# caki35/UNet-Torch

Measured on AMD Instinct MI355X. Metric: images/sec training step, 4-level U-Net 1ch→2cls 512×512, at 1/2/4/8 MI355X, higher is better.
Workload: dtype f16

## Files before the change

### include/unetmi.h

```cpp
#ifndef UNETMI_H
#define UNETMI_H
#include <stddef.h>
#include <stdint.h>

#ifdef __cplusplus
extern "C" {
#endif

typedef void* umi_stream_t;

enum { UMI_F32 = 0, UMI_F16 = 1 };
enum { UMI_OK = 0, UMI_ERR_BADARG = -1, UMI_ERR_UNSUPPORTED = -2, UMI_ERR_WORKSPACE = -3 };
enum { UMI_CONV_UPSAMPLE2 = 1,
       UMI_CONV_FORCE_GENERIC = 2,
       UMI_CONV_DGRAD_STRIDED = 4,
       UMI_CONV_ACCUMULATE = 8,
       UMI_CONV_F32_MFMA = 16       };

int umi_version(void);
const char* umi_arch(void);

int umi_tune_conv3x3_impl(int impl);

int umi_pack_kn(const float* src, void* dst, int T, int K, int N, long st, long sk, long sn,
                int flip_t, int Kpad, int Npad, int dtype, umi_stream_t stream);

int umi_pack_kn8(const float* src, void* dst, int T, int K, int N, long st, long sk, long sn,
                 int flip_t, int Kpad, int Npad, int dtype, umi_stream_t stream);

int umi_conv_fwd(const void* x, int ldx, const void* tx, const void* wp, const float* bias,
                 void* y, int ldy, float* stat_part,
                 int N, int H, int W, int Ci, int Co, int R, int S, int stride, int pad,
                 int Ho, int Wo, int off_h, int off_w, int out_H, int out_W,
                 int in_dtype, int out_dtype, int flags, umi_stream_t stream);
int umi_linear_fused(const void* x, int ldx, const void* wp8, const float* bias, void* y, int ldy, long M, int Ci, int Co,
                     int epi, float p, unsigned seed, const unsigned* seed_dev, void* mask, const void* aux, int ldaux,
                     void* y2, int ldy2, int dtype, umi_stream_t stream);

int umi_conv_fwd_plan(int N, int H, int W, int Ci, int Co, int R, int S, int stride, int pad,
                      int ldx, int ldy, int in_dtype, int out_dtype, int flags, int has_bias,
                      int* layout, int* stat_rows);

int umi_bn_finalize(const float* stat_part, int rows, int C, double count,
                    const float* gamma, const float* beta, float eps, float momentum,
                    float* running_mean, float* running_var,
                    void* tx_out, float* rstd_out, umi_stream_t stream);

int umi_pool2_fwd(const void* x, int ldx, const void* tx, void* y, int ldy,
                  int N, int H, int W, int C, int dtype, umi_stream_t stream);
int umi_pool2_bwd(const void* dpool, int lddp, const void* x, int ldx, const void* tx,
                  void* da, int ldda, int accumulate,
                  int N, int H, int W, int C, int dtype, umi_stream_t stream);

size_t umi_bn_bwd_ws_bytes(long M, int C);
int umi_bn_bwd_reduce(const void* da, int ldda, const void* y, int ldy, const void* tx,
                      const float* rstd, float* sum_dz, float* sum_dzx,
                      long M, int C, int dtype, void* ws, size_t ws_bytes, umi_stream_t stream);
int umi_bn_bwd_apply(void* da, int ldda, const void* y, int ldy, const void* tx,
                     const float* rstd, const float* sum_dz, const float* sum_dzx,
                     long M, int C, int dtype, umi_stream_t stream);

int umi_conv_dgrad_bnred(const void* dy, int lddy, const void* wp8, void* da, int ldda, const void* ybn, int ldybn,
                         const void* txbn, const float* rstd, float* part, int N, int H, int W, int Ci, int Co,
                         int dtype, umi_stream_t stream);

int umi_conv_gather_bnred_rows(int N, int H, int W, int Ci, int Co, int R, int S, int stride, int pad, int Ho, int Wo,
                               int ldx, int ldy, int dtype, int flags);
int umi_conv_gather_bnred(const void* x, int ldx, const void* wp8, void* y, int ldy, const void* ybn, int ldybn,
                          const void* txbn, const float* rstd, float* part, int N, int H, int W, int Ci, int Co, int R, int S,
                          int stride, int pad, int Ho, int Wo, int dtype, int flags, umi_stream_t stream);

int umi_head_dgrad_bnred_rows(long P, int Ci, int Co, int ldda, int dtype);
int umi_head_dgrad_bnred(const void* dl, int lddl, const void* wp, void* da, int ldda, const void* ybn, int ldybn,
                         const void* txbn, const float* rstd, float* part, long P, int Ci, int Co, int dtype,
                         umi_stream_t stream);
size_t umi_head_bwd_fused_ws_bytes(long P, int Ci, int Co);
int umi_head_bwd_fused(const void* dl, int lddl, const void* wp, void* da, int ldda, const void* ybn, int ldybn,
                       const void* txbn, const float* rstd, float* part, float* dW, long s_co, long s_ci, float out_scale,
                       void* ws, size_t ws_bytes, long P, int Ci, int Co, int dtype, umi_stream_t stream);

int umi_conv3x3_fwd_act(const void* x, int ldx, const void* tx, const void* wp8, const void* out_tx, void* y, int ldy,
                        int N, int H, int W, int Ci, int Co, int dtype, umi_stream_t stream);
int umi_bn_stats_rows(long M, int C);
int umi_bn_stats(const void* x, int ldx, float* part, long M, int C, int dtype, umi_stream_t stream);
int umi_pool2_bwd_bnred_stat_rows(int N, int H, int W, int C);
int umi_pool2_bwd_bnred(const void* dpool, int lddp, const void* x, int ldx, const void* tx, const float* rstd, void* da,
                        int ldda, int accumulate, float* part, int N, int H, int W, int C, int dtype, umi_stream_t stream);
int umi_bn_bwd_from_partials(const float* part, int rows, int C, float* sum_dz, float* sum_dzx, umi_stream_t stream);

size_t umi_conv_wgrad_ws_bytes(int N, int Ho, int Wo, int Ci, int Co, int R, int S, int dtype, int flags);
int umi_conv_wgrad(const void* x, int ldx, const void* txa, const void* dy, int lddy, const void* txb,
                   float* dW, long s_co, long s_ci, long s_t, float out_scale,
                   int N, int H, int W, int Ci, int Co, int R, int S, int stride, int pad,
                   int Ho, int Wo, int dtype, int flags, void* ws, size_t ws_bytes, umi_stream_t stream);
typedef struct umi_wgrad_pending {
    const float* part;
    float* dW;
    long s_co, s_ci, s_t;
    float scale;
    int splits, RS, Ci, Co;
} umi_wgrad_pending;
int umi_conv_wgrad_deferred(const void* x, int ldx, const void* txa, const void* dy, int lddy, const void* txb,
                            float* dW, long s_co, long s_ci, long s_t, float out_scale, int N, int H, int W, int Ci, int Co,
                            int R, int S, int stride, int pad, int Ho, int Wo, int dtype, int flags, void* ws, size_t ws_bytes,
                            umi_wgrad_pending* out, umi_stream_t stream);
int umi_wgrad_reduce_group(int n, const void* items , umi_stream_t stream);
int umi_conv_wgrad_bias(const void* x, int ldx, const void* dy, int lddy, const void* txb, float* dW, long s_co, long s_ci,
                        long s_t, float* dbias, float out_scale, int N, int H, int W, int Ci, int Co, int Ho, int Wo, int dtype,
                        int flags, void* ws, size_t ws_bytes, umi_wgrad_pending* out, umi_stream_t stream);
int umi_conv_wgrad_group(int n, const void* const* x, int ldx, const void* const* dy, int lddy, float* const* dW, long s_co,
                         long s_ci, float out_scale, long M, int Ci, int Co, int dtype, umi_stream_t stream);
int umi_conv_wgrad_bnapply(const void* x, int ldx, const void* txa, const void* da, int ldda, const void* y, int ldy,
                           const void* tx_bn, const float* rstd, const float* sum_dz, const float* sum_dzx, void* dz,
                           int lddz, float* dW, long s_co, long s_ci, long s_t, float out_scale, int N, int H, int W,
                           int Ci, int Co, int R, int S, int stride, int pad, int dtype, int flags, void* ws,
                           size_t ws_bytes, umi_stream_t stream);

size_t umi_colsum_ws_bytes(long M, int C);
int umi_colsum(const void* x, int ldx, float* out, float out_scale, long M, int C, int dtype,
               void* ws, size_t ws_bytes, umi_stream_t stream);
int umi_colsum_group(int n, const void* const* xs, int ldx, float* const* outs, float out_scale, long M, int C, int dtype,
                     void* ws, size_t ws_bytes, umi_stream_t stream);

int umi_materialize_nchw(const void* x, int ldx, const void* tx, float* y_nchw,
                         int N, int H, int W, int C, int dtype, umi_stream_t stream);


int umi_wstd_fwd(const float* w, float* wstd, float* rstd, int Co, int K, float eps, umi_stream_t stream);
int umi_wstd_bwd(const float* wstd, const float* rstd, const float* g, float* dw, int Co, int K, umi_stream_t stream);
typedef struct umi_wstd_desc {
    const float* w;
    float* ws;
    float* rstd;
    long off;
    int Co, K;
    float eps;
    int blk0;
    float* dw;
} umi_wstd_desc;
int umi_wstd_fwd_multi(const void* descs, int n_desc, int total_rows, umi_stream_t stream);
int umi_wstd_bwd_multi(const void* descs, int n_desc, int total_rows, const float* g_base, float* dw_base, umi_stream_t stream);

size_t umi_gn_fwd_ws_bytes(int N, long HW, int C);
int umi_gn_fwd(const void* x, int ldx, const float* gamma, const float* beta, const void* res, int ldr, void* y, int ldy,
               float* mean, float* rstd, int relu, int N, long HW, int C, int G, float eps, int dtype,
               void* ws, size_t ws_bytes, umi_stream_t stream);
size_t umi_gn_bwd_ws_bytes(int N, long HW, int C, int G);
int umi_gn_bwd(const void* dy, int lddy, const void* y, int ldy, const void* x, int ldx, const float* mean,
               const float* rstd, const float* gamma, int relu, void* dx, int lddx, void* dres, int lddr,
               float* dgamma, float* dbeta, float out_scale, int N, long HW, int C, int G, int dtype,
               void* ws, size_t ws_bytes, float* part_out, umi_stream_t stream);
int umi_gn_param_grads_group(int n, const float* const* parts, const int* Cs, int N, float* const* dgammas,
                             float* const* dbetas, float out_scale, umi_stream_t stream);

int umi_pool3s2_fwd(const void* x, int ldx, void* y, int ldy, void* idx, int N, int H, int W, int C, int dtype,
                    umi_stream_t stream);
int umi_pool3s2_bwd(const void* dy, int lddy, const void* x, int ldx, const void* idx, void* dx, int lddx, int N, int H, int W,
                    int C, int dtype, umi_stream_t stream);

int umi_ln_fwd(const void* x, int ldx, const float* gamma, const float* beta, void* y, int ldy, float* mean, float* rstd,
               long M, int C, float eps, int dtype, umi_stream_t stream);
size_t umi_ln_bwd_ws_bytes(long M, int C);
int umi_ln_bwd(const void* dy, int lddy, const void* x, int ldx, const float* gamma, const float* mean,
               const float* rstd, void* dx, int lddx, float* dgamma, float* dbeta, float out_scale, long M, int C,
               int dtype, void* ws, size_t ws_bytes, int* rows_out, umi_stream_t stream);

int umi_elementwise(int mode, const void* x, int ldx, const void* g, int ldg, void* y, int ldy, long M, int C,
                    long bcast_rows, int dtype, umi_stream_t stream);

int umi_dropout(const void* x, int ldx, void* y, int ldy, void* mask, int backward, float p, unsigned seed, long M, int C,
                int dtype, const void* tx, const unsigned* seed_dev, umi_stream_t stream);
int umi_dropout_fused(const void* x, int ldx, void* y, int ldy, void* mask, int backward, float p, unsigned seed, long M, int C,
                      int dtype, const unsigned* seed_dev, const void* aux, int ldaux, int gelu, umi_stream_t stream);

int umi_attn_fwd(const void* q, const void* k, const void* v, int ld, void* o, int ldo, float* lse, int B, int N, int heads,
                 int D, int dtype, umi_stream_t stream);
int umi_attn_bwd(const void* q, const void* k, const void* v, int ld, const void* o, const void* dO, int ldo,
                 const float* lse, void* dq, void* dk, void* dv, int ldd, float* delta, int B, int N, int heads, int D,
                 int dtype, umi_stream_t stream);

int umi_bilinear2x(const void* x, int ldx, const void* tx, void* y, int ldy, int backward, int N, int H, int W, int C,
                   int dtype, umi_stream_t stream);

size_t umi_dice_ce_ws_bytes(int N, int C, long HW);
int umi_dice_ce_fwd(const float* logits, const void* target, int target_dtype, int N, int C, long HW, float* stats, void* ws,
                    size_t ws_bytes, umi_stream_t stream);
int umi_dice_ce_bwd(const float* logits, const void* target, int target_dtype, const float* stats, const float* gout, int N,
                    int C, long HW, float* dlogits, umi_stream_t stream);

size_t umi_hdt_ws_bytes(int B, int H, int W);
int umi_hdt_fwd(const float* pred, const float* target, int B, int C, int H, int W, float alpha, float* D, float* fields,
                float* loss, void* ws, size_t ws_bytes, umi_stream_t stream);
int umi_hdt_bwd(const float* pred, const float* target, const float* D, const float* gout, int B, int C, int H, int W,
                float* dpred, umi_stream_t stream);

size_t umi_binloss_ws_bytes(int B, int C, long HW);
int umi_dice_bce_fwd(const float* pred, const float* target, int B, long HW, double* stats, float* loss, void* ws,
                     size_t ws_bytes, umi_stream_t stream);
int umi_dice_bce_bwd(const float* pred, const float* target, const double* stats, const float* gout, int B, long HW,
                     float* dpred, umi_stream_t stream);
int umi_tversky_fwd(const float* pred, const void* target, int target_dtype, int B, int C, long HW, float alpha, float beta,
                    double* stats, float* loss, void* ws, size_t ws_bytes, umi_stream_t stream);
int umi_tversky_bwd(const float* pred, const void* target, int target_dtype, const double* stats, const float* gout, int B,
                    int C, long HW, float alpha, float beta, float* dpred, umi_stream_t stream);

size_t umi_topk_loss_ws_bytes(long N);
int umi_topk_loss_fwd(const float* pred, const float* target, long N, long k, int mode, unsigned char* mask, float* loss,
                      void* ws, size_t ws_bytes, umi_stream_t stream);
int umi_topk_loss_bwd(const float* pred, const float* target, const unsigned char* mask, const float* gout, long N, long k,
                      float* dpred, umi_stream_t stream);

size_t umi_mt_ratio_ws_bytes(int B, long HW);
size_t umi_mt_ratio_stats_len(int B);
int umi_mt_ratio_fwd(const float* o1, const float* o2, const float* l1, const float* l2, int B, long HW, int gate,
                     const float* gate_dev, double* stats, float* loss, float* loss1, float* loss2, float* ratio, void* ws, size_t ws_bytes,
                     umi_stream_t stream);
int umi_mt_ratio_bwd(const float* o1, const float* o2, const float* l1, const float* l2, const double* stats,
                     const float* gout, int B, long HW, float* d1, float* d2, umi_stream_t stream);

typedef struct umi_optim_desc {
    float* p;
    const float* g;
    float* s0;
    float* s1;
    long n;
    int blk0;
    int pad_;
} umi_optim_desc;
int umi_optim_block_elems(void);
int umi_table_upload(const void* host_pinned, void* dev, size_t nbytes, umi_stream_t stream);
int umi_optim_sgd_multi(const void* descs, int n_desc, int total_blocks, double lr, double momentum, double dampening,
                        double weight_decay, int nesterov, int first_step, umi_stream_t stream);
int umi_optim_adam_multi(const void* descs, int n_desc, int total_blocks, double step_size, double beta1, double beta2,
                         double bc2_sqrt, double eps, double weight_decay, umi_stream_t stream);

typedef struct umi_optim_hyper {
    double lr, base_lr, iter, max_iter, power, adam_t, beta1, beta2;
    float lr_f, step_size_f, bc2_sqrt_f, pad_;
    double pad2_[2];
} umi_optim_hyper;
size_t umi_optim_hyper_bytes(void);
int umi_optim_hyper_pre(void* hyper, int adam, umi_stream_t stream);
int umi_optim_hyper_poly(void* hyper, umi_stream_t stream);
int umi_optim_sgd_multi_dev(const void* descs, int n_desc, int total_blocks, const void* hyper, double momentum,
                            double dampening, double weight_decay, int nesterov, int first_step, umi_stream_t stream);
int umi_optim_adam_multi_dev(const void* descs, int n_desc, int total_blocks, const void* hyper, double beta1, double beta2,
                             double eps, double weight_decay, umi_stream_t stream);

typedef struct umi_pack_desc {
    const float* src;
    void* dst;
    long st, sk, sn;
    int T, K, N, flip_t, Kpad, Npad, k8, blk0;
    int ldn, pad_;
} umi_pack_desc;
int umi_pack_block_elems(void);
int umi_pack_kn_multi(const void* descs, int n_desc, int total_blocks, int dtype, umi_stream_t stream);

int umi_add2_relu_fwd(const void* a, int lda, const void* txa, const void* b, int ldb, const void* txb, void* y, int ldy,
                      long M, int C, int dtype, umi_stream_t stream);
int umi_add2_relu_bwd(const void* dy, int lddy, const void* y, int ldy, void* da, int ldda, void* db, int lddb, long M, int C,
                      int dtype, umi_stream_t stream);
int umi_gate_fwd(const void* x, int ldx, const void* txx, const void* p, const void* txp, void* y, int ldy, long M, int C,
                 int dtype, umi_stream_t stream);
int umi_gate_bwd(const void* dy, int lddy, const void* x, int ldx, const void* txx, const void* p, const void* txp, void* dx,
                 int lddx, void* dp, long M, int C, int dtype, umi_stream_t stream);

size_t umi_znorm_ws_bytes(void);
int umi_znorm_hwc(const void* img, int src_dtype, float* out_chw, long HW, int C, int reverse_channels, void* ws,
// ... 57 lines not shown
```

### unet-torch_amd/csrc/api.hip

```cpp
#include "kernels.h"
#include <stdio.h>
#include <stdlib.h>

static ConvFwdProblem fwd_problem(int N, int H, int W, int Ci, int Co, int R, int S, int stride, int pad, int Ho, int Wo, int ldx,
                                  int ldy, int in_dtype, int out_dtype, int flags, bool has_tx, bool has_bias, bool has_stats) {
    return ConvFwdProblem{N, H, W, Ci, Co, R, S, stride, pad, Ho, Wo, ldx, ldy, in_dtype, out_dtype, flags, has_tx, has_bias, has_stats};
}
static ConvFwdProblem fwd_problem_3x3(int N, int H, int W, int Ci, int Co, int ldx, int ldy, int dtype, bool has_tx) {
    return fwd_problem(N, H, W, Ci, Co, 3, 3, 1, 1, H, W, ldx, ldy, dtype, dtype, 0, has_tx, false, false);
}

extern "C" int umi_version(void) { return 1; }
extern "C" const char* umi_arch(void) { return "gfx950"; }

extern "C" int umi_linear_fused(const void* x, int ldx, const void* wp8, const float* bias, void* y, int ldy, long M, int Ci,
                                int Co, int epi, float p, unsigned seed, const unsigned* seed_dev, void* mask, const void* aux,
                                int ldaux, void* y2, int ldy2, int dtype, umi_stream_t stream) {
    if (!x || !wp8 || !y || !mask || M <= 0 || M >= (1L << 31) || Ci <= 0 || Co <= 0 || !(p >= 0.f && p <= 1.f)) return UMI_ERR_BADARG;
    if (epi != 1 && epi != 2) return UMI_ERR_BADARG;
    if ((epi == 1 && (!y2 || ldy2 % 8)) || (epi == 2 && (!aux || ldaux % 8))) return UMI_ERR_BADARG;
    const ConvFwdProblem pr = fwd_problem(1, 1, (int)M, Ci, Co, 1, 1, 1, 0, 1, (int)M, ldx, ldy, dtype, dtype, 0, false, bias != nullptr, false);
    if (umi_conv_fwd_path(pr) != FWD_MFMA1X1) return UMI_ERR_UNSUPPORTED;
    if (((uintptr_t)x | (uintptr_t)y | (uintptr_t)wp8 | (uintptr_t)y2 | (uintptr_t)aux) & 15 || ((uintptr_t)mask & 7)) return UMI_ERR_UNSUPPORTED;
    const UmiLinearEpi e{epi, p, seed, seed_dev, mask, aux, ldaux, y2, ldy2, nullptr, nullptr, nullptr};
    return umi_conv1x1_mfma(pr, x, nullptr, wp8, bias, y, 0, 0, 1, (int)M, (hipStream_t)stream, &e);
}

extern "C" int umi_conv_gather_bnred_rows(int N, int H, int W, int Ci, int Co, int R, int S, int stride, int pad, int Ho, int Wo,
                                          int ldx, int ldy, int dtype, int flags) {
    if (flags & (UMI_CONV_UPSAMPLE2 | UMI_CONV_ACCUMULATE | UMI_CONV_FORCE_GENERIC)) return 0;
    const ConvFwdProblem p = fwd_problem(N, H, W, Ci, Co, R, S, stride, pad, Ho, Wo, ldx, ldy, dtype, dtype, flags, false, false, false);
    if (umi_conv_fwd_path(p) != FWD_MFMA1X1 || umi_conv3x3_mfma_ok(p)) return 0;
    return umi_conv1x1_bnred_rows((long)N * Ho * Wo, Co);
}
extern "C" int umi_conv_gather_bnred(const void* x, int ldx, const void* wp8, void* y, int ldy, const void* ybn, int ldybn,
                                     const void* txbn, const float* rstd, float* part, int N, int H, int W, int Ci, int Co, int R,
                                     int S, int stride, int pad, int Ho, int Wo, int dtype, int flags, umi_stream_t stream) {
    if (!x || !wp8 || !y || !ybn || !txbn || !rstd || !part || N <= 0 || H <= 0 || W <= 0) return UMI_ERR_BADARG;
    if (umi_conv_gather_bnred_rows(N, H, W, Ci, Co, R, S, stride, pad, Ho, Wo, ldx, ldy, dtype, flags) <= 0 || ldybn % 8 || ldybn < Co)
        return UMI_ERR_UNSUPPORTED;
    if (((uintptr_t)x | (uintptr_t)y | (uintptr_t)wp8 | (uintptr_t)ybn) & 15) return UMI_ERR_BADARG;
    const UmiLinearEpi e{3, 0.f, 0u, nullptr, nullptr, ybn, ldybn, nullptr, 0, txbn, rstd, part};
    const ConvFwdProblem p = fwd_problem(N, H, W, Ci, Co, R, S, stride, pad, Ho, Wo, ldx, ldy, dtype, dtype, flags, false, false, false);
    return umi_conv1x1_mfma(p, x, nullptr, wp8, nullptr, y, 0, 0, Ho, Wo, (hipStream_t)stream, &e);
}

extern "C" int umi_conv_fwd_plan(int N, int H, int W, int Ci, int Co, int R, int S, int stride, int pad, int ldx,
                                 int ldy, int in_dtype, int out_dtype, int flags, int has_bias, int* layout,
                                 int* stat_rows) {
    if (N <= 0 || H <= 0 || W <= 0 || Ci <= 0 || Co <= 0 || R <= 0 || S <= 0 || stride <= 0) return UMI_ERR_BADARG;
    const bool ups = flags & UMI_CONV_UPSAMPLE2;
    const int Ho = ups ? H : (H + 2 * pad - R) / stride + 1, Wo = ups ? W : (W + 2 * pad - S) / stride + 1;
    const ConvFwdPath path = umi_conv_fwd_path(fwd_problem(N, H, W, Ci, Co, R, S, stride, pad, Ho, Wo, ldx, ldy, in_dtype, out_dtype,
                                                           flags, false, has_bias != 0, true));
    if ((flags & UMI_CONV_ACCUMULATE) && path != FWD_MFMA1X1) return UMI_ERR_UNSUPPORTED;
    if (layout) *layout = (path == FWD_MFMA3X3 || path == FWD_MFMA1X1) ? 1 : 0;
    if (stat_rows)
        *stat_rows = path == FWD_MFMA3X3_F32 ? umi_conv3x3_f32_mfma_stat_rows(N, H, W)
                     : path == FWD_MFMA3X3 ? umi_conv3x3_mfma_stat_rows(N, H, W, Co)
                     : path == FWD_STEM  ? umi_stem_stat_rows(N, H, W)
                     : path == FWD_HEAD  ? umi_head_stat_rows((long)N * H * W, Ci)
                                         : umi_cdiv((long)N * Ho * Wo, 64);
    return UMI_OK;
}

extern "C" int umi_conv_dgrad_bnred(const void* dy, int lddy, const void* wp8, void* da, int ldda, const void* ybn, int ldybn,
                                    const void* txbn, const float* rstd, float* part, int N, int H, int W, int Ci, int Co,
                                    int dtype, umi_stream_t stream) {
    if (!dy || !wp8 || !da || !ybn || !txbn || !rstd || !part || N <= 0 || H <= 0 || W <= 0) return UMI_ERR_BADARG;
    const ConvFwdProblem p = fwd_problem_3x3(N, H, W, Ci, Co, lddy, ldda, dtype, false);
    if (umi_conv_fwd_path(p) != FWD_MFMA3X3 || ldybn % 8 || ldybn < Co) return UMI_ERR_UNSUPPORTED;
    if (((uintptr_t)dy | (uintptr_t)da | (uintptr_t)wp8 | (uintptr_t)ybn) & 15) return UMI_ERR_BADARG;
    return umi_conv3x3_mfma_bnred(p, dy, wp8, da, ybn, ldybn, txbn, rstd, part, (hipStream_t)stream);
}

static bool head_dgrad_ok(int Ci, int Co, int ldda, int dtype) {
    return umi_smallk_fwd_ok(fwd_problem(1, 1, 1, Ci, Co, 1, 1, 1, 0, 1, 1, Ci, ldda, dtype, dtype, 0, false, false, false));
}
extern "C" int umi_head_dgrad_bnred_rows(long P, int Ci, int Co, int ldda, int dtype) {
    if (!head_dgrad_ok(Ci, Co, ldda, dtype)) return 0;
    return umi_smallk_bnred_rows(P, Co);
}
extern "C" int umi_head_dgrad_bnred(const void* dl, int lddl, const void* wp, void* da, int ldda, const void* ybn, int ldybn,
                                    const void* txbn, const float* rstd, float* part, long P, int Ci, int Co, int dtype,
                                    umi_stream_t stream) {
    if (!dl || !wp || !da || !ybn || !txbn || !rstd || !part || P <= 0) return UMI_ERR_BADARG;
    if (!head_dgrad_ok(Ci, Co, ldda, dtype) || ldybn % 8 || ldybn < Co || lddl < Ci) return UMI_ERR_UNSUPPORTED;
    return umi_smallk_fwd_bnred(dl, lddl, wp, da, ldda, ybn, ldybn, txbn, rstd, part, P, Ci, Co, (hipStream_t)stream);
}
extern "C" size_t umi_head_bwd_fused_ws_bytes(long P, int Ci, int Co) {
    return (size_t)umi_smallk_bnred_rows(P, Co) * Co * Ci * sizeof(float);
}
extern "C" int umi_head_bwd_fused(const void* dl, int lddl, const void* wp, void* da, int ldda, const void* ybn, int ldybn,
                                  const void* txbn, const float* rstd, float* part, float* dW, long s_co, long s_ci, float out_scale,
                                  void* ws, size_t ws_bytes, long P, int Ci, int Co, int dtype, umi_stream_t stream) {
    if (!dl || !wp || !da || !ybn || !txbn || !rstd || !part || !dW || !ws || P <= 0) return UMI_ERR_BADARG;
    if (!head_dgrad_ok(Ci, Co, ldda, dtype) || Co > 256 || ldybn % 8 || ldybn < Co || lddl < Ci) return UMI_ERR_UNSUPPORTED;
    return umi_smallk_fwd_bnred(dl, lddl, wp, da, ldda, ybn, ldybn, txbn, rstd, part, P, Ci, Co, (hipStream_t)stream, dW, s_co, s_ci,
                                out_scale, ws, ws_bytes);
}

extern "C" int umi_conv3x3_fwd_act(const void* x, int ldx, const void* tx, const void* wp8, const void* out_tx, void* y, int ldy,
                                   int N, int H, int W, int Ci, int Co, int dtype, umi_stream_t stream) {
    if (!x || !wp8 || !out_tx || !y || N <= 0 || H <= 0 || W <= 0 || ldx < Ci || ldy < Co) return UMI_ERR_BADARG;
    const ConvFwdProblem p = fwd_problem_3x3(N, H, W, Ci, Co, ldx, ldy, dtype, tx != nullptr);
    if (umi_conv_fwd_path(p) != FWD_MFMA3X3) return UMI_ERR_UNSUPPORTED;
    if (((uintptr_t)x | (uintptr_t)y | (uintptr_t)wp8 | (uintptr_t)out_tx) & 15) return UMI_ERR_BADARG;
    return umi_conv3x3_mfma_act(p, x, tx, wp8, out_tx, y, (hipStream_t)stream);
}

extern "C" int umi_bn_stats_rows(long M, int C) { return umi_colsum_rows_f16v(M, C); }
extern "C" int umi_bn_stats(const void* x, int ldx, float* part, long M, int C, int dtype, umi_stream_t stream) {
    if (!x || !part || M <= 0 || C <= 0 || ldx < C) return UMI_ERR_BADARG;
    if (dtype != UMI_F16 || !umi_bn_stats_f16v(x, ldx, part, M, C, (hipStream_t)stream)) return UMI_ERR_UNSUPPORTED;
    UMI_LAUNCH_CHECK();
    return UMI_OK;
}

extern "C" int umi_pool2_bwd_bnred(const void* dpool, int lddp, const void* x, int ldx, const void* tx, const float* rstd,
                                   void* da, int ldda, int accumulate, float* part, int N, int H, int W, int C, int dtype,
                                   umi_stream_t stream) {
    if (!dpool || !x || !tx || !rstd || !da || !part || N <= 0 || H <= 0 || W <= 0 || C <= 0) return UMI_ERR_BADARG;
    if (dtype != UMI_F16) return UMI_ERR_UNSUPPORTED;
    if (!umi_pool2_bwd_bnred_f16v(dpool, lddp, x, ldx, tx, rstd, da, ldda, accumulate, part, N, H, W, C, (hipStream_t)stream))
        return UMI_ERR_UNSUPPORTED;
    UMI_LAUNCH_CHECK();
    return UMI_OK;
}
extern "C" int umi_pool2_bwd_bnred_stat_rows(int N, int H, int W, int C) { return umi_pool2_bwd_bnred_rows(N, H, W, C); }

extern "C" int umi_bn_bwd_from_partials(const float* part, int rows, int C, float* sum_dz, float* sum_dzx, umi_stream_t stream) {
    if (!part || !sum_dz || !sum_dzx || rows <= 0 || C <= 0) return UMI_ERR_BADARG;
    umi_launch_reduce_rows2(part, rows, C, sum_dz, sum_dzx, 1.f, (hipStream_t)stream);
    UMI_LAUNCH_CHECK();
    return UMI_OK;
}

static bool trace_generic() {
    static const bool on = [] { const char* e = getenv("UMI_TRACE_GENERIC"); return e && e[0] == '1'; }();
    return on;
}
#define UMI_TRACE(kind)                                                                                                  \
    if (trace_generic())                                                                                                 \
        fprintf(stderr, "[umi generic %s] N=%d H=%d W=%d Ci=%d Co=%d R=%d stride=%d pad=%d flags=%d\n", kind, N, H, W, Ci, Co, R, \
                stride, pad, flags)

extern "C" int umi_conv_fwd(const void* x, int ldx, const void* tx, const void* wp, const float* bias, void* y, int ldy,
                            float* stat_part, int N, int H, int W, int Ci, int Co, int R, int S, int stride, int pad,
                            int Ho, int Wo, int off_h, int off_w, int out_H, int out_W, int in_dtype, int out_dtype,
                            int flags, umi_stream_t stream) {
    if (!x || !wp || !y || N <= 0 || H <= 0 || W <= 0 || Ci <= 0 || Co <= 0 || R <= 0 || S <= 0 || stride <= 0 ||
        Ho <= 0 || Wo <= 0 || ldx < Ci || ldy < Co || out_H <= 0 || out_W <= 0)
        return UMI_ERR_BADARG;
    ConvFwdProblem p = fwd_problem(N, H, W, Ci, Co, R, S, stride, pad, Ho, Wo, ldx, ldy, in_dtype, out_dtype, flags,
                                   tx != nullptr, bias != nullptr, stat_part != nullptr);
    const ConvFwdPath path = umi_conv_fwd_path(p);
    if (path != FWD_MFMA3X3_F32) p.flags = flags &= ~UMI_CONV_F32_MFMA;
    if ((flags & UMI_CONV_ACCUMULATE) && (stat_part || path != FWD_MFMA1X1)) return UMI_ERR_UNSUPPORTED;
    if (flags & UMI_CONV_DGRAD_STRIDED) {
        if (flags & UMI_CONV_UPSAMPLE2) return UMI_ERR_BADARG;
        if (H != (Ho + 2 * pad - R) / stride + 1 || W != (Wo + 2 * pad - S) / stride + 1) return UMI_ERR_BADARG;
        if (out_H != Ho || out_W != Wo || off_h || off_w || stat_part) return UMI_ERR_BADARG;
    } else if (!(flags & UMI_CONV_UPSAMPLE2)) {
        if (Ho != (H + 2 * pad - R) / stride + 1 || Wo != (W + 2 * pad - S) / stride + 1) return UMI_ERR_BADARG;
        if (out_H != Ho || out_W != Wo || off_h || off_w) return UMI_ERR_BADARG;
    } else {
        if (Ho != H || Wo != W) return UMI_ERR_BADARG;
    }
    const hipStream_t s = (hipStream_t)stream;
    switch (path) {
    case FWD_MFMA3X3_F32: return umi_conv3x3_f32_mfma(p, x, tx, wp, y, stat_part, s);
    case FWD_MFMA3X3:
        if (((uintptr_t)x | (uintptr_t)y | (uintptr_t)wp) & 15) return UMI_ERR_BADARG;
        return umi_conv3x3_mfma(p, x, tx, wp, y, stat_part, s);
    case FWD_MFMA1X1:
        if (stat_part) return UMI_ERR_UNSUPPORTED;
        if (((uintptr_t)x | (uintptr_t)y | (uintptr_t)wp) & 15) return UMI_ERR_BADARG;
        return umi_conv1x1_mfma(p, x, tx, wp, bias, y, off_h, off_w, out_H, out_W, s);
    case FWD_STEM: return umi_stem_fwd(p, x, tx, wp, y, stat_part, s);
    case FWD_HEAD: return umi_head_fwd(p, x, tx, wp, bias, y, stat_part, s);
    case FWD_SMALLK: return umi_smallk_fwd(p, x, wp, y, s);
    case FWD_ROOT: return umi_root_fwd(p, x, wp, y, s);
    case FWD_HEAD3: return umi_head3_fwd(p, x, tx, wp, bias, y, s);
    case FWD_GENERIC: break;
    }
    UMI_TRACE((flags & UMI_CONV_DGRAD_STRIDED) ? "dgrad_strided" : "fwd");
    return umi_conv_fwd_generic(p, x, tx, wp, bias, y, stat_part, off_h, off_w, out_H, out_W, s);
}

static WgradProblem wgrad_problem(int N, int H, int W, int Ci, int Co, int R, int S, int stride, int pad, int Ho, int Wo, int ldx,
                                  int lddy, int dtype, int flags, bool has_txa, bool has_txb) {
    return WgradProblem{N, H, W, Ci, Co, R, S, stride, pad, Ho, Wo, ldx, lddy, dtype, flags, has_txa, has_txb};
}

extern "C" size_t umi_conv_wgrad_ws_bytes(int N, int Ho, int Wo, int Ci, int Co, int R, int S, int dtype, int flags) {
    WgradProblem p = wgrad_problem(N, 0, 0, Ci, Co, R, S, 0, 0, Ho, Wo, 0, 0, dtype, flags, false, false);
    const size_t f32_mfma = umi_wgrad3x3_f32_mfma_ws_bound(p);
    p.flags &= ~UMI_CONV_F32_MFMA;
    const size_t bounds[] = {f32_mfma, umi_wgrad3x3_mfma_ws_bound(p), umi_wgrad1x1_mfma_ws_bound(p), umi_wgradT_mfma_ws_bound(p),
                             umi_wgrad_gather_mfma_ws_bound(p), umi_stem_wgrad_ws_bound(p), umi_head_wgrad_ws_bound(p),
                             umi_root_wgrad_ws_bound(p), umi_head3_wgrad_ws_bound(p), umi_conv_wgrad_generic_ws_bound(p)};
    size_t most = 0;
    for (size_t b : bounds) most = b > most ? b : most;
    return most;
}

static int conv_wgrad(const WgradProblem& asked, WgradPath path, const void* x, const void* txa, const void* dy, const void* txb,
                      const WgradOut& o, hipStream_t s) {
    WgradProblem p = asked;
    if (path != WGRAD_MFMA3X3_F32) p.flags &= ~UMI_CONV_F32_MFMA;
    if (!x || !dy || !o.dW || !o.ws || p.N <= 0 || p.H <= 0 || p.W <= 0 || p.Ci <= 0 || p.Co <= 0 || p.ldx < p.Ci || p.lddy < p.Co)
        return UMI_ERR_BADARG;
    switch (path) {
    case WGRAD_MFMA3X3_F32: return umi_wgrad3x3_f32_mfma(p, x, txa, dy, o, s);
    case WGRAD_MFMA3X3: return umi_wgrad3x3_mfma(p, x, txa, dy, o, s);
    case WGRAD_MFMA1X1: return umi_wgrad1x1_mfma(p, x, txa, dy, o, s);
    case WGRAD_T: return umi_wgradT_mfma(p, x, dy, txb, o, s);
    case WGRAD_GATHER: return umi_wgrad_gather_mfma(p, x, txa, dy, o, s);
    case WGRAD_STEM: return umi_stem_wgrad(p, x, txa, dy, o, s);
    case WGRAD_HEAD: return umi_head_wgrad(p, x, txa, dy, o, s);
    case WGRAD_ROOT: return umi_root_wgrad(p, x, dy, o, s);
    case WGRAD_HEAD3: return umi_head3_wgrad(p, x, txa, dy, o, s);
    case WGRAD_GENERIC: break;
    }
    if (trace_generic())
        fprintf(stderr, "[umi generic wgrad] N=%d H=%d W=%d Ci=%d Co=%d R=%d stride=%d pad=%d flags=%d\n", p.N, p.H, p.W, p.Ci, p.Co,
                p.R, p.stride, p.pad, p.flags);
    return umi_conv_wgrad_generic(p, x, txa, dy, txb, o, s);
}

extern "C" int umi_conv_wgrad(const void* x, int ldx, const void* txa, const void* dy, int lddy, const void* txb,
                              float* dW, long s_co, long s_ci, long s_t, float out_scale, int N, int H, int W, int Ci,
                              int Co, int R, int S, int stride, int pad, int Ho, int Wo, int dtype, int flags, void* ws,
                              size_t ws_bytes, umi_stream_t stream) {
    const WgradProblem p = wgrad_problem(N, H, W, Ci, Co, R, S, stride, pad, Ho, Wo, ldx, lddy, dtype, flags, txa != nullptr, txb != nullptr);
    const WgradOut o{dW, s_co, s_ci, s_t, out_scale, ws, ws_bytes, nullptr, nullptr};
    return conv_wgrad(p, umi_conv_wgrad_path(p), x, txa, dy, txb, o, (hipStream_t)stream);
}

extern "C" int umi_conv_wgrad_deferred(const void* x, int ldx, const void* txa, const void* dy, int lddy, const void* txb,
                                       float* dW, long s_co, long s_ci, long s_t, float out_scale, int N, int H, int W, int Ci,
                                       int Co, int R, int S, int stride, int pad, int Ho, int Wo, int dtype, int flags, void* ws,
                                       size_t ws_bytes, umi_wgrad_pending* out, umi_stream_t stream) {
    if (!out) return UMI_ERR_BADARG;
    out->part = nullptr;
    const WgradProblem p = wgrad_problem(N, H, W, Ci, Co, R, S, stride, pad, Ho, Wo, ldx, lddy, dtype, flags, txa != nullptr, txb != nullptr);
    const WgradOut o{dW, s_co, s_ci, s_t, out_scale, ws, ws_bytes, out, nullptr};
    return conv_wgrad(p, umi_conv_wgrad_path(p), x, txa, dy, txb, o, (hipStream_t)stream);
}

extern "C" int umi_conv_wgrad_bias(const void* x, int ldx, const void* dy, int lddy, const void* txb, float* dW, long s_co,
                                   long s_ci, long s_t, float* dbias, float out_scale, int N, int H, int W, int Ci, int Co, int Ho,
                                   int Wo, int dtype, int flags, void* ws, size_t ws_bytes, umi_wgrad_pending* out,
                                   umi_stream_t stream) {
    if (!dbias) return UMI_ERR_BADARG;
    const WgradProblem p = wgrad_problem(N, H, W, Ci, Co, 2, 2, 2, 0, Ho, Wo, ldx, lddy, dtype, flags, false, txb != nullptr);
    if (umi_conv_wgrad_path(p) != WGRAD_T) return UMI_ERR_UNSUPPORTED;
    if (out) out->part = nullptr;
    const WgradOut o{dW, s_co, s_ci, s_t, out_scale, ws, ws_bytes, out, dbias};
    return conv_wgrad(p, WGRAD_T, x, nullptr, dy, txb, o, (hipStream_t)stream);
}

extern "C" int umi_conv_wgrad_group(int n, const void* const* x, int ldx, const void* const* dy, int lddy, float* const* dW,
                                    long s_co, long s_ci, float out_scale, long M, int Ci, int Co, int dtype,
                                    umi_stream_t stream) {
    if (n <= 0 || !x || !dy || !dW || M <= 0 || Ci <= 0 || Co <= 0 || ldx < Ci || lddy < Co) return UMI_ERR_BADARG;
    for (int i = 0; i < n; ++i)
        if (!x[i] || !dy[i] || !dW[i]) return UMI_ERR_BADARG;
    if (M >= (1L << 31) ||
        umi_conv_wgrad_path(wgrad_problem(1, 1, (int)M, Ci, Co, 1, 1, 1, 0, 1, (int)M, ldx, lddy, dtype, 0, false, false)) != WGRAD_MFMA1X1)
        return UMI_ERR_UNSUPPORTED;
    return umi_wgrad1x1_mfma_group(n, x, ldx, dy, lddy, dW, s_co, s_ci, out_scale, M, Ci, Co, (hipStream_t)stream);
}

extern "C" int umi_conv_wgrad_bnapply(const void* x, int ldx, const void* txa, const void* da, int ldda, const void* y, int ldy,
                                      const void* tx_bn, const float* rstd, const float* sum_dz, const float* sum_dzx,
                                      void* dz, int lddz, float* dW, long s_co, long s_ci, long s_t, float out_scale, int N,
                                      int H, int W, int Ci, int Co, int R, int S, int stride, int pad, int dtype, int flags,
                                      void* ws, size_t ws_bytes, umi_stream_t stream) {
    if (!x || !da || !y || !tx_bn || !rstd || !sum_dz || !sum_dzx || !dW || !ws || N <= 0 || H <= 0 || W <= 0 || Ci <= 0 ||
        Co <= 0 || ldx < Ci || ldda < Co || ldy < Co || (dz && (lddz < Co || dz == da || dz == y)))
        return UMI_ERR_BADARG;
    const WgradProblem p = wgrad_problem(N, H, W, Ci, Co, R, S, stride, pad, H, W, ldx, ldda, dtype, flags, txa != nullptr, false);
    const WgradPath path = umi_conv_wgrad_path(p);
    const WgradOut o{dW, s_co, s_ci, s_t, out_scale, ws, ws_bytes, nullptr, nullptr};
    const WgradBnApply bna{y, ldy, tx_bn, rstd, sum_dz, sum_dzx, dz, lddz};
    if (!dz) {
        if (path != WGRAD_STEM || ldy % 8) return UMI_ERR_UNSUPPORTED;
        return umi_stem_wgrad(p, x, txa, da, o, (hipStream_t)stream, &bna);
    }
    if (path != WGRAD_MFMA3X3 || ldy % 8 || lddz % 8 || (long)H * W * (ldy > lddz ? ldy : lddz) * 2 >= 0x7FFFFFF0L)
        return UMI_ERR_UNSUPPORTED;
    return umi_wgrad3x3_mfma(p, x, txa, da, o, (hipStream_t)stream, &bna);
}
```

### unet-torch_amd/csrc/common.h

```cpp
#pragma once
#include <hip/hip_runtime.h>
#include <stdint.h>
#include <stddef.h>
#include "../../include/unetmi.h"

typedef _Float16 half_t;

#define UMI_LAUNCH_CHECK()                                    \
    do {                                                      \
        hipError_t e__ = hipGetLastError();                   \
        if (e__ != hipSuccess) return (int)e__;               \
    } while (0)

__device__ __forceinline__ float umi_tx_pre(float v, const float4 t) {
    return fmaf(v, t.y, t.z);
}
__device__ __forceinline__ float umi_tx(float v, const float4 t) {
    return fmaxf(umi_tx_pre(v, t), t.w);
}

__device__ __forceinline__ float umi_bn_dz_inner(float y, float g, const float4 t, float rstd, float c1, float c2) {
#pragma clang fp contract(off)
    const float z = umi_tx_pre(y, t);
    const float dz = z > t.w ? g : 0.f;
    const float xh = (y - t.x) * rstd;
    return fmaf(-xh, c2, dz - c1);
}
__device__ __forceinline__ unsigned umi_mul2_f16(float a0, float b0, float a1, float b1) {
    unsigned r;
    asm("v_fma_mixlo_f16 %0, %1, %2, 0\n\tv_fma_mixhi_f16 %0, %3, %4, 0" : "=&v"(r) : "v"(a0), "v"(b0), "v"(a1), "v"(b1));
    return r;
}
__device__ __forceinline__ _Float16 umi_mul_f16(float a, float b) {
    unsigned r;
    asm("v_fma_mixlo_f16 %0, %1, %2, 0" : "=v"(r) : "v"(a), "v"(b));
    return __builtin_bit_cast(_Float16, (unsigned short)(r & 0xffffu));
}
template <typename T>
__device__ __forceinline__ T umi_bn_dz(float y, float g, const float4 t, float rstd, float c1, float c2);
template <>
__device__ __forceinline__ _Float16 umi_bn_dz<_Float16>(float y, float g, const float4 t, float rstd, float c1, float c2) {
    return umi_mul_f16(t.y, umi_bn_dz_inner(y, g, t, rstd, c1, c2));
}
template <>
__device__ __forceinline__ float umi_bn_dz<float>(float y, float g, const float4 t, float rstd, float c1, float c2) {
    return t.y * umi_bn_dz_inner(y, g, t, rstd, c1, c2);
}

typedef _Float16 umi_half8 __attribute__((ext_vector_type(8)));
typedef unsigned umi_uint4v __attribute__((ext_vector_type(4)));
__device__ __forceinline__ umi_half8 umi_bn_dz8(umi_half8 y, umi_half8 g, const float4* t, const float* rstd, const float* c1,
                                                const float* c2) {
    umi_uint4v r;
#pragma unroll
    for (int j = 0; j < 4; ++j)
        r[j] = umi_mul2_f16(t[2 * j].y, umi_bn_dz_inner((float)y[2 * j], (float)g[2 * j], t[2 * j], rstd[2 * j], c1[2 * j], c2[2 * j]),
                            t[2 * j + 1].y, umi_bn_dz_inner((float)y[2 * j + 1], (float)g[2 * j + 1], t[2 * j + 1], rstd[2 * j + 1],
                                                            c1[2 * j + 1], c2[2 * j + 1]));
    return __builtin_bit_cast(umi_half8, r);
}
__device__ __forceinline__ umi_half8 umi_tx8(umi_half8 v, const float4* t) {
#ifdef UMI_EXP_TX_PK
    umi_half8 sc, sh, lo_;
#pragma unroll
    for (int j = 0; j < 8; ++j) { sc[j] = (half_t)t[j].y; sh[j] = (half_t)t[j].z; lo_[j] = (half_t)t[j].w; }
    return __builtin_elementwise_max(v * sc + sh, lo_);
#endif
    typedef unsigned int u32x4 __attribute__((ext_vector_type(4)));
    u32x4 in = __builtin_bit_cast(u32x4, v), out;
    umi_half8 lo;
#pragma unroll
    for (int p = 0; p < 4; ++p) {
        unsigned d;
        asm("v_fma_mixlo_f16 %0, %1, %2, %3 op_sel_hi:[1,0,0]\n\t"
            "v_fma_mixhi_f16 %0, %1, %4, %5 op_sel:[1,0,0] op_sel_hi:[1,0,0]"
            : "=&v"(d)
            : "v"(in[p]), "v"(t[2 * p].y), "v"(t[2 * p].z), "v"(t[2 * p + 1].y), "v"(t[2 * p + 1].z));
        out[p] = d;
        lo[2 * p] = (half_t)t[2 * p].w;
        lo[2 * p + 1] = (half_t)t[2 * p + 1].w;
    }
    return __builtin_elementwise_max(__builtin_bit_cast(umi_half8, out), lo);
}

template <typename T> __device__ __forceinline__ float umi_ld(const T* p) { return (float)(*p); }
template <typename T> __device__ __forceinline__ void umi_st(T* p, float v) { *p = (T)v; }

static inline int umi_cdiv(long a, long b) { return (int)((a + b - 1) / b); }

__device__ __forceinline__ void umi_divmod(long i, int d, long& q, int& r) {
    if ((unsigned long)i <= 0xFFFFFFFFul) {
        const unsigned ui = (unsigned)i, qq = ui / (unsigned)d;
        q = (long)qq;
        r = (int)(ui - qq * (unsigned)d);
    } else {
        q = i / d;
        r = (int)(i - q * d);
    }
}
```

### unet-torch_amd/csrc/kernels.h

```cpp
#pragma once
#include "common.h"

struct ConvFwdProblem {
    int N, H, W, Ci, Co, R, S, stride, pad, Ho, Wo, ldx, ldy, in_dtype, out_dtype, flags;
    bool has_tx, has_bias, has_stats;
};
enum ConvFwdPath { FWD_MFMA3X3_F32, FWD_MFMA3X3, FWD_MFMA1X1, FWD_STEM, FWD_HEAD, FWD_SMALLK, FWD_ROOT, FWD_HEAD3, FWD_GENERIC };

bool umi_conv3x3_f32_mfma_ok(const ConvFwdProblem& p);
bool umi_conv3x3_mfma_ok(const ConvFwdProblem& p);
bool umi_conv1x1_mfma_ok(const ConvFwdProblem& p);
bool umi_stem_fwd_ok(const ConvFwdProblem& p);
bool umi_head_fwd_ok(const ConvFwdProblem& p);
bool umi_smallk_fwd_ok(const ConvFwdProblem& p);
bool umi_root_fwd_ok(const ConvFwdProblem& p);
bool umi_head3_fwd_ok(const ConvFwdProblem& p);

inline ConvFwdPath umi_conv_fwd_path(const ConvFwdProblem& p) {
    if (p.flags & UMI_CONV_F32_MFMA) {
        if (umi_conv3x3_f32_mfma_ok(p)) return FWD_MFMA3X3_F32;
        ConvFwdProblem q = p;
        q.flags &= ~UMI_CONV_F32_MFMA;
        return umi_conv_fwd_path(q);
    }
    if (p.flags & UMI_CONV_DGRAD_STRIDED)
        return umi_conv1x1_mfma_ok(p) ? FWD_MFMA1X1 : FWD_GENERIC;
    if (umi_conv3x3_mfma_ok(p)) return FWD_MFMA3X3;
    if (umi_conv1x1_mfma_ok(p)) return FWD_MFMA1X1;
    if (umi_stem_fwd_ok(p)) return FWD_STEM;
    if ((!p.has_stats || p.out_dtype == UMI_F16) && umi_head_fwd_ok(p)) return FWD_HEAD;
    if (p.has_stats) return FWD_GENERIC;
    if (umi_smallk_fwd_ok(p)) return FWD_SMALLK;
    if (umi_root_fwd_ok(p)) return FWD_ROOT;
    if (umi_head3_fwd_ok(p)) return FWD_HEAD3;
    return FWD_GENERIC;
}

struct UmiLinearEpi {
    int mode; float p; unsigned seed; const unsigned* seed_dev; void* mask; const void* aux; int ldaux; void* y2; int ldy2;
    const void* bn_tx; const float* bn_rstd; float* bn_part;
};

int umi_conv_fwd_generic(const ConvFwdProblem& p, const void* x, const void* tx, const void* wp, const float* bias, void* y,
                         float* stat_part, int off_h, int off_w, int out_H, int out_W, hipStream_t s);
int umi_conv3x3_f32_mfma_stat_rows(int N, int H, int W);
int umi_conv3x3_f32_mfma(const ConvFwdProblem& p, const void* x, const void* tx, const void* wp, void* y, float* stat_part,
                         hipStream_t s);
int umi_conv3x3_mfma_stat_rows(int N, int H, int W, int Co);
int umi_conv3x3_mfma(const ConvFwdProblem& p, const void* x, const void* tx, const void* wp8, void* y, float* stat_part,
                     hipStream_t s);
int umi_conv3x3_mfma_bnred(const ConvFwdProblem& p, const void* dy, const void* wp8, void* da, const void* ybn, int ldybn,
                           const void* txbn, const float* rstd, float* part, hipStream_t s);
int umi_conv3x3_mfma_act(const ConvFwdProblem& p, const void* x, const void* tx, const void* wp8, const void* out_tx, void* y,
                         hipStream_t s);
int umi_conv1x1_bnred_rows(long M, int Ntot);
int umi_conv1x1_mfma(const ConvFwdProblem& p, const void* x, const void* tx, const void* wp8, const float* bias, void* y,
                     int off_h, int off_w, int out_H, int out_W, hipStream_t s, const UmiLinearEpi* epi = nullptr);
int umi_stem_stat_rows(int N, int H, int W);
int umi_stem_fwd(const ConvFwdProblem& p, const void* x, const void* tx, const void* wp, void* y, float* part, hipStream_t s);
int umi_head_stat_rows(long P, int Ci);
int umi_head_fwd(const ConvFwdProblem& p, const void* x, const void* tx, const void* wp, const float* bias, void* y, float* part,
                 hipStream_t s);
int umi_smallk_fwd(const ConvFwdProblem& p, const void* x, const void* wp, void* y, hipStream_t s);
int umi_smallk_bnred_rows(long P, int Co);
int umi_smallk_fwd_bnred(const void* x, int ldx, const void* wp, void* y, int ldy, const void* ybn, int ldybn, const void* txbn,
                         const float* rstd, float* part, long P, int Ci, int Co, hipStream_t s, float* dW = nullptr, long s_co = 0,
                         long s_ci = 0, float out_scale = 1.f, void* ws = nullptr, size_t ws_bytes = 0);
int umi_root_fwd(const ConvFwdProblem& p, const void* x, const void* wp, void* y, hipStream_t s);
int umi_head3_fwd(const ConvFwdProblem& p, const void* x, const void* tx, const void* wp, const float* bias, void* y,
                  hipStream_t s);

struct WgradProblem {
    int N, H, W, Ci, Co, R, S, stride, pad, Ho, Wo, ldx, lddy, dtype, flags;
    bool has_txa, has_txb;
};
struct WgradOut {
    float* dW; long s_co, s_ci, s_t; float out_scale;
    void* ws; size_t ws_bytes;
    umi_wgrad_pending* defer;
    float* convT_bias;
};
struct WgradBnApply { const void* y; int ldy; const void* tx_bn; const float *rstd, *sum_dz, *sum_dzx; void* dz; int lddz; };
enum WgradPath { WGRAD_MFMA3X3_F32, WGRAD_MFMA3X3, WGRAD_MFMA1X1, WGRAD_T, WGRAD_GATHER, WGRAD_STEM, WGRAD_HEAD, WGRAD_ROOT, WGRAD_HEAD3, WGRAD_GENERIC };

bool umi_wgrad3x3_f32_mfma_ok(const WgradProblem& p);
bool umi_wgrad3x3_mfma_ok(const WgradProblem& p);
bool umi_wgrad1x1_mfma_ok(const WgradProblem& p);
bool umi_wgradT_mfma_ok(const WgradProblem& p);
bool umi_wgrad_gather_mfma_ok(const WgradProblem& p);
bool umi_stem_wgrad_ok(const WgradProblem& p);
bool umi_head_wgrad_ok(const WgradProblem& p);
bool umi_root_wgrad_ok(const WgradProblem& p);
bool umi_head3_wgrad_ok(const WgradProblem& p);

inline WgradPath umi_conv_wgrad_path(const WgradProblem& p) {
    if (p.flags & UMI_CONV_F32_MFMA) {
        if (umi_wgrad3x3_f32_mfma_ok(p)) return WGRAD_MFMA3X3_F32;
        WgradProblem q = p;
        q.flags &= ~UMI_CONV_F32_MFMA;
        return umi_conv_wgrad_path(q);
    }
    if (umi_wgrad3x3_mfma_ok(p)) return WGRAD_MFMA3X3;
    if (umi_wgrad1x1_mfma_ok(p)) return WGRAD_MFMA1X1;
    if (umi_wgradT_mfma_ok(p)) return WGRAD_T;
    if (umi_wgrad_gather_mfma_ok(p)) return WGRAD_GATHER;
    if (umi_stem_wgrad_ok(p)) return WGRAD_STEM;
    if (umi_head_wgrad_ok(p)) return WGRAD_HEAD;
    if (umi_root_wgrad_ok(p)) return WGRAD_ROOT;
    if (umi_head3_wgrad_ok(p)) return WGRAD_HEAD3;
    return WGRAD_GENERIC;
}

size_t umi_wgrad3x3_f32_mfma_ws_bound(const WgradProblem& p);
size_t umi_wgrad3x3_mfma_ws_bound(const WgradProblem& p);
size_t umi_wgrad1x1_mfma_ws_bound(const WgradProblem& p);
size_t umi_wgradT_mfma_ws_bound(const WgradProblem& p);
size_t umi_wgrad_gather_mfma_ws_bound(const WgradProblem& p);
size_t umi_stem_wgrad_ws_bound(const WgradProblem& p);
size_t umi_head_wgrad_ws_bound(const WgradProblem& p);
size_t umi_root_wgrad_ws_bound(const WgradProblem& p);
size_t umi_head3_wgrad_ws_bound(const WgradProblem& p);
size_t umi_conv_wgrad_generic_ws_bound(const WgradProblem& p);

int umi_wgrad3x3_f32_mfma(const WgradProblem& p, const void* x, const void* txa, const void* dy, const WgradOut& o, hipStream_t s);
int umi_wgrad3x3_mfma(const WgradProblem& p, const void* x, const void* txa, const void* dy, const WgradOut& o, hipStream_t s,
                      const WgradBnApply* bna = nullptr);
int umi_wgrad1x1_mfma(const WgradProblem& p, const void* x, const void* txa, const void* dy, const WgradOut& o, hipStream_t s);
int umi_wgradT_mfma(const WgradProblem& p, const void* x, const void* dy, const void* txb, const WgradOut& o, hipStream_t s);
int umi_wgrad_gather_mfma(const WgradProblem& p, const void* x, const void* txa, const void* dy, const WgradOut& o, hipStream_t s);
int umi_stem_wgrad(const WgradProblem& p, const void* x, const void* txa, const void* dy, const WgradOut& o, hipStream_t s,
                   const WgradBnApply* bna = nullptr);
int umi_head_wgrad(const WgradProblem& p, const void* x, const void* txa, const void* dy, const WgradOut& o, hipStream_t s);
int umi_root_wgrad(const WgradProblem& p, const void* x, const void* dy, const WgradOut& o, hipStream_t s);
int umi_head3_wgrad(const WgradProblem& p, const void* x, const void* txa, const void* dy, const WgradOut& o, hipStream_t s);
int umi_conv_wgrad_generic(const WgradProblem& p, const void* x, const void* txa, const void* dy, const void* txb,
                           const WgradOut& o, hipStream_t s);
int umi_wgrad1x1_mfma_group(int n, const void* const* x, int ldx, const void* const* dy, int lddy, float* const* dW, long s_co,
                            long s_ci, float out_scale, long M, int Ci, int Co, hipStream_t s);

void umi_launch_wgrad_reduce(int splits, int RS, int Ci, int Co, const WgradOut& o, hipStream_t s);
void umi_launch_reduce_rows2(const float* ws, int rows, int C, float* out0, float* out1, float scale, hipStream_t s);

int umi_bn_bwd_rpb_f16v(long M);
int umi_colsum_rows_f16v(long M, int C);
bool umi_colsum_f16v(const void* x, int ldx, float* ws, long M, int C, hipStream_t s);
bool umi_colsum_group_f16v(int n, const void* const* xs, int ldx, float* const* outs, float scale, float* ws, long M, int C,
                           hipStream_t s);
bool umi_bn_stats_f16v(const void* x, int ldx, float* part, long M, int C, hipStream_t s);
bool umi_bn_bwd_reduce1_f16v(const void* da, int ldda, const void* y, int ldy, const void* tx, const float* rstd, float* ws,
                             long M, int C, hipStream_t s);
bool umi_bn_bwd_apply_f16v(void* da, int ldda, const void* y, int ldy, const void* tx, const float* rstd,
                           const float* sum_dz, const float* sum_dzx, long M, int C, hipStream_t s);
bool umi_pool2_fwd_f16v(const void* x, int ldx, const void* tx, void* y, int ldy, int N, int H, int W, int C,
                        hipStream_t s);
bool umi_pool2_bwd_f16v(const void* dp, int lddp, const void* x, int ldx, const void* tx, void* da, int ldda,
                        int accumulate, int N, int H, int W, int C, hipStream_t s);
int umi_pool2_bwd_bnred_rows(int N, int H, int W, int C);
bool umi_pool2_bwd_bnred_f16v(const void* dp, int lddp, const void* x, int ldx, const void* tx, const float* rstd, void* da,
                              int ldda, int accumulate, float* part, int N, int H, int W, int C, hipStream_t s);

int umi_gn_splits(int N, long HW);
bool umi_gn_fwd_f16v(const void* x, int ldx, const float* gamma, const float* beta, const void* res, int ldr, void* y, int ldy,
                     float* mean, float* rstd, int relu, int N, long HW, int C, int G, float eps, float* ws, hipStream_t s);
bool umi_gn_bwd_f16v(const void* dy, int lddy, const void* y, int ldy, const void* x, int ldx, const float* mean,
                     const float* rstd, const float* gamma, int relu, void* dx, int lddx, void* dres, int lddr, int N, long HW,
                     int C, int G, float* part, float* ws, hipStream_t s);
void umi_gn_param_grads_launch(int n, const float* const* parts, const int* Cs, int N, float* const* dgammas, float* const* dbetas,
                               float scale, hipStream_t s);

bool umi_ew_f16v(int mode, const void* x, int ldx, const void* g, int ldg, void* y, int ldy, long M, int C, long bcast_rows,
                 hipStream_t s);
bool umi_pool3s2_fwd_f16v(const void* x, int ldx, void* y, int ldy, void* idx, int N, int H, int W, int C, hipStream_t s);
bool umi_pool3s2_bwd_f16v(const void* dy, int lddy, const void* idx, void* dx, int lddx, int N, int H, int W, int C, hipStream_t s);
bool umi_dropout_f16v(const void* x, int ldx, void* y, int ldy, void* mask, int backward, float p, unsigned seed, long M, int C,
                      const void* tx, const unsigned* seed_dev, hipStream_t s);
bool umi_dropout_fused_f16v(const void* x, int ldx, void* y, int ldy, void* mask, int backward, float p, unsigned seed, long M,
                            int C, const unsigned* seed_dev, const void* aux, int ldaux, int gelu, hipStream_t s);
int umi_ln_bwd_rows_f16v();
bool umi_ln_bwd_f16v(const void* dy, int lddy, const void* x, int ldx, const float* gamma, const float* mean, const float* rstd,
                     void* dx, int lddx, float* part, long M, int C, hipStream_t s);
bool umi_bilinear2x_f16v(const void* x, int ldx, const void* tx, void* y, int ldy, int backward, int N, int H, int W, int C,
                         hipStream_t s);

bool umi_attn_mfma_ok(int D, int ld, int ldo, int dtype, const void* a, const void* b, const void* c);
int umi_attn_fwd_mfma(const void* q, const void* k, const void* v, int ld, void* o, int ldo, float* lse, int B, int N, int Hh,
                      hipStream_t s);
int umi_attn_bwd_mfma(const void* q, const void* k, const void* v, int ld, const void* o, const void* dO, int ldo,
                      const float* lse, void* dq, void* dk, void* dv, int ldd, float* delta, int B, int N, int Hh,
                      hipStream_t s);
```

### unet-torch_amd/csrc/stem_head.hip

```cpp
#include "kernels.h"

typedef _Float16 half8 __attribute__((ext_vector_type(8)));

namespace {

constexpr int STEM_PPB = 1024;
constexpr int WG_PPB = 4096;

inline bool al16(const void* p) { return (((uintptr_t)p) & 15) == 0; }

template <int CI>
__global__ __launch_bounds__(256) void stem3x3_fwd_kernel(const half_t* __restrict__ x, int ldx,
                                                          const float4* __restrict__ tx, const half_t* __restrict__ wp,
                                                          half_t* __restrict__ y, int ldy, float* __restrict__ part,
                                                          int N, int H, int W, int Co) {
    extern __shared__ __attribute__((aligned(16))) float sm[];
    const int tid = threadIdx.x;
    const int G = Co >> 3, PL = 256 / G;
    const int cg = tid % G, pl = tid / G;
    float* wsm = sm;
    for (int i = tid; i < 9 * CI * Co; i += 256) wsm[i] = (float)wp[i];
    __syncthreads();
    const long P = (long)N * H * W;
    const long p0 = (long)blockIdx.x * STEM_PPB;
// ... 126 lines not shown
    if (p < pend) {
        n = (int)(p / ((long)H * W));
        const int r = (int)(p - (long)n * H * W);
        yy = r / W;
        xx = r - yy * W;
    }
#pragma unroll 4
    for (; p < pend; p += PL) {
        const half8 g = *reinterpret_cast<const half8*>(dy + p * lddy + cg * 8);
        float win[9];
#pragma unroll
        for (int dy_ = 0; dy_ < 3; ++dy_) {
            const int hi = yy + dy_ - 1;
            const bool rowok = hi >= 0 && hi < H;
            const half_t* xr = x + ((long)((long)n * H + (rowok ? hi : 0)) * W) * ldx + ci;
#pragma unroll
            for (int dx = 0; dx < 3; ++dx) {
                const int wi = xx + dx - 1;
                const bool ok = rowok && wi >= 0 && wi < W;
                float v = (float)xr[(long)(ok ? wi : 0) * ldx];
                if (tx) v = umi_tx(v, tc);
                win[dy_ * 3 + dx] = ok ? v : 0.f;
            }
        }
        float gf[8];
        if (BNA) {
            const half8 yv = *reinterpret_cast<const half8*>(ba.y + p * ba.ldy + cg * 8);
#pragma unroll
            for (int j = 0; j < 8; ++j) gf[j] = (float)umi_bn_dz<_Float16>((float)yv[j], (float)g[j], tb[j], rsb[j], c1[j], c2[j]);
        } else {
#pragma unroll
            for (int j = 0; j < 8; ++j) gf[j] = (float)g[j];
        }
#pragma unroll
        for (int tap = 0; tap < 9; ++tap)
#pragma unroll
            for (int j = 0; j < 8; ++j) acc[tap][j] = fmaf(win[tap], gf[j], acc[tap][j]);
        xx += PL;
        while (xx >= W) {
            xx -= W;
            if (++yy == H) { yy = 0; ++n; }
        }
    }
    for (int tap = 0; tap < 9; ++tap) {
        __syncthreads();
#pragma unroll
        for (int j = 0; j < 8; ++j) red[tid][j] = acc[tap][j];
        __syncthreads();
        if (tid < Co) {
            float a = 0.f;
            for (int k = 0; k < PL; ++k) a += red[k * G + (tid >> 3)][tid & 7];
            part[(((long)blockIdx.x * 9 + tap) * Ci + ci) * Co + tid] = a;
        }
    }
}

template <int NC, typename TO, bool STATS>
__global__ __launch_bounds__(256) void head1x1_fwd_kernel(const half_t* __restrict__ x, int ldx,
                                                          const float4* __restrict__ tx, const half_t* __restrict__ wp,
                                                          const float* __restrict__ bias, TO* __restrict__ y, int ldy,
                                                          float* __restrict__ part, long P, int C) {
    const int G = C >> 3;
    const long gt = (long)blockIdx.x * 256 + threadIdx.x;
    const int cg = (int)(gt % G);
    const long stride_p = ((long)gridDim.x * 256) / G;
    float4 t[8];
    float w[8][NC];
#pragma unroll
    for (int j = 0; j < 8; ++j) {
        t[j] = tx ? tx[cg * 8 + j] : make_float4(0.f, 1.f, 0.f, -INFINITY);
#pragma unroll
        for (int k = 0; k < NC; ++k) w[j][k] = (float)wp[(cg * 8 + j) * NC + k];
    }
    float ssum[NC], ssq[NC];
#pragma unroll
    for (int k = 0; k < NC; ++k) ssum[k] = ssq[k] = 0.f;
    const long Pr = ((P + stride_p - 1) / stride_p) * stride_p;
    for (long p = gt / G; p < Pr; p += stride_p) {
        float acc[NC];
#pragma unroll
        for (int k = 0; k < NC; ++k) acc[k] = 0.f;
        if (p < P) {
            half8 v = *reinterpret_cast<const half8*>(x + p * ldx + cg * 8);
#pragma unroll
            for (int j = 0; j < 8; ++j) {
                float a = umi_tx((float)v[j], t[j]);
#pragma unroll
                for (int k = 0; k < NC; ++k) acc[k] = fmaf(a, w[j][k], acc[k]);
            }
        }
        for (int o = G >> 1; o > 0; o >>= 1)
#pragma unroll
            for (int k = 0; k < NC; ++k) acc[k] += __shfl_xor(acc[k], o);
        if (cg == 0 && p < P) {
#pragma unroll
            for (int k = 0; k < NC; ++k) {
                const TO o = (TO)(acc[k] + (bias ? bias[k] : 0.f));
                y[p * ldy + k] = o;
                if (STATS) {
                    const float vr = (float)o;
                    ssum[k] += vr;
                    ssq[k] = fmaf(vr, vr, ssq[k]);
                }
            }
        }
    }
    if (STATS) {
        __shared__ float red[4][2][NC];
#pragma unroll
        for (int k = 0; k < NC; ++k)
            for (int o = 32; o > 0; o >>= 1) {
                ssum[k] += __shfl_xor(ssum[k], o);
                ssq[k] += __shfl_xor(ssq[k], o);
            }
        if ((threadIdx.x & 63) == 0) {
#pragma unroll
            for (int k = 0; k < NC; ++k) {
                red[threadIdx.x >> 6][0][k] = ssum[k];
                red[threadIdx.x >> 6][1][k] = ssq[k];
            }
        }
        __syncthreads();
        if (threadIdx.x < 2 * NC) {
            const int which = threadIdx.x / NC, k = threadIdx.x - which * NC;
            part[((long)blockIdx.x * 2 + which) * NC + k] =
                (red[0][which][k] + red[1][which][k]) + (red[2][which][k] + red[3][which][k]);
        }
    }
}

template <int NC>
__global__ __launch_bounds__(256) void smallk1x1_fwd_kernel(const half_t* __restrict__ x, int ldx,
                                                            const half_t* __restrict__ wp, half_t* __restrict__ y,
                                                            int ldy, long P, int C) {
    const int G = C >> 3;
    const long gt = (long)blockIdx.x * 256 + threadIdx.x;
    const int cg = (int)(gt % G);
    const long stride_p = ((long)gridDim.x * 256) / G;
    float w[NC][8];
#pragma unroll
    for (int k = 0; k < NC; ++k)
#pragma unroll
        for (int j = 0; j < 8; ++j) w[k][j] = (float)wp[k * C + cg * 8 + j];
    for (long p = gt / G; p < P; p += stride_p) {
        float d[NC];
#pragma unroll
        for (int k = 0; k < NC; ++k) d[k] = (float)x[p * ldx + k];
        half8 o;
#pragma unroll
        for (int j = 0; j < 8; ++j) {
            float a = 0.f;
#pragma unroll
            for (int k = 0; k < NC; ++k) a = fmaf(d[k], w[k][j], a);
            o[j] = (half_t)a;
        }
        *reinterpret_cast<half8*>(y + p * ldy + cg * 8) = o;
    }
}

template <int NC>
__global__ __launch_bounds__(256) void smallk1x1_bnred_kernel(const half_t* __restrict__ x, int ldx,
                                                              const half_t* __restrict__ wp, half_t* __restrict__ y,
                                                              int ldy, const half_t* __restrict__ ybn, int ldybn,
                                                              const float4* __restrict__ txbn, const float* __restrict__ rstd,
                                                              float* __restrict__ part, long P, int C, float* __restrict__ wpart) {
    __shared__ float red[2][256][9];
    const int G = C >> 3;
    const long gt = (long)blockIdx.x * 256 + threadIdx.x;
    const int cg = (int)(gt % G);
    const long stride_p = ((long)gridDim.x * 256) / G;
    float w[NC][8], wacc[NC][8];
    float4 t[8];
    float rs[8], s[8], q[8];
#pragma unroll
    for (int j = 0; j < 8; ++j) {
        t[j] = txbn[cg * 8 + j];
        rs[j] = rstd[cg * 8 + j];
        s[j] = q[j] = 0.f;
#pragma unroll
        for (int k = 0; k < NC; ++k) wacc[k][j] = 0.f;
#pragma unroll
        for (int k = 0; k < NC; ++k) w[k][j] = (float)wp[k * C + cg * 8 + j];
    }
    for (long p = gt / G; p < P; p += stride_p) {
        const half8 yv = *reinterpret_cast<const half8*>(ybn + p * ldybn + cg * 8);
        float d[NC];
#pragma unroll
        for (int k = 0; k < NC; ++k) d[k] = (float)x[p * ldx + k];
        half8 o;
#pragma unroll
        for (int j = 0; j < 8; ++j) {
            float a = 0.f;
#pragma unroll
            for (int k = 0; k < NC; ++k) a = fmaf(d[k], w[k][j], a);
            o[j] = (half_t)a;
            const float yy = (float)yv[j];
            const float dz = umi_tx_pre(yy, t[j]) > t[j].w ? (float)o[j] : 0.f;
            s[j] += dz;
            q[j] = fmaf(dz, (yy - t[j].x) * rs[j], q[j]);
            if (wpart) {
                const float av = umi_tx(yy, t[j]);
#pragma unroll
                for (int k = 0; k < NC; ++k) wacc[k][j] = fmaf(av, d[k], wacc[k][j]);
            }
        }
        *reinterpret_cast<half8*>(y + p * ldy + cg * 8) = o;
    }
#pragma unroll
    for (int j = 0; j < 8; ++j) { red[0][threadIdx.x][j] = s[j]; red[1][threadIdx.x][j] = q[j]; }
    __syncthreads();
    for (int i = threadIdx.x; i < 2 * C; i += 256) {
        const int which = i / C, c = i - which * C;
        float a = 0.f;
        for (int k = 0; k < 256 / G; ++k) a += red[which][k * G + (c >> 3)][c & 7];
        part[((long)blockIdx.x * 2 + which) * C + c] = a;
    }
    if (wpart) {
        for (int k = 0; k < NC; ++k) {
            __syncthreads();
#pragma unroll
            for (int j = 0; j < 8; ++j) red[0][threadIdx.x][j] = wacc[k][j];
            __syncthreads();
            if ((int)threadIdx.x < C) {
                float a = 0.f;
                for (int qq = 0; qq < 256 / G; ++qq) a += red[0][qq * G + (threadIdx.x >> 3)][threadIdx.x & 7];
                wpart[((long)blockIdx.x * C + threadIdx.x) * NC + k] = a;
            }
        }
    }
}

template <int NC>
__global__ __launch_bounds__(256) void head1x1_wgrad_kernel(const half_t* __restrict__ x, int ldx,
                                                            const float4* __restrict__ tx,
                                                            const half_t* __restrict__ dl, int lddl,
                                                            float* __restrict__ part, long P, int C, int ppb) {
    __shared__ float red[256][9];
    const int tid = threadIdx.x;
    const int G = C >> 3, PL = 256 / G;
    const int cg = tid % G, pl = tid / G;
    const long p0 = (long)blockIdx.x * ppb;
    float4 t[8];
#pragma unroll
    for (int j = 0; j < 8; ++j) t[j] = tx ? tx[cg * 8 + j] : make_float4(0.f, 1.f, 0.f, -INFINITY);
    float acc[NC][8];
#pragma unroll
    for (int k = 0; k < NC; ++k)
#pragma unroll
        for (int j = 0; j < 8; ++j) acc[k][j] = 0.f;
    for (long p = p0 + pl; p < p0 + ppb && p < P; p += PL) {
        half8 v = *reinterpret_cast<const half8*>(x + p * ldx + cg * 8);
        float a[8];
#pragma unroll
        for (int j = 0; j < 8; ++j) a[j] = umi_tx((float)v[j], t[j]);
#pragma unroll
        for (int k = 0; k < NC; ++k) {
            float d = (float)dl[p * lddl + k];
#pragma unroll
            for (int j = 0; j < 8; ++j) acc[k][j] = fmaf(a[j], d, acc[k][j]);
        }
    }
    for (int k = 0; k < NC; ++k) {
        __syncthreads();
#pragma unroll
        for (int j = 0; j < 8; ++j) red[tid][j] = acc[k][j];
        __syncthreads();
        if (tid < C) {
            float s = 0.f;
            for (int q = 0; q < PL; ++q) s += red[q * G + (tid >> 3)][tid & 7];
            part[((long)blockIdx.x * C + tid) * NC + k] = s;
        }
    }
}

__global__ __launch_bounds__(256) void head_wpart_reduce_kernel(const float* __restrict__ wpart, int rows, int C, int NC,
                                                                float* __restrict__ dW, long s_co, long s_ci, float scale) {
    __shared__ double sh[256];
    const int e = blockIdx.x, tid = threadIdx.x;
    double a = 0.0;
    for (int r = tid; r < rows; r += 256) a += (double)wpart[(long)r * C * NC + e];
    sh[tid] = a;
    __syncthreads();
    for (int o = 128; o > 0; o >>= 1) {
        if (tid < o) sh[tid] += sh[tid + o];
        __syncthreads();
    }
    if (tid == 0) dW[(e % NC) * s_co + (e / NC) * s_ci] = (float)(sh[0] * (double)scale);
}

int grid_for(long items) {
    long g = (items + 255) / 256;
    if (g > 8192) g = 8192;
    return g < 1 ? 1 : (int)g;
}

bool groups_ok(int C) { return C % 8 == 0 && C / 8 <= 64 && (256 % (C / 8)) == 0; }

}

bool umi_stem_fwd_ok(const ConvFwdProblem& p) {
    if (p.flags & (UMI_CONV_UPSAMPLE2 | UMI_CONV_FORCE_GENERIC)) return false;
    return p.in_dtype == UMI_F16 && p.out_dtype == UMI_F16 && !p.has_bias && p.R == 3 && p.S == 3 && p.stride == 1 && p.pad == 1 &&
           p.Ci >= 1 && p.Ci <= 4 && groups_ok(p.Co) && p.ldy % 8 == 0 && 9 * p.Ci * p.Co * 4 <= 48 * 1024;
}
int umi_stem_stat_rows(int N, int H, int W) { return (int)(((long)N * H * W + STEM_PPB - 1) / STEM_PPB); }

int umi_stem_fwd(const ConvFwdProblem& p, const void* x, const void* tx, const void* wp, void* y, float* part, hipStream_t s) {
    if (!al16(y)) return UMI_ERR_BADARG;
    const int Ci = p.Ci, Co = p.Co;
    const int rows = umi_stem_stat_rows(p.N, p.H, p.W);
    size_t smem = (size_t)9 * Ci * Co * 4;
    if (smem < 2 * 256 * 9 * 4) smem = 2 * 256 * 9 * 4;
#define GO(CI) hipLaunchKernelGGL(stem3x3_fwd_kernel<CI>, dim3(rows), dim3(256), smem, s, (const half_t*)x, p.ldx, (const float4*)tx, (const half_t*)wp, (half_t*)y, p.ldy, part, p.N, p.H, p.W, Co)
    switch (Ci) { case 1: GO(1); break; case 2: GO(2); break; case 3: GO(3); break; default: GO(4); }
#undef GO
    UMI_LAUNCH_CHECK();
    return UMI_OK;
}

bool umi_stem_wgrad_ok(const WgradProblem& p) {
    if (p.flags & UMI_CONV_FORCE_GENERIC) return false;
    return p.dtype == UMI_F16 && !p.has_txb && p.R == 3 && p.S == 3 && p.stride == 1 && p.pad == 1 && p.Ci >= 1 && p.Ci <= 4 &&
           groups_ok(p.Co) && p.Co <= 256 && p.lddy % 8 == 0;
}
static size_t stem_wgrad_ws_bytes(long P, int Ci, int Co) {
    return (size_t)((P + WG_PPB - 1) / WG_PPB) * 9 * Ci * Co * sizeof(float);
}
size_t umi_stem_wgrad_ws_bound(const WgradProblem& facts) {
    WgradProblem p = facts;
    p.stride = p.pad = 1; p.ldx = p.lddy = 8;
    return umi_stem_wgrad_ok(p) ? stem_wgrad_ws_bytes((long)p.N * p.Ho * p.Wo, p.Ci, p.Co) : 0;
}
int umi_stem_wgrad(const WgradProblem& p, const void* x, const void* txa, const void* dy, const WgradOut& o, hipStream_t s,
                   const WgradBnApply* bna) {
    if (o.ws_bytes < stem_wgrad_ws_bytes((long)p.N * p.H * p.W, p.Ci, p.Co)) return UMI_ERR_WORKSPACE;
    if (!al16(dy) || (bna && !al16(bna->y))) return UMI_ERR_BADARG;
    const int N = p.N, H = p.H, W = p.W, Ci = p.Ci, Co = p.Co;
    int blocks = (int)(((long)N * H * W + WG_PPB - 1) / WG_PPB);
    if (!bna)
        hipLaunchKernelGGL(stem3x3_wgrad_kernel<false>, dim3(blocks, Ci), dim3(256), 0, s, (const half_t*)x, p.ldx, (const float4*)txa,
                           (const half_t*)dy, p.lddy, (float*)o.ws, N, H, W, Ci, Co, StemBna{});
    else {
        const StemBna ba{(const half_t*)bna->y, bna->ldy, (const float4*)bna->tx_bn, bna->rstd, bna->sum_dz, bna->sum_dzx, (long)N * H * W};
        hipLaunchKernelGGL(stem3x3_wgrad_kernel<true>, dim3(blocks, Ci), dim3(256), 0, s, (const half_t*)x, p.ldx, (const float4*)txa,
                           (const half_t*)dy, p.lddy, (float*)o.ws, N, H, W, Ci, Co, ba);
    }
    UMI_LAUNCH_CHECK();
    umi_launch_wgrad_reduce(blocks, 9, Ci, Co, o, s);
    UMI_LAUNCH_CHECK();
    return UMI_OK;
}

bool umi_head_fwd_ok(const ConvFwdProblem& p) {
    if (p.flags & (UMI_CONV_UPSAMPLE2 | UMI_CONV_FORCE_GENERIC)) return false;
    return p.in_dtype == UMI_F16 && (p.out_dtype == UMI_F32 || p.out_dtype == UMI_F16) && p.R == 1 && p.S == 1 && p.stride == 1 &&
           p.pad == 0 && p.Co >= 1 && p.Co <= 8 && groups_ok(p.Ci) && p.ldx % 8 == 0;
}
int umi_head_stat_rows(long P, int Ci) { return grid_for(P * (Ci / 8)); }
int umi_head_fwd(const ConvFwdProblem& p, const void* x, const void* tx, const void* wp, const float* bias, void* y, float* part,
                 hipStream_t s) {
    if (!al16(x)) return UMI_ERR_BADARG;
    const long P = (long)p.N * p.H * p.W;
    const int Ci = p.Ci, out_dtype = p.out_dtype;
    if (part && out_dtype != UMI_F16) return UMI_ERR_UNSUPPORTED;
    int grid = grid_for(P * (Ci / 8));
#define GO_(NC, TO, ST) hipLaunchKernelGGL((head1x1_fwd_kernel<NC, TO, ST>), dim3(grid), dim3(256), 0, s, (const half_t*)x, p.ldx, (const float4*)tx, (const half_t*)wp, bias, (TO*)y, p.ldy, part, P, Ci)
#define GO(NC)                                                          \
    do {                                                                \
        if (out_dtype == UMI_F32) GO_(NC, float, false);                \
        else if (part) GO_(NC, half_t, true);                           \
        else GO_(NC, half_t, false);                                    \
    } while (0)
    switch (p.Co) { case 1: GO(1); break; case 2: GO(2); break; case 3: GO(3); break; case 4: GO(4); break;
                    case 5: GO(5); break; case 6: GO(6); break; case 7: GO(7); break; default: GO(8); }
#undef GO
#undef GO_
    UMI_LAUNCH_CHECK();
    return UMI_OK;
}

bool umi_smallk_fwd_ok(const ConvFwdProblem& p) {
    if (p.flags & (UMI_CONV_UPSAMPLE2 | UMI_CONV_FORCE_GENERIC)) return false;
    return p.in_dtype == UMI_F16 && p.out_dtype == UMI_F16 && !p.has_tx && !p.has_bias && p.R == 1 && p.S == 1 && p.stride == 1 &&
           p.pad == 0 && p.Ci >= 1 && p.Ci <= 8 && groups_ok(p.Co) && p.ldy % 8 == 0;
}
int umi_smallk_fwd(const ConvFwdProblem& p, const void* x, const void* wp, void* y, hipStream_t s) {
    if (!al16(y)) return UMI_ERR_BADARG;
    const long P = (long)p.N * p.H * p.W;
    const int Co = p.Co;
    int grid = grid_for(P * (Co / 8));
#define GO(NC) hipLaunchKernelGGL(smallk1x1_fwd_kernel<NC>, dim3(grid), dim3(256), 0, s, (const half_t*)x, p.ldx, (const half_t*)wp, (half_t*)y, p.ldy, P, Co)
    switch (p.Ci) { case 1: GO(1); break; case 2: GO(2); break; case 3: GO(3); break; case 4: GO(4); break;
                    case 5: GO(5); break; case 6: GO(6); break; case 7: GO(7); break; default: GO(8); }
#undef GO
    UMI_LAUNCH_CHECK();
    return UMI_OK;
}

int umi_smallk_bnred_rows(long P, int Co) { return grid_for(P * (Co / 8)); }
int umi_smallk_fwd_bnred(const void* x, int ldx, const void* wp, void* y, int ldy, const void* ybn, int ldybn, const void* txbn,
                         const float* rstd, float* part, long P, int Ci, int Co, hipStream_t s, float* dW, long s_co, long s_ci,
                         float out_scale, void* ws, size_t ws_bytes) {
    if (!al16(y) || !al16(ybn)) return UMI_ERR_BADARG;
    int grid = grid_for(P * (Co / 8));
    float* wpart = nullptr;
    if (dW) {
        if (!ws || ws_bytes < (size_t)grid * Co * Ci * sizeof(float)) return UMI_ERR_WORKSPACE;
        wpart = (float*)ws;
    }
#define GO(NC) hipLaunchKernelGGL(smallk1x1_bnred_kernel<NC>, dim3(grid), dim3(256), 0, s, (const half_t*)x, ldx, (const half_t*)wp, (half_t*)y, ldy, (const half_t*)ybn, ldybn, (const float4*)txbn, rstd, part, P, Co, wpart)
    switch (Ci) { case 1: GO(1); break; case 2: GO(2); break; case 3: GO(3); break; case 4: GO(4); break;
                  case 5: GO(5); break; case 6: GO(6); break; case 7: GO(7); break; default: GO(8); }
#undef GO
    UMI_LAUNCH_CHECK();
    if (dW) {
        hipLaunchKernelGGL(head_wpart_reduce_kernel, dim3(Co * Ci), dim3(256), 0, s, (const float*)wpart, grid, Co, Ci, dW, s_co, s_ci,
                           out_scale);
        UMI_LAUNCH_CHECK();
    }
    return UMI_OK;
}

bool umi_head_wgrad_ok(const WgradProblem& p) {
    if (p.flags & UMI_CONV_FORCE_GENERIC) return false;
    return p.dtype == UMI_F16 && !p.has_txb && p.R == 1 && p.S == 1 && p.stride == 1 && p.pad == 0 && p.Co >= 1 && p.Co <= 8 &&
           groups_ok(p.Ci) && p.Ci <= 256 && p.ldx % 8 == 0;
}
static int head_wgrad_ppb(long P) {
    long ppb = (P + 2047) / 2048;
    ppb = ((ppb + 255) / 256) * 256;
    if (ppb > WG_PPB) ppb = WG_PPB;
    return (int)ppb;
}
static size_t head_wgrad_ws_bytes(long P, int Ci, int Co) {
    const int ppb = head_wgrad_ppb(P);
    return (size_t)((P + ppb - 1) / ppb) * Ci * Co * sizeof(float);
}
size_t umi_head_wgrad_ws_bound(const WgradProblem& facts) {
    WgradProblem p = facts;
    p.stride = 1; p.pad = 0; p.ldx = p.lddy = 8;
    return umi_head_wgrad_ok(p) ? head_wgrad_ws_bytes((long)p.N * p.Ho * p.Wo, p.Ci, p.Co) : 0;
}
int umi_head_wgrad(const WgradProblem& p, const void* x, const void* txa, const void* dy, const WgradOut& o, hipStream_t s) {
    if (o.ws_bytes < head_wgrad_ws_bytes((long)p.N * p.H * p.W, p.Ci, p.Co)) return UMI_ERR_WORKSPACE;
    if (!al16(x)) return UMI_ERR_BADARG;
    const long P = (long)p.N * p.H * p.W;
    const int Ci = p.Ci, ppb = head_wgrad_ppb(P);
    int blocks = (int)((P + ppb - 1) / ppb);
#define GO(NC) hipLaunchKernelGGL(head1x1_wgrad_kernel<NC>, dim3(blocks), dim3(256), 0, s, (const half_t*)x, p.ldx, (const float4*)txa, (const half_t*)dy, p.lddy, (float*)o.ws, P, Ci, ppb)
    switch (p.Co) { case 1: GO(1); break; case 2: GO(2); break; case 3: GO(3); break; case 4: GO(4); break;
                    case 5: GO(5); break; case 6: GO(6); break; case 7: GO(7); break; default: GO(8); }
#undef GO
    UMI_LAUNCH_CHECK();
    umi_launch_wgrad_reduce(blocks, 1, Ci, p.Co, o, s);
    UMI_LAUNCH_CHECK();
    return UMI_OK;
}
```

### unet-torch_amd/csrc/wgrad_mfma.hip

```cpp
#include "kernels.h"
#include <type_traits>
#include <stdlib.h>

typedef _Float16 half8 __attribute__((ext_vector_type(8)));
typedef _Float16 half4 __attribute__((ext_vector_type(4)));
typedef short short4v __attribute__((ext_vector_type(4)));
typedef float floatx16 __attribute__((ext_vector_type(16)));

#ifdef UMI_STAMP
__device__ unsigned long long umi_stamp_buf_w[2048 * 8];
#define UMI_TW(var)                                                                       \
    unsigned long long var;                                                               \
    __builtin_amdgcn_sched_barrier(0);                                                    \
    asm volatile("s_memtime %0\n\ts_waitcnt lgkmcnt(0)" : "=s"(var)::"memory");           \
    __builtin_amdgcn_sched_barrier(0)
extern "C" int umi_debug_read_stamps_w(void* dst) {
    return (int)hipMemcpyFromSymbol(dst, HIP_SYMBOL(umi_stamp_buf_w), sizeof(umi_stamp_buf_w));
}
#endif

namespace {

constexpr int TR = 4;
constexpr int HPIX = (TR + 2) * 34;
// ... 62 lines not shown
    for (int a = 0; a < 9; ++a)
#pragma unroll
        for (int r = 0; r < 16; ++r) acc[a][r] = 0.f;

    half8 araw[KPA], braw[KPB];
    bool avalid[KPA];

    int nx_n, nx_y, nx_x;
    {
        const int tpi = tiles_x * tiles_y;
        nx_n = t_begin / tpi;
        const int rm = t_begin - nx_n * tpi;
        nx_y = (rm / tiles_x) * TR;
        nx_x = (rm % tiles_x) * 32;
    }
#define UMI_ISSUE()                                                                                              \
    do {                                                                                                        \
                \
        const __amdgpu_buffer_rsrc_t xrs = __builtin_amdgcn_make_buffer_rsrc((void*)(x + nx_n * ximg), 0, (int)(ximg * 2), 0x00020000); \
        const __amdgpu_buffer_rsrc_t yrs = __builtin_amdgcn_make_buffer_rsrc((void*)(dy + nx_n * yimg), 0, (int)(yimg * 2), 0x00020000); \
        const int org = nx_y * W + nx_x;                                                                        \
        const unsigned abase = (unsigned)org * (unsigned)(ldx * 2), bbase = (unsigned)org * (unsigned)(lddy * 2);  \
        _Pragma("unroll") for (int k = 0; k < KPA; ++k) {                                                       \
            const int gy = nx_y + (hyx[k] >> 16), gx = nx_x + (int)(short)(hyx[k] & 0xffff);                    \
            avalid[k] = hyx[k] != (int)0x80000000 && (unsigned)gy < (unsigned)H && (unsigned)gx < (unsigned)W;  \
            araw[k] = __builtin_bit_cast(half8, __builtin_amdgcn_raw_buffer_load_b128(                          \
                xrs, avalid[k] ? abase + (unsigned)aoff[k] : OOB, 0, 0));                                       \
        }                                                                                                       \
        _Pragma("unroll") for (int k = 0; k < KPB; ++k) {                                                       \
            const bool ok = b_on && nx_y + k < H && nx_x + bcol < W;                                            \
            braw[k] = __builtin_bit_cast(half8, __builtin_amdgcn_raw_buffer_load_b128(                          \
                yrs, ok ? bbase + (unsigned)(boff0 + k * W * lddy * 2) : OOB, 0, 0));                           \
        }                                                                                                       \
        nx_x += 32;                                                                                             \
        if (nx_x >= W) { nx_x = 0; nx_y += TR; if (nx_y >= H) { nx_y = 0; ++nx_n; } }                           \
    } while (0)

    const int g = lane >> 4, li = lane & 15, lq = li >> 2, lp = li & 3;
    const int frag_lane = (8 * (g >> 1) + lq) * PROW + (16 * (g & 1) + 4 * lp) * 2;
    const unsigned char* a_frag = smem + wci * A_CHUNK + frag_lane;
    const unsigned char* b_frag = smem + A_BYTES + wco * B_CHUNK + frag_lane;

    if (t_begin < t_end) UMI_ISSUE();
#ifdef UMI_STAMP
    UMI_TW(t_loop);
#endif
    for (int tile = t_begin; tile < t_end; ++tile) {
#ifdef UMI_STAMP
        UMI_TW(t0);
        asm volatile("s_waitcnt vmcnt(0)" ::: "memory");
        UMI_TW(t0b);
#endif
        if (HAS_TX) {
            int opaque = 0;
            asm volatile("" : "+v"(opaque));
            float4 t[8];
#pragma unroll
            for (int j = 0; j < 8; ++j) t[j] = txs[j * 8 + sub + opaque];
#pragma unroll
            for (int k = 0; k < KPA; ++k)
                if (avalid[k]) {
                    araw[k] = umi_tx8(araw[k], t);
                }
        }
#pragma unroll
        for (int k = 0; k < KPA; ++k)
            if ((tid >> 3) + 32 * k < HPIX) *reinterpret_cast<half8*>(smem + a_lds + k * 32 * PROW) = araw[k];
#pragma unroll
        for (int k = 0; k < KPB; ++k) *reinterpret_cast<half8*>(smem + b_lds + k * 32 * PROW) = braw[k];
#ifdef UMI_STAMP
        UMI_TW(t1);
#endif
        __syncthreads();
#ifdef UMI_STAMP
        UMI_TW(t2);
#endif
        if (tile + 1 < t_end) UMI_ISSUE();

#pragma unroll
        for (int xh = 0; xh < 2; ++xh) {
            half8 bfr[TR];
#pragma unroll
            for (int r = 0; r < TR; ++r) {
#ifndef UMI_EXP_W_NO_FRAG
                bfr[r] = tr_frag(b_frag + (r * 32 + 16 * xh) * PROW);
#else
                bfr[r] = braw[r];
#endif
            }
#pragma unroll
            for (int dx = 0; dx < 3; ++dx) {
                half8 afr[TR + 2];
#pragma unroll
                for (int rr = 0; rr < TR + 2; ++rr) {
#ifndef UMI_EXP_W_NO_FRAG
                    afr[rr] = tr_frag(a_frag + (rr * 34 + 16 * xh + dx) * PROW);
#else
                    afr[rr] = araw[rr];
#endif
                }
#pragma unroll
                for (int r = 0; r < TR; ++r)
#pragma unroll
                    for (int dyi = 0; dyi < 3; ++dyi) {
#ifndef UMI_EXP_W_NO_MFMA
                        acc[dyi * 3 + dx] =
                            __builtin_amdgcn_mfma_f32_32x32x16_f16(afr[r + dyi], bfr[r], acc[dyi * 3 + dx], 0, 0, 0);
#else
                        asm volatile("" ::"v"(afr[r + dyi]), "v"(bfr[r]));
#endif
                    }
            }
        }
#ifdef UMI_STAMP
        UMI_TW(t3);
#endif
        __syncthreads();
#ifdef UMI_STAMP
        UMI_TW(t4);
        seg[0] += t0b - t0; seg[1] += t1 - t0b; seg[2] += t2 - t1; seg[3] += t3 - t2; seg[4] += t4 - t3;
#endif
    }
#undef UMI_ISSUE
#ifdef UMI_STAMP
    UMI_TW(t_ep0);
#endif

    const int co = co0 + wco * 32 + (lane & 31);
#pragma unroll
    for (int tap = 0; tap < 9; ++tap)
#pragma unroll
        for (int r = 0; r < 16; ++r) {
            int ci = ci0 + wci * 32 + (r & 3) + 8 * (r >> 2) + 4 * (lane >> 5);
            if (ci < Ci && co < Co) part[(((long)blockIdx.y * 9 + tap) * Ci + ci) * Co + co] = acc[tap][r];
        }
#ifdef UMI_STAMP
    UMI_TW(t_end_);
    const int bid = blockIdx.y * gridDim.x + blockIdx.x;
    if (lane == 0 && bid < 512) {
#pragma unroll
        for (int i = 0; i < 5; ++i) umi_stamp_buf_w[(bid * 4 + wave) * 8 + i] = seg[i];
        umi_stamp_buf_w[(bid * 4 + wave) * 8 + 5] = t_end - t_begin;
        umi_stamp_buf_w[(bid * 4 + wave) * 8 + 6] = t_loop - t_start;
        umi_stamp_buf_w[(bid * 4 + wave) * 8 + 7] = t_end_ - t_ep0;
    }
#endif
}

constexpr int WS_SMEM = 2 * SMEM;

struct BnApply {
    const half_t* y; int ldy; const float4* tx; const float* rstd; const float* sum_dz; const float* sum_dzx; long M;
    half_t* dz; int lddz;
};

template <bool HAS_TX, bool BNA>
__global__ __launch_bounds__(512, 1) void wgrad3x3_ws_kernel(
    const half_t* __restrict__ x, int ldx, const float4* __restrict__ tx, const half_t* __restrict__ dy, int lddy,
    float* __restrict__ part, int N, int H, int W, int Ci, int Co, int tiles_x, int tiles_y, int tiles_total,
    int tiles_per_split, int n_co_t, int fast_ci, BnApply ba) {
    extern __shared__ __attribute__((aligned(16))) unsigned char smem_ws[];
    float4* txs = reinterpret_cast<float4*>(smem_ws + WS_SMEM);
    const int tid = threadIdx.x;
    const int lane = tid & 63, wave = tid >> 6;
    const bool producer = wave >= 4;
    const int n_ci_t = (int)gridDim.x / n_co_t;
    const int ci0 = (fast_ci ? (int)blockIdx.x % n_ci_t : (int)blockIdx.x / n_co_t) * 64;
    const int co0 = (fast_ci ? (int)blockIdx.x / n_ci_t : (int)blockIdx.x % n_co_t) * 64;
    const int t_begin = blockIdx.y * tiles_per_split;
    int t_end = t_begin + tiles_per_split;
    if (t_end > tiles_total) t_end = tiles_total;
    const int ntile = t_end - t_begin;
    if (HAS_TX) {
        if (tid < 64) txs[(tid & 7) * 8 + (tid >> 3)] = ci0 + tid < Ci ? tx[ci0 + tid] : make_float4(0.f, 1.f, 0.f, 0.f);
        __syncthreads();
    }

    if (producer) {
        const int ptid = tid - 256;
        const int sub = ptid & 7;
        const bool a_on = ci0 + sub * 8 < Ci, b_on = co0 + sub * 8 < Co;
        constexpr unsigned OOB = 0x7FFFFFFFu;
        int hyx[KPA], aoff[KPA];
#pragma unroll
        for (int k = 0; k < KPA; ++k) {
            int hp = (ptid >> 3) + 32 * k;
            int hy = hp / 34, hx = hp - hy * 34;
            hyx[k] = (hp < HPIX && a_on) ? (int)(((unsigned)(hy - 1) << 16) | ((unsigned)(hx - 1) & 0xffffu)) : (int)0x80000000;
            aoff[k] = (((hy - 1) * W + (hx - 1)) * ldx + ci0 + sub * 8) * 2;
        }
        const bool whole_tiles = (W & 31) == 0 && H % TR == 0;
        const int aback = (W + 1) * ldx * 2;
        int ering[KPA];
        unsigned aoffb[KPA];
#pragma unroll
        for (int k = 0; k < KPA; ++k) {
            int hp = (ptid >> 3) + 32 * k;
            int hy = hp / 34, hx = hp - hy * 34;
            ering[k] = (hp < HPIX && a_on) ? ((hx == 0 ? 1 : 0) | (hx == 33 ? 2 : 0) | (hy == 0 ? 4 : 0) | (hy == TR + 1 ? 8 : 0)) : 16;
            aoffb[k] = (unsigned)(aoff[k] + aback);
        }
        const int bcol = ptid >> 3;
        const int boff0 = (bcol * lddy + co0 + sub * 8) * 2;
        const int a_lds = (sub >> 2) * A_CHUNK + (ptid >> 3) * PROW + (sub & 3) * 16;
        const int b_lds = A_BYTES + (sub >> 2) * B_CHUNK + (ptid >> 3) * PROW + (sub & 3) * 16;
        const long ximg = (long)H * W * ldx, yimg = (long)H * W * lddy;
        float4 t[8];
#pragma unroll
        for (int j = 0; j < 8; ++j) t[j] = HAS_TX ? txs[j * 8 + sub] : make_float4(0.f, 1.f, 0.f, 0.f);
        float4 tb[8];
        float rsb[8], c1[8], c2[8];
        const long ybimg = BNA ? (long)H * W * ba.ldy : 0;
        const int ybo0 = BNA ? (bcol * ba.ldy + co0 + sub * 8) * 2 : 0;
        const bool dz_writer = BNA && ci0 == 0;
        if (BNA) {
            const float invM = 1.f / (float)ba.M;
#pragma unroll
            for (int j = 0; j < 8; ++j) {
                const int c = co0 + sub * 8 + j;
                const bool in = c < Co;
                tb[j] = in ? ba.tx[c] : make_float4(0.f, 1.f, 0.f, 0.f);
                rsb[j] = in ? ba.rstd[c] : 0.f;
                c1[j] = in ? ba.sum_dz[c] * invM : 0.f;
                c2[j] = in ? ba.sum_dzx[c] * invM : 0.f;
            }
        }
        half8 yraw0[KPB], yraw1[KPB];
        bool bvalid0[KPB], bvalid1[KPB];
        int st_n0 = 0, st_y0 = 0, st_x0 = 0, st_n1 = 0, st_y1 = 0, st_x1 = 0;
        half8 araw0[KPA], braw0[KPB], araw1[KPA], braw1[KPB];
        bool avalid0[KPA], avalid1[KPA];
        int nx_n, nx_y, nx_x;
        {
            const int tpi = tiles_x * tiles_y;
            nx_n = t_begin / tpi;
            const int rm = t_begin - nx_n * tpi;
            nx_y = (rm / tiles_x) * TR;
            nx_x = (rm % tiles_x) * 32;
        }
#ifdef UMI_EXP_WS_NO_LOAD
#define UMI_EXP_LOAD_OK(c_) ((c_) && H < 0)
#else
#define UMI_EXP_LOAD_OK(c_) (c_)
#endif
#define UMI_ISSUE_WS(S)                                                                                          \
    do {                                                                                                        \
        const __amdgpu_buffer_rsrc_t xrs = __builtin_amdgcn_make_buffer_rsrc((void*)(x + nx_n * ximg), 0, (int)(ximg * 2), 0x00020000); \
        const __amdgpu_buffer_rsrc_t yrs = __builtin_amdgcn_make_buffer_rsrc((void*)(dy + nx_n * yimg), 0, (int)(yimg * 2), 0x00020000); \
        const int org = nx_y * W + nx_x;                                                                        \
        const unsigned abase = (unsigned)org * (unsigned)(ldx * 2), bbase = (unsigned)org * (unsigned)(lddy * 2);  \
        if (whole_tiles) {                                                                                      \
            const __amdgpu_buffer_rsrc_t xrsb = __builtin_amdgcn_make_buffer_rsrc((void*)((const char*)(x + nx_n * ximg) - aback), 0, (int)(ximg * 2) + aback, 0x00020000); \
            const int edge = (nx_x == 0 ? 1 : 0) | (nx_x + 32 >= W ? 2 : 0) | (nx_y == 0 ? 4 : 0) | (nx_y + TR >= H ? 8 : 0) | 16; \
            _Pragma("unroll") for (int k = 0; k < KPA; ++k) {                                                   \
                avalid##S[k] = (ering[k] & edge) == 0;                                                          \
                araw##S[k] = __builtin_bit_cast(half8, __builtin_amdgcn_raw_buffer_load_b128(                   \
                    xrsb, UMI_EXP_LOAD_OK(avalid##S[k]) ? aoffb[k] : OOB, abase, 0));                           \
            }                                                                                                   \
        } else {                                                                                                \
            _Pragma("unroll") for (int k = 0; k < KPA; ++k) {                                                   \
                const int gy = nx_y + (hyx[k] >> 16), gx = nx_x + (int)(short)(hyx[k] & 0xffff);                \
                avalid##S[k] = hyx[k] != (int)0x80000000 && (unsigned)gy < (unsigned)H && (unsigned)gx < (unsigned)W; \
                araw##S[k] = __builtin_bit_cast(half8, __builtin_amdgcn_raw_buffer_load_b128(                   \
                    xrs, UMI_EXP_LOAD_OK(avalid##S[k]) ? abase + (unsigned)aoff[k] : OOB, 0, 0));               \
            }                                                                                                   \
        }                                                                                                       \
        _Pragma("unroll") for (int k = 0; k < KPB; ++k) {                                                       \
            const bool ok = b_on && (whole_tiles || (nx_y + k < H && nx_x + bcol < W));                         \
            braw##S[k] = __builtin_bit_cast(half8, __builtin_amdgcn_raw_buffer_load_b128(                       \
                yrs, UMI_EXP_LOAD_OK(ok) ? (unsigned)boff0 : OOB, bbase + k * W * lddy * 2, 0));                \
            if (BNA) {                                                                                          \
                const __amdgpu_buffer_rsrc_t ybrs = __builtin_amdgcn_make_buffer_rsrc((void*)(ba.y + nx_n * ybimg), 0, (int)(ybimg * 2), 0x00020000); \
                bvalid##S[k] = ok;                                                                              \
                yraw##S[k] = __builtin_bit_cast(half8, __builtin_amdgcn_raw_buffer_load_b128(                   \
                    ybrs, ok ? (unsigned)org * (unsigned)(ba.ldy * 2) + (unsigned)(ybo0 + k * W * ba.ldy * 2) : OOB, 0, 0)); \
            }                                                                                                   \
        }                                                                                                       \
        if (BNA) { st_n##S = nx_n; st_y##S = nx_y; st_x##S = nx_x; }                                            \
        nx_x += 32;                                                                                             \
        if (nx_x >= W) { nx_x = 0; nx_y += TR; if (nx_y >= H) { nx_y = 0; ++nx_n; } }                           \
    } while (0)
#ifdef UMI_EXP_WS_NO_STORE
#define UMI_STORE_WS(S, buf_)                                                                                    \
    do {                                                                                                        \
        _Pragma("unroll") for (int k = 0; k < KPA; ++k) asm volatile("" ::"v"(araw##S[k]));                     \
        _Pragma("unroll") for (int k = 0; k < KPB; ++k) asm volatile("" ::"v"(braw##S[k]));                     \
    } while (0)
#else
#define UMI_STORE_WS(S, buf_)                                                                                    \
    do {                                                                                                        \
        unsigned char* sb = smem_ws + (buf_) * SMEM;                                                            \
        if (HAS_TX) {                                                                                           \
            _Pragma("unroll") for (int k = 0; k < KPA; ++k) {                                                   \
                const half8 t8 = umi_tx8(araw##S[k], t);                                                        \
                araw##S[k] = avalid##S[k] ? t8 : araw##S[k];       \
            }                                                                                                   \
        }                                                                                                       \
        _Pragma("unroll") for (int k = 0; k < KPA; ++k)                                                         \
            if ((ptid >> 3) + 32 * k < HPIX) *reinterpret_cast<half8*>(sb + a_lds + k * 32 * PROW) = araw##S[k]; \
        if (BNA) {                                                                                              \
            _Pragma("unroll") for (int k = 0; k < KPB; ++k) {                                                   \
                const half8 o = umi_bn_dz8(yraw##S[k], braw##S[k], tb, rsb, c1, c2);    \
                braw##S[k] = bvalid##S[k] ? o : braw##S[k];              \
                if (dz_writer && bvalid##S[k])                                                                  \
                    *reinterpret_cast<half8*>(ba.dz + ((long)((long)st_n##S * H + st_y##S + k) * W + st_x##S + bcol) * ba.lddz + \
                                              co0 + sub * 8) = braw##S[k];                                      \
            }                                                                                                   \
        }                                                                                                       \
        _Pragma("unroll") for (int k = 0; k < KPB; ++k) *reinterpret_cast<half8*>(sb + b_lds + k * 32 * PROW) = braw##S[k]; \
    } while (0)
#endif

        if (ntile > 0) UMI_ISSUE_WS(0);
        if (ntile > 1) UMI_ISSUE_WS(1);
        if (ntile > 0) UMI_STORE_WS(0, 0);
        if (ntile > 2) UMI_ISSUE_WS(0);
        __syncthreads();
#ifdef UMI_STAMP
        unsigned long long pw = 0, pb = 0;
#define UMI_PS(a_) UMI_TW(a_)
#else
#define UMI_PS(a_)
#endif
        for (int i = 0; i < ntile; i += 2) {
            UMI_PS(q0);
#ifndef UMI_EXP_WS_NO_PROD
            if (i + 1 < ntile) {
                UMI_STORE_WS(1, 1);
                if (i + 3 < ntile) UMI_ISSUE_WS(1);
            }
#endif
            UMI_PS(q1);
            __syncthreads();
            UMI_PS(q2);
            if (i + 1 < ntile) {
#ifndef UMI_EXP_WS_NO_PROD
                if (i + 2 < ntile) {
                    UMI_STORE_WS(0, 0);
                    if (i + 4 < ntile) UMI_ISSUE_WS(0);
                }
#endif
                UMI_PS(q3);
                __syncthreads();
                UMI_PS(q4);
#ifdef UMI_STAMP
                pw += q3 - q2; pb += q4 - q3;
#endif
            }
#ifdef UMI_STAMP
            pw += q1 - q0; pb += q2 - q1;
#endif
        }
#ifdef UMI_STAMP
        {
            const int bid = blockIdx.y * gridDim.x + blockIdx.x;
            if (lane == 0 && bid < 256) {
                umi_stamp_buf_w[(bid * 8 + wave) * 8 + 0] = pw;
                umi_stamp_buf_w[(bid * 8 + wave) * 8 + 1] = pb;
                umi_stamp_buf_w[(bid * 8 + wave) * 8 + 5] = ntile;
            }
        }
#endif
#undef UMI_PS
#undef UMI_ISSUE_WS
#undef UMI_STORE_WS
        return;
    }

    __builtin_amdgcn_s_setprio(3);
    const int wci = wave >> 1, wco = wave & 1;
    typedef float floatx4 __attribute__((ext_vector_type(4)));
    floatx4 acc[9][2][2];
#pragma unroll
    for (int t = 0; t < 9; ++t)
#pragma unroll
        for (int ca = 0; ca < 2; ++ca)
#pragma unroll
            for (int cb = 0; cb < 2; ++cb)
#pragma unroll
                for (int r = 0; r < 4; ++r) acc[t][ca][cb][r] = 0.f;
    const int g = lane >> 4, li = lane & 15, lq = li >> 2, lp = li & 3;
    const int frag_lane = (8 * g + lq) * PROW + (4 * lp) * 2;
    __syncthreads();
#define UMI_LD_A16(dst, ca_, dx_)                                                                                \
    _Pragma("unroll") for (int rr = 0; rr < TR + 2; ++rr) dst[rr] = tr_frag(a_frag + (rr * 34 + (dx_)) * PROW + (ca_) * 32)
#define UMI_MMA16(af_, ca_, dx_)                                                                                 \
    _Pragma("unroll") for (int r = 0; r < TR; ++r)                                                              \
        _Pragma("unroll") for (int dyi = 0; dyi < 3; ++dyi)                                                     \
            _Pragma("unroll") for (int cb = 0; cb < 2; ++cb)                                                    \
                acc[dyi * 3 + (dx_)][ca_][cb] = __builtin_amdgcn_mfma_f32_16x16x32_f16(af_[r + dyi], bfr[r][cb], acc[dyi * 3 + (dx_)][ca_][cb], 0, 0, 0)
#define UMI_PIN() __builtin_amdgcn_sched_barrier(0)
#ifdef UMI_STAMP
    unsigned long long cw = 0, cb_ = 0, cstart = 0;
#endif
    for (int i = 0; i < ntile; ++i) {
#ifdef UMI_STAMP
        UMI_TW(c0);
#endif
        const unsigned char* a_frag = smem_ws + (i & 1) * SMEM + wci * A_CHUNK + frag_lane;
        const unsigned char* b_frag = smem_ws + (i & 1) * SMEM + A_BYTES + wco * B_CHUNK + frag_lane;
        half8 a0[TR + 2], a1[TR + 2], bfr[TR][2];
#pragma unroll
        for (int r = 0; r < TR; ++r)
#pragma unroll
            for (int cb = 0; cb < 2; ++cb) bfr[r][cb] = tr_frag(b_frag + (r * 32) * PROW + cb * 32);
#ifndef UMI_WS_COARSE
#define UMI_STEP(ld_, mma_) do { ld_; mma_;                                                              \
            _Pragma("unroll") for (int i_ = 0; i_ < 12; ++i_) {                                                     \
                __builtin_amdgcn_sched_group_barrier(0x008, 2, 0); __builtin_amdgcn_sched_group_barrier(0x100, 1, 0); }  \
            UMI_PIN(); } while (0)
        UMI_LD_A16(a0, 0, 0); UMI_PIN();
        UMI_STEP(UMI_LD_A16(a1, 1, 0), UMI_MMA16(a0, 0, 0));
        UMI_STEP(UMI_LD_A16(a0, 0, 1), UMI_MMA16(a1, 1, 0));
        UMI_STEP(UMI_LD_A16(a1, 1, 1), UMI_MMA16(a0, 0, 1));
        UMI_STEP(UMI_LD_A16(a0, 0, 2), UMI_MMA16(a1, 1, 1));
        UMI_STEP(UMI_LD_A16(a1, 1, 2), UMI_MMA16(a0, 0, 2));
        UMI_MMA16(a1, 1, 2);
#undef UMI_STEP
#else
        UMI_LD_A16(a0, 0, 0); UMI_PIN();
#ifdef UMI_STAMP_STEPS
        asm volatile("s_waitcnt lgkmcnt(0)" ::: "memory");
        UMI_TW(cs0);
        cstart += cs0 - c0;
#endif
        UMI_LD_A16(a1, 1, 0); UMI_PIN(); UMI_MMA16(a0, 0, 0); UMI_PIN();
        UMI_LD_A16(a0, 0, 1); UMI_PIN(); UMI_MMA16(a1, 1, 0); UMI_PIN();
        UMI_LD_A16(a1, 1, 1); UMI_PIN(); UMI_MMA16(a0, 0, 1); UMI_PIN();
        UMI_LD_A16(a0, 0, 2); UMI_PIN(); UMI_MMA16(a1, 1, 1); UMI_PIN();
        UMI_LD_A16(a1, 1, 2); UMI_PIN(); UMI_MMA16(a0, 0, 2); UMI_PIN();
        UMI_MMA16(a1, 1, 2);
#endif
#ifdef UMI_STAMP
        UMI_TW(c1);
#endif
        __syncthreads();
#ifdef UMI_STAMP
        UMI_TW(c2);
        cw += c1 - c0; cb_ += c2 - c1;
#endif
    }
#ifdef UMI_STAMP
    {
        const int bid = blockIdx.y * gridDim.x + blockIdx.x;
        if (lane == 0 && bid < 256) {
            umi_stamp_buf_w[(bid * 8 + wave) * 8 + 0] = cw;
            umi_stamp_buf_w[(bid * 8 + wave) * 8 + 1] = cb_;
            umi_stamp_buf_w[(bid * 8 + wave) * 8 + 2] = cstart;
            umi_stamp_buf_w[(bid * 8 + wave) * 8 + 5] = ntile;
        }
    }
#endif
#undef UMI_LD_A16
#undef UMI_MMA16
#undef UMI_PIN
#pragma unroll
    for (int tap = 0; tap < 9; ++tap)
#pragma unroll
        for (int ca = 0; ca < 2; ++ca)
#pragma unroll
            for (int cb = 0; cb < 2; ++cb) {
                const int co = co0 + wco * 32 + cb * 16 + (lane & 15);
// ... 363 lines not shown
    int tt, splits, tps;
    plan1(M, Ci, Co, wgrad1x1_tm(Ci, Co), &tt, &splits, &tps, taps);
    return (size_t)splits * taps * Ci * Co * sizeof(float);
}
size_t umi_wgrad1x1_mfma_ws_bound(const WgradProblem& facts) {
    WgradProblem p = facts;
    p.H = p.Ho; p.W = p.Wo; p.stride = 1; p.pad = 0; p.ldx = p.lddy = 8;
    return umi_wgrad1x1_mfma_ok(p) ? wgrad1x1_ws_bytes((long)p.N * p.Ho * p.Wo, p.Ci, p.Co, 1) : 0;
}

int umi_wgrad1x1_mfma(const WgradProblem& p, const void* x, const void* txa, const void* dy, const WgradOut& o, hipStream_t s) {
    const long M = (long)p.N * p.H * p.W;
    const int Ci = p.Ci, Co = p.Co, TM = wgrad1x1_tm(Ci, Co);
    int tt, splits, tps;
    plan1(M, Ci, Co, TM, &tt, &splits, &tps);
    if (o.ws_bytes < (size_t)splits * Ci * Co * sizeof(float)) return UMI_ERR_WORKSPACE;
    if (((uintptr_t)x | (uintptr_t)dy) & 15) return UMI_ERR_BADARG;
    const int n_co_t = (Co + TM - 1) / TM;
    dim3 grid(((Ci + TM - 1) / TM) * n_co_t, splits), block(256);
    const WGeo geo{1, 1, 1, 1, 1, 1, 0};
#define GO(T_, H_) hipLaunchKernelGGL((wgrad1x1_mfma_kernel<T_, H_, false>), grid, block, 0, s, (const half_t*)x, p.ldx, (const float4*)txa, (const half_t*)dy, p.lddy, (float*)o.ws, M, Ci, Co, tt, tps, n_co_t, geo, WNoGroup{})
    if (TM == 128) { if (txa) GO(128, true); else GO(128, false); }
    else { if (txa) GO(64, true); else GO(64, false); }
#undef GO
    UMI_LAUNCH_CHECK();
    umi_launch_wgrad_reduce(splits, 1, Ci, Co, o, s);
    UMI_LAUNCH_CHECK();
    return UMI_OK;
}

int umi_wgrad1x1_mfma_group(int n, const void* const* x, int ldx, const void* const* dy, int lddy, float* const* dW, long s_co,
                            long s_ci, float out_scale, long M, int Ci, int Co, hipStream_t s) {
    const bool t128 = Ci % 128 == 0 && Co % 128 == 0 && (long)(Ci / 128) * (Co / 128) * (n < 16 ? n : 16) >= 96;
    const int TM = t128 ? 128 : 64;
    const int tt = (int)((M + 63) / 64), n_co_t = (Co + TM - 1) / TM;
    const WGeo geo{1, 1, 1, 1, 1, 1, 0};
    for (int g0 = 0; g0 < n; g0 += 16) {
        const int cnt = n - g0 < 16 ? n - g0 : 16;
        WGroup grp;
        for (int i = 0; i < 16; ++i) {
            const int j = g0 + (i < cnt ? i : 0);
            if (((uintptr_t)x[j] | (uintptr_t)dy[j]) & 15) return UMI_ERR_BADARG;
            grp.x[i] = (const half_t*)x[j]; grp.dy[i] = (const half_t*)dy[j]; grp.dW[i] = dW[j];
        }
        grp.s_co = s_co; grp.s_ci = s_ci; grp.scale = out_scale;
        dim3 grid(((Ci + TM - 1) / TM) * n_co_t, 1, cnt), block(256);
        if (TM == 128)
            hipLaunchKernelGGL((wgrad1x1_mfma_kernel<128, false, false, true>), grid, block, 0, s, (const half_t*)nullptr, ldx,
                               (const float4*)nullptr, (const half_t*)nullptr, lddy, (float*)nullptr, M, Ci, Co, tt, tt, n_co_t, geo, grp);
        else
            hipLaunchKernelGGL((wgrad1x1_mfma_kernel<64, false, false, true>), grid, block, 0, s, (const half_t*)nullptr, ldx,
                               (const float4*)nullptr, (const half_t*)nullptr, lddy, (float*)nullptr, M, Ci, Co, tt, tt, n_co_t, geo, grp);
        UMI_LAUNCH_CHECK();
    }
    return UMI_OK;
}

static bool wgrad_gather_shape_ok(const WgradProblem& p) {
    if (p.flags & UMI_CONV_FORCE_GENERIC) return false;
    if (p.dtype != UMI_F16 || p.has_txb) return false;
    return p.R * p.S <= 49 && p.Ci % 64 == 0 && p.Co % 64 == 0;
}
bool umi_wgrad_gather_mfma_ok(const WgradProblem& p) {
    if (!wgrad_gather_shape_ok(p) || p.stride < 1 || p.pad < 0) return false;
    if (p.Ho != (p.H + 2 * p.pad - p.R) / p.stride + 1 || p.Wo != (p.W + 2 * p.pad - p.S) / p.stride + 1) return false;
    if (p.ldx % 8 || p.lddy % 8) return false;
    if ((long)p.N * p.Ho * p.Wo * p.lddy * 2 >= 0x7FFFFFF0L || (long)p.N * p.H * p.W * p.ldx * 2 >= 0x7FFFFFF0L) return false;
    return true;
}
size_t umi_wgrad_gather_mfma_ws_bound(const WgradProblem& p) {
    return wgrad_gather_shape_ok(p) ? wgrad1x1_ws_bytes((long)p.N * p.Ho * p.Wo, p.Ci, p.Co, p.R * p.S) : 0;
}

int umi_wgrad_gather_mfma(const WgradProblem& p, const void* x, const void* txa, const void* dy, const WgradOut& o, hipStream_t s) {
    const int Ci = p.Ci, Co = p.Co, TM = wgrad1x1_tm(Ci, Co), taps = p.R * p.S;
    const long M = (long)p.N * p.Ho * p.Wo;
    int tt, splits, tps;
    plan1(M, Ci, Co, TM, &tt, &splits, &tps, taps);
    if (o.ws_bytes < (size_t)splits * taps * Ci * Co * sizeof(float)) return UMI_ERR_WORKSPACE;
    if (((uintptr_t)x | (uintptr_t)dy) & 15) return UMI_ERR_BADARG;
    const int n_co_t = Co / TM;
    dim3 grid((Ci / TM) * n_co_t, splits, taps), block(256);
    const WGeo geo{p.Ho, p.Wo, p.H, p.W, p.S, p.stride, p.pad};
#define GO(T_, H_) hipLaunchKernelGGL((wgrad1x1_mfma_kernel<T_, H_, true>), grid, block, 0, s, (const half_t*)x, p.ldx, (const float4*)txa, (const half_t*)dy, p.lddy, (float*)o.ws, M, Ci, Co, tt, tps, n_co_t, geo, WNoGroup{})
    if (TM == 128) { if (txa) GO(128, true); else GO(128, false); }
    else { if (txa) GO(64, true); else GO(64, false); }
#undef GO
    UMI_LAUNCH_CHECK();
    umi_launch_wgrad_reduce(splits, taps, Ci, Co, o, s);
    UMI_LAUNCH_CHECK();
    return UMI_OK;
}

bool umi_wgradT_mfma_ok(const WgradProblem& p) {
    if (p.flags & UMI_CONV_FORCE_GENERIC) return false;
    if (p.dtype != UMI_F16 || p.has_txa) return false;
    if (p.R != 2 || p.S != 2 || p.stride != 2 || p.pad != 0 || p.H != 2 * p.Ho || p.W != 2 * p.Wo) return false;
    if (p.Ci % 64 || p.Co % 64 || p.ldx % 8 || p.lddy % 8) return false;
    return true;
}
size_t umi_wgradT_mfma_ws_bound(const WgradProblem& facts) {
    WgradProblem p = facts;
    p.H = 2 * p.Ho; p.W = 2 * p.Wo; p.stride = 2; p.pad = 0; p.ldx = p.lddy = 8;
    if (!umi_wgradT_mfma_ok(p)) return 0;
    int tx_, ty_, tt, splits, tps;
    planT(p.N, p.Ho, p.Wo, p.Ci, p.Co, &tx_, &ty_, &tt, &splits, &tps);
    return (size_t)splits * 4 * p.Ci * p.Co * sizeof(float) + (size_t)splits * 2 * p.Ci * sizeof(float);
}

int umi_wgradT_mfma(const WgradProblem& p, const void* x, const void* dy, const void* txb, const WgradOut& o, hipStream_t s) {
    const int N = p.N, Ho = p.Ho, Wo = p.Wo, Ci = p.Ci, Co = p.Co;
    int tiles_x, tiles_y, tiles_total, splits, tps;
    planT(N, Ho, Wo, Ci, Co, &tiles_x, &tiles_y, &tiles_total, &splits, &tps);
    float* const bias_out = o.convT_bias;
    if (o.ws_bytes < (size_t)splits * 4 * Ci * Co * sizeof(float) + (bias_out ? (size_t)splits * 2 * Ci * sizeof(float) : 0)) return UMI_ERR_WORKSPACE;
    if (((uintptr_t)x | (uintptr_t)dy) & 15) return UMI_ERR_BADARG;
    float* const cpart = bias_out ? (float*)o.ws + (size_t)splits * 4 * Ci * Co : nullptr;
    const bool wide = Co % 128 == 0;
    const int n_cy_t = wide ? Co / 128 : Co / 64;
    dim3 grid((Ci / 64) * n_cy_t, splits), block(256);
#define UMI_GO_T(HT, YH_)                                                                                        \
    hipLaunchKernelGGL((wgradT2x2_mfma_kernel<HT, YH_>), grid, block, 0, s, (const half_t*)x, p.ldx, (const half_t*)dy, p.lddy, \
                       (const float4*)txb, (float*)o.ws, N, Ho, Wo, Ci, Co, tiles_x, tiles_y, tiles_total, tps, n_cy_t, cpart)
    if (txb) { if (wide) UMI_GO_T(true, 2); else UMI_GO_T(true, 1); }
    else { if (wide) UMI_GO_T(false, 2); else UMI_GO_T(false, 1); }
#undef UMI_GO_T
    if (bias_out) {
        UMI_LAUNCH_CHECK();
        umi_launch_reduce_rows2(cpart, splits, Ci, bias_out, nullptr, o.out_scale, s);
    }
    UMI_LAUNCH_CHECK();
    umi_launch_wgrad_reduce(splits, 4, Ci, Co, o, s);
    UMI_LAUNCH_CHECK();
    return UMI_OK;
}

bool umi_wgrad3x3_mfma_ok(const WgradProblem& p) {
    if (p.flags & UMI_CONV_FORCE_GENERIC) return false;
    if (p.dtype != UMI_F16 || p.has_txb) return false;
    if (p.R != 3 || p.S != 3 || p.stride != 1 || p.pad != 1 || p.Ho != p.H || p.Wo != p.W) return false;
    if (p.Ci % 8 || p.Co % 8 || p.ldx % 8 || p.lddy % 8) return false;
    if ((long)p.H * p.W * (p.ldx > p.lddy ? p.ldx : p.lddy) * 2 >= 0x7FFFFFF0L) return false;
    return true;
}
size_t umi_wgrad3x3_mfma_ws_bound(const WgradProblem& facts) {
    WgradProblem p = facts;
    p.H = p.Ho; p.W = p.Wo; p.stride = p.pad = 1; p.ldx = p.lddy = 8;
    if (!umi_wgrad3x3_mfma_ok(p)) return 0;
    int tx_, ty_, tt, splits, tps;
    plan(p.N, p.H, p.W, p.Ci, p.Co, &tx_, &ty_, &tt, &splits, &tps);
    return (size_t)splits * 9 * p.Ci * p.Co * sizeof(float);
}

int umi_wgrad3x3_mfma(const WgradProblem& p, const void* x, const void* txa, const void* dy, const WgradOut& o, hipStream_t s,
                      const WgradBnApply* bna) {
    const int N = p.N, H = p.H, W = p.W, Ci = p.Ci, Co = p.Co, ldx = p.ldx, lddy = p.lddy;
    void* const ws = o.ws;
    int tiles_x, tiles_y, tiles_total, splits, tps;
    plan(N, H, W, Ci, Co, &tiles_x, &tiles_y, &tiles_total, &splits, &tps);
    if (o.ws_bytes < (size_t)splits * 9 * Ci * Co * sizeof(float)) return UMI_ERR_WORKSPACE;
    if (((uintptr_t)x | (uintptr_t)dy) & 15) return UMI_ERR_BADARG;
    const int n_co_t = (Co + 63) / 64;
    dim3 grid(((Ci + 63) / 64) * n_co_t, splits), block(256);
    static const int force_fast = [] { const char* e = getenv("UMI_WGRAD_FAST_CI"); return e ? atoi(e) : -1; }();
    const int fast_ci = force_fast >= 0 ? force_fast : (Co < 1.59 * Ci ? 1 : 0);
    static const bool classic = [] { const char* e = getenv("UMI_WGRAD_CLASSIC"); return e && e[0] == '1'; }();
    if (bna && classic) return UMI_ERR_UNSUPPORTED;
    if (!classic) {
        constexpr int dyn = WS_SMEM + 64 * (int)sizeof(float4);
        static const int attr_rc = [] {
            int a = (int)hipFuncSetAttribute((const void*)wgrad3x3_ws_kernel<true, false>, hipFuncAttributeMaxDynamicSharedMemorySize, dyn);
            int b = (int)hipFuncSetAttribute((const void*)wgrad3x3_ws_kernel<false, false>, hipFuncAttributeMaxDynamicSharedMemorySize, dyn);
            int c = (int)hipFuncSetAttribute((const void*)wgrad3x3_ws_kernel<true, true>, hipFuncAttributeMaxDynamicSharedMemorySize, dyn);
            int d = (int)hipFuncSetAttribute((const void*)wgrad3x3_ws_kernel<false, true>, hipFuncAttributeMaxDynamicSharedMemorySize, dyn);
            return a ? a : (b ? b : (c ? c : d));
        }();
        if (attr_rc) return attr_rc;
        dim3 block_ws(512);
        const BnApply ba = bna ? BnApply{(const half_t*)bna->y, bna->ldy, (const float4*)bna->tx_bn, bna->rstd, bna->sum_dz, bna->sum_dzx,
                                         (long)N * H * W, (half_t*)bna->dz, bna->lddz}
                               : BnApply{nullptr, 0, nullptr, nullptr, nullptr, nullptr, 1, nullptr, 0};
#define GO_WS(HT, BN_)                                                                                              \
        hipLaunchKernelGGL((wgrad3x3_ws_kernel<HT, BN_>), grid, block_ws, dyn, s, (const half_t*)x, ldx, (const float4*)txa,   \
                           (const half_t*)dy, lddy, (float*)ws, N, H, W, Ci, Co, tiles_x, tiles_y, tiles_total, tps, n_co_t, fast_ci, ba)
        if (bna) { if (txa) GO_WS(true, true); else GO_WS(false, true); }
        else { if (txa) GO_WS(true, false); else GO_WS(false, false); }
#undef GO_WS
    } else if (txa)
        hipLaunchKernelGGL(wgrad3x3_mfma_kernel<true>, grid, block, 0, s, (const half_t*)x, ldx, (const float4*)txa,
                           (const half_t*)dy, lddy, (float*)ws, N, H, W, Ci, Co, tiles_x, tiles_y, tiles_total, tps,
                           n_co_t, fast_ci);
    else
        hipLaunchKernelGGL(wgrad3x3_mfma_kernel<false>, grid, block, 0, s, (const half_t*)x, ldx, (const float4*)txa,
                           (const half_t*)dy, lddy, (float*)ws, N, H, W, Ci, Co, tiles_x, tiles_y, tiles_total, tps,
                           n_co_t, fast_ci);
    UMI_LAUNCH_CHECK();
    umi_launch_wgrad_reduce(splits, 9, Ci, Co, o, s);
    UMI_LAUNCH_CHECK();
    return UMI_OK;
}
```

### unet-torch_amd/umi/graph.py

```python
import os

import torch

from . import lib as L
from . import ops


def _fuse_bnred():
    return os.environ.get("UMI_NO_BNRED_FUSION") != "1"


def _defer_wgrad_reduce():
    return os.environ.get("UMI_NO_WGRAD_REDUCE_GROUP") != "1"


def _fuse_bnapply(Ci):
    mode = os.environ.get("UMI_BNAPPLY_FUSION", "")
    return mode != "0" and (Ci <= int(os.environ.get("UMI_BNAPPLY_MAXCI", "64")) or mode == "all")


class Act:
    __slots__ = ("raw", "tx", "grad", "parts", "needs_grad", "bn_rstd", "bn_part", "bn_part_at", "gives")

    def __init__(self, raw, tx=None, parts=None, needs_grad=True):
        self.raw, self.tx, self.grad, self.parts, self.needs_grad = raw, tx, None, parts, needs_grad
        self.bn_rstd = None
        self.bn_part = None
        self.gives = 0
        self.bn_part_at = -1

    @property
    def shape(self):
        return tuple(self.raw.shape)

    def full_tx(self):
        return self.tx


class Tape:
    def __init__(self, dtype, training, record, loss_scale=1.0, grad_sink=None, pack_cache=None, seed=0, seed_dev=None):
        self.dtype = dtype
        self._seed = int(seed)
        self._seed_dev = seed_dev
        self._drop_count = 0
        self.pack_cache = pack_cache
        self.grad_sink = grad_sink
        self.training = training
        self.record = record
        self.loss_scale = float(loss_scale)
        self.inv = (grad_sink.grad_scale if grad_sink is not None else 1.0) / self.loss_scale
        self.steps = []
        self.param_grads = {}
        self._deferred_unscale = []
        self._deferred_zero = []
        self._nbt = []
        self._wgrad_deferred = None
        self._pending_fill = []
        self._late_adds = []
        self._late_ready = []
        self._inputs = []
        self.conv3x3_flags = 0

    def alloc(self, N, H, W, C, dtype=None, zero=False, device=None):
        f = torch.zeros if zero else torch.empty
        return f((N, H, W, C), dtype=dtype or self.dtype, device=device)

    def _pack(self, kind, weight, wf, k8):
        c = self.pack_cache
        if c is not None and isinstance(weight, torch.nn.Parameter) and weight.dtype == torch.float32:
            return c.get(kind, weight, self.dtype, k8)
        return ops.PACKERS[kind](wf, self.dtype, k8=k8)

    def _f3(self, R, S, stride, pad, cin):
        return self.conv3x3_flags if (R, S, stride, pad) == (3, 3, 1, 1) and cin % 8 == 0 else 0

    def _defer_list(self, weight, gw):
        if self._wgrad_deferred is None:
            return None
        self._mark_deferred_fill(gw)
        return self._wgrad_deferred

    def _mark_deferred_fill(self, *bufs):
        for b in bufs:
            self._pending_fill.append((b.data_ptr(), b.data_ptr() + b.numel() * b.element_size()))

    def _is_pending_fill(self, t):
        a = t.data_ptr()
        return any(lo <= a < hi for lo, hi in self._pending_fill)

    def _new_pgrad(self, p):
        v = self.grad_sink.buffer_for(p) if self.grad_sink is not None else None
        return v if v is not None else torch.empty_like(p, dtype=torch.float32)

    def _set_pgrad(self, p, g):
        key = id(p)
        if key in self.param_grads:
            dst = self.param_grads[key][1]
            if self.grad_sink is not None and self.grad_sink.buffer_for(p) is not None:
                raise NotImplementedError("a parameter used twice in one tape under a gradient sink (umi.ddp.GradReducer)")
            if self._is_pending_fill(dst) or self._is_pending_fill(g):
                self._late_adds.append((dst, g))
            else:
                dst.add_(g)
            return
        v = self.grad_sink.buffer_for(p) if self.grad_sink is not None else None
        late = False
        if v is not None:
            late = self._is_pending_fill(g)
            if v.data_ptr() != g.data_ptr():
                if late:
                    raise RuntimeError("deferred gradient fills must target the sink's bucket slot (Tape._new_pgrad)")
                v.copy_(g)
            g = v
        self.param_grads[key] = (p, g)
        if v is not None:
            if late:
                self._late_ready.append(p)
            else:
                self.grad_sink.mark_ready(p)

    def _set_pgrad_scaled(self, p, g, scale):
        v = self.grad_sink.buffer_for(p) if self.grad_sink is not None else None
        if v is not None and id(p) not in self.param_grads and v.shape == g.shape:
            torch.mul(g, scale, out=v)
            self._set_pgrad(p, v)
        else:
            self._set_pgrad(p, g * scale)

    def _give(self, act: Act, g):
        if act.parts is not None:
            for part, c0, c1 in act.parts:
                self._give(part, g[..., c0:c1])
            return
        if not act.needs_grad:
            return
        act.gives += 1
        if act.grad is None:
            act.grad = g
        else:
            act.grad.add_(g)

    def _accumulate_target(self, act: Act, src, R, S, stride, pad):
        if (act.parts is not None or not act.needs_grad or act.grad is None or act.grad.dtype != torch.float16
                or os.environ.get("UMI_NO_DGRAD_ACCUMULATE") == "1"):
            return None
        return act.grad if ops.conv_accumulate_ok(src, act.grad, R, S, stride, pad) else None

    def finish_forward(self):
        if self._nbt:
            torch._foreach_add_(self._nbt, 1)
            self._nbt = []

    def input_nchw(self, x: torch.Tensor, needs_grad=False):
        if not x.is_cuda:
            raise RuntimeError("unet-torch_amd: the HIP path needs the input on device 'cuda' (MI355X); "
                               "no CPU fallback exists in the product path")
        N, C, H, W = x.shape
        raw = torch.empty((N, H, W, C), dtype=self.dtype, device=x.device)
        if C == 1 and x.is_contiguous():
            raw.view(-1).copy_(x.view(-1))
        else:
            raw.copy_(x.permute(0, 2, 3, 1))
        a = Act(raw, None, needs_grad=needs_grad)
        self._inputs.append(a)
        return a

    def input_nhwc(self, raw, tx=None, needs_grad=False):
        a = Act(raw, tx, needs_grad=needs_grad)
        self._inputs.append(a)
        return a

    def conv_bn(self, a: Act, weight, bn, out=None, stride=1, pad=1, input_exclusive=False, relu=True, bias=None):
        Co, Ci, R, S = weight.shape
        N, H, W, Ca = a.shape
        assert Ca == Ci, f"conv expects {Ci} input channels, got {Ca}"
        Ho, Wo = (H + 2 * pad - R) // stride + 1, (W + 2 * pad - S) // stride + 1
        if out is None:
            out = self.alloc(N, Ho, Wo, Co, device=a.raw.device)
        wf = weight.detach().float()
        if (not self.training and not self.record and _eval_fold() and self.dtype == torch.float16 and (R, S, stride, pad) == (3, 3, 1, 1)
                and ops.conv_plan(a.raw, out, 3, 3, 1, 1)[0] == 1):
            tx, _ = ops.eval_bn_tx(bn.weight.detach(), bn.bias.detach(), bn.running_mean, bn.running_var, bn.eps)
            if bias is not None:
                tx[:, 2] += tx[:, 1] * bias.detach().float()
            if not relu:
                tx[:, 3] = ops.NEG_INF
            if ops.conv3x3_fwd_act(a.raw, a.tx, self._pack("conv_fwd", weight, wf, True), tx, out):
                return Act(out, None)
        part, flags, two_pass = None, self._f3(R, S, stride, pad, Ci), False
        if self.training and (R, S) == (1, 1):
            two_pass = (self.dtype == torch.float16 and Co % 8 == 0 and
                        ops.conv_plan(a.raw, out, R, S, stride, pad, 0, False)[0] == 1)
            narrow = self.dtype == torch.float16 and Co <= 8
            flags = 0 if (two_pass or narrow) else L.CONV_FORCE_GENERIC
        res = ops.conv_fwd(a.raw, a.tx, lambda lay: self._pack("conv_fwd", weight, wf, bool(lay)), None, out,
                           R, S, stride, pad, want_stats=self.training and not two_pass, flags=flags)
        part = ops.bn_stats(out) if two_pass else res
        if self.training and part is None:
            raise RuntimeError("conv_bn: no BatchNorm statistics were produced for this layer")
        if self.training:
            mom = bn.momentum if bn.momentum is not None else 0.1
            tx, rstd = ops.bn_finalize(part, Co, N * Ho * Wo, bn.weight.detach(), bn.bias.detach(), bn.eps, mom,
                                       bn.running_mean if bn.track_running_stats else None,
                                       bn.running_var if bn.track_running_stats else None)
            if bn.track_running_stats and bn.num_batches_tracked is not None:
                self._nbt.append(bn.num_batches_tracked)
            if bias is not None and bn.track_running_stats:
                bn.running_mean.add_(bias.detach().float(), alpha=mom)
        else:
            tx, rstd = ops.eval_bn_tx(bn.weight.detach(), bn.bias.detach(), bn.running_mean, bn.running_var, bn.eps)
            if bias is not None:
                tx[:, 2] += tx[:, 1] * bias.detach().float()
        if not relu:
            tx[:, 3] = ops.NEG_INF
        o = Act(out, tx)
        o.bn_rstd = rstd
        if self.record:
            def bwd():
                if o.grad is None:
                    return
                if not self.training:
                    raise RuntimeError("backward through BatchNorm in eval mode is not supported by the HIP path")
                inv = self.inv
                partials = o.bn_part if o.bn_part_at == o.gives else None
                fuse = (_fuse_bnapply(Ci) and self.dtype == torch.float16 and (R, S, stride, pad) == (3, 3, 1, 1)
                        and Ci % 8 == 0 and Co % 8 == 0)
                stem_fuse = (not fuse and self.dtype == torch.float16 and (R, S, stride, pad) == (3, 3, 1, 1) and Ci <= 4
                             and Co % 8 == 0 and not _wants_grad(a) and os.environ.get("UMI_NO_STEM_BNAPPLY") != "1")
                dbeta, dgamma = ops.bn_bwd(o.grad, out, tx, rstd, partials=partials, apply=not (fuse or stem_fuse))
                o.bn_part = None
                if self.grad_sink is None and inv != 1.0:
                    self._deferred_unscale += [dgamma, dbeta]
                    self._set_pgrad(bn.weight, dgamma)
                    self._set_pgrad(bn.bias, dbeta)
                else:
                    self._set_pgrad_scaled(bn.weight, dgamma, inv)
                    self._set_pgrad_scaled(bn.bias, dbeta, inv)
                gw = self._new_pgrad(weight)
                if fuse:
                    dz = self.alloc(N, Ho, Wo, Co, device=out.device)
                    if ops.conv_wgrad_bnapply(a.raw, a.tx, o.grad, out, tx, rstd, dbeta, dgamma, dz, gw, Ci * R * S, R * S, 1,
                                              inv, R, S, stride, pad):
                        o.grad = dz
                    else:
                        fuse = False
                        ops.bn_bwd_apply(o.grad, out, tx, rstd, dbeta, dgamma)
                if stem_fuse:
                    if not ops.conv_wgrad_bnapply(a.raw, a.tx, o.grad, out, tx, rstd, dbeta, dgamma, None, gw, Ci * R * S, R * S, 1,
                                                  inv, R, S, stride, pad):
                        stem_fuse = False
                        ops.bn_bwd_apply(o.grad, out, tx, rstd, dbeta, dgamma)
                if not fuse and not stem_fuse:
                    ops.conv_wgrad(a.raw, a.tx, o.grad, None, gw, Ci * R * S, R * S, 1, inv, R, S, stride, pad,
                                   flags=self._f3(R, S, stride, pad, Ci), defer=self._defer_list(weight, gw))
                self._set_pgrad(weight, gw)
                if bias is not None:
                    gb = self._new_pgrad(bias)
                    if self.grad_sink is None:
                        self._deferred_zero.append(gb)
                        self._mark_deferred_fill(gb)
                    else:
                        gb.zero_()
                    self._set_pgrad(bias, gb)
                if _wants_grad(a):
                    if stride != 1:
                        raise NotImplementedError("dgrad for strided conv_bn")
                    tgt = self._accumulate_target(a, o.grad, R, S, 1, R - 1 - pad)
                    if tgt is not None:
                        ops.conv_fwd(o.grad, None, lambda lay: self._pack("conv_dgrad", weight, wf, bool(lay)), None, tgt,
                                     R, S, 1, R - 1 - pad, flags=L.CONV_ACCUMULATE)
                        a.gives += 1
                        return
                    dx = self.alloc(N, H, W, Ci, device=out.device)
                    part = None
                    if (input_exclusive and _fuse_bnred() and a.grad is None and a.parts is None and a.bn_rstd is not None
                            and a.tx is not None and (R, S, pad) == (3, 3, 1) and self.dtype == torch.float16):
                        part = ops.conv_dgrad_bnred(o.grad, self._pack("conv_dgrad", weight, wf, True), dx, a.raw, a.tx,
                                                    a.bn_rstd)
                    if part is not None:
                        a.bn_part, a.bn_part_at = part, a.gives + 1
                    else:
                        ops.conv_fwd(o.grad, None, lambda lay: self._pack("conv_dgrad", weight, wf, bool(lay)), None, dx,
                                     R, S, 1, R - 1 - pad, flags=self._f3(R, S, stride, R - 1 - pad, Co))
                    self._give(a, dx)
            self.steps.append(bwd)
        return o

    def conv_bias(self, a: Act, weight, bias, out_dtype=None, pad=0):
        Co, Ci, R, S = weight.shape
        N, H, W, Ca = a.shape
        assert Ca == Ci
        out = self.alloc(N, H + 2 * pad - R + 1, W + 2 * pad - S + 1, Co, dtype=out_dtype or self.dtype,
                         device=a.raw.device)
        wf0 = weight.detach().float()
        ops.conv_fwd(a.raw, a.tx, lambda lay: self._pack("conv_fwd", weight, wf0, bool(lay)),
                     bias.detach().float() if bias is not None else None, out, R, S, 1, pad)
        o = Act(out, None)
        if self.record:
            def bwd():
                if o.grad is None:
                    return
                inv = self.inv
                g = o.grad
                gw = self._new_pgrad(weight)
                dx, part, fused_w = None, None, False
                if (_wants_grad(a) and (R, S, pad) == (1, 1, 0) and _fuse_bnred() and os.environ.get("UMI_NO_HEAD_BNRED") != "1"
                        and a.grad is None and a.parts is None and a.bn_rstd is not None and a.tx is not None
                        and self.dtype == torch.float16 and g.dtype == torch.float16):
                    dx = self.alloc(N, H, W, Ci, device=out.device)
                    wf = weight.detach().float()
                    want_w = os.environ.get("UMI_NO_HEAD_WGRAD_FUSION") != "1"
                    part = ops.head_dgrad_bnred(g, self._pack("conv_dgrad", weight, wf, False), dx, a.raw, a.tx, a.bn_rstd,
                                                dW=gw if want_w else None, out_scale=inv)
                    fused_w = part is not None and want_w
                if not fused_w:
                    ops.conv_wgrad(a.raw, a.tx, g, None, gw, Ci * R * S, R * S, 1, inv, R, S, 1, pad,
                                   defer=self._defer_list(weight, gw))
                self._set_pgrad(weight, gw)
                if bias is not None:
                    gb = self._new_pgrad(bias)
                    ops.colsum(g, gb, inv)
                    self._set_pgrad(bias, gb)
                if _wants_grad(a):
                    if dx is None:
                        dx = self.alloc(N, H, W, Ci, device=out.device)
                    if part is not None:
                        a.bn_part, a.bn_part_at = part, a.gives + 1
                    else:
                        wf = weight.detach().float()
                        ops.conv_fwd(g, None, lambda lay: self._pack("conv_dgrad", weight, wf, bool(lay)), None, dx,
                                     R, S, 1, R - 1 - pad)
                    self._give(a, dx)
            self.steps.append(bwd)
        return o

    def pool2(self, a: Act):
        N, H, W, C = a.shape
        out = self.alloc(N, H // 2, W // 2, C, device=a.raw.device)
        ops.pool2_fwd(a.raw, a.tx, out)
        o = Act(out, None)
        if self.record:
            def bwd():
                if o.grad is None or not _wants_grad(a):
                    return
                if a.parts is not None:
                    raise NotImplementedError("pool2 backward into a concat input")
                acc = a.grad is not None
                if not acc:
                    a.grad = self.alloc(N, H, W, C, device=out.device)
                part = None
                if (a.bn_rstd is not None and a.tx is not None and self.dtype == torch.float16 and _fuse_bnred()
                        and os.environ.get("UMI_NO_POOLRED_FUSION") != "1"):
                    part = ops.pool2_bwd_bnred(o.grad, a.raw, a.tx, a.bn_rstd, a.grad, acc)
                if part is None:
                    ops.pool2_bwd(o.grad, a.raw, a.tx, a.grad, acc)
                a.gives += 1
                a.bn_part, a.bn_part_at = part, a.gives
            self.steps.append(bwd)
        return o

    def conv_transpose2x2(self, a: Act, weight, bias, dest, out_hw=None, bias_cancelled=False):
        Cin, Cout = weight.shape[:2]
        N, h, w, Ca = a.shape
        assert Ca == Cin
        _, Hd, Wd, Cd = dest.shape
        assert Cd == Cout
        dY, dX = Hd - 2 * h, Wd - 2 * w
        if dY < 0 or dX < 0:
            raise NotImplementedError("skip smaller than the upsampled map (negative F.pad) is not supported")
        oy, ox = dY // 2, dX // 2
        if dY or dX:
            dest.zero_()
        wf = weight.detach().float()
        ops.conv_fwd(a.raw, a.tx, lambda lay: self._pack("convT_fwd", weight, wf, bool(lay)),
                     bias.detach().float() if bias is not None else None, dest, 2, 2, 2, 0,
                     flags=L.CONV_UPSAMPLE2, up_offset=(oy, ox))
        o = Act(dest, None)
        if self.record:
            def bwd():
                if o.grad is None:
                    return
                inv = self.inv
                g = o.grad
                if dY or dX:
                    g = g[:, oy:oy + 2 * h, ox:ox + 2 * w, :].contiguous()
                gw = self._new_pgrad(weight)
                dlist = self._defer_list(weight, gw)
                fused = False
                if bias is not None:
                    gb = self._new_pgrad(bias)
                    if bias_cancelled and self.training and not (dY or dX):
                        gb.zero_()
                    elif os.environ.get("UMI_NO_CONVT_BIAS_FUSION") != "1" and ops.convT_wgrad_bias(g, a.raw, a.tx, gw, gb, inv,
                                                                                                    defer=dlist):
                        fused = True
                    else:
                        ops.colsum(g, gb, inv)
                    self._set_pgrad(bias, gb)
                if not fused:
                    ops.conv_wgrad(g, None, a.raw, a.tx, gw, Cout * 4, 4, 1, inv, 2, 2, 2, 0, defer=dlist)
                self._set_pgrad(weight, gw)
                if _wants_grad(a):
                    tgt = self._accumulate_target(a, g, 2, 2, 2, 0)
                    if tgt is not None:
                        ops.conv_fwd(g, None, lambda lay: self._pack("convT_dgrad", weight, wf, bool(lay)), None, tgt,
                                     2, 2, 2, 0, flags=L.CONV_ACCUMULATE)
                        a.gives += 1
                        return
                    dx = self.alloc(N, h, w, Cin, device=dest.device)
                    part = None
                    if (_fuse_bnred() and os.environ.get("UMI_NO_CONVT_BNRED") != "1" and a.grad is None and a.parts is None
                            and a.bn_rstd is not None and a.tx is not None and self.dtype == torch.float16 and g.dtype == torch.float16):
                        part = ops.conv_gather_bnred(g, self._pack("convT_dgrad", weight, wf, True), dx, a.raw, a.tx, a.bn_rstd,
                                                     2, 2, 2, 0)
                    if part is not None:
                        a.bn_part, a.bn_part_at = part, a.gives + 1
                    else:
                        ops.conv_fwd(g, None, lambda lay: self._pack("convT_dgrad", weight, wf, bool(lay)), None, dx,
                                     2, 2, 2, 0)
                    self._give(a, dx)
            self.steps.append(bwd)
        return o

    def dropout(self, a: Act, p):
        if not self.training or p <= 0.0:
            return a
        from . import ops_tu
        N, H, W, C = a.shape
        out = self.alloc(N, H, W, C, device=a.raw.device)
        mask = torch.empty(N * H * W * C, dtype=torch.uint8, device=a.raw.device)
        self._drop_count += 1
        ops_tu.dropout(a.raw, out, mask, False, p, (self._seed * 7919 + self._drop_count) & 0x7FFFFFFF, a.tx,
                       seed_dev=self._seed_dev)
        o = Act(out, None)
        if self.record:
            def bwd():
                if o.grad is None or not _wants_grad(a):
                    return
                dx = self.alloc(N, H, W, C, device=out.device)
                ops_tu.dropout(o.grad, dx, mask, True, p, 0)
                self._give(a, dx)
            self.steps.append(bwd)
        return o

    def copy_into(self, a: Act, dest):
        assert a.parts is None and tuple(dest.shape) == a.shape
        dest.copy_(a.raw)
        o = Act(dest, a.tx, needs_grad=a.needs_grad)
        if self.record:
            def bwd():
                if o.grad is not None and _wants_grad(a):
                    self._give(a, o.grad)
            self.steps.append(bwd)
        return o

    def add_relu(self, a: Act, b: Act):
        N, H, W, C = a.shape
        assert b.shape == a.shape
        out = self.alloc(N, H, W, C, device=a.raw.device)
        ops.add2_relu(a.raw, a.tx, b.raw, b.tx, out)
        o = Act(out, None)
        if self.record:
            def bwd():
                if o.grad is None:
                    return
                da = self.alloc(N, H, W, C, device=out.device)
                db = self.alloc(N, H, W, C, device=out.device)
                ops.add2_relu_bwd(o.grad, out, da, db)
                self._give(a, da)
                self._give(b, db)
            self.steps.append(bwd)
        return o

    def gate(self, x: Act, p: Act, dest):
        N, H, W, C = x.shape
        assert p.shape == (N, H, W, 1) and tuple(dest.shape) == x.shape
        ops.gate(x.raw, x.tx, p.raw, p.tx, dest)
        o = Act(dest, None)
        if self.record:
            def bwd():
                if o.grad is None:
                    return
                dx = self.alloc(N, H, W, C, device=dest.device)
                dp = self.alloc(N, H, W, 1, device=dest.device)
                ops.gate_bwd(o.grad, x.raw, x.tx, p.raw, p.tx, dx, dp)
                self._give(x, dx)
                self._give(p, dp)
            self.steps.append(bwd)
        return o

    def concat(self, buf, acts):
        txs, parts, c0 = [], [], 0
        for a in acts:
            C = a.shape[3]
            assert a.raw.data_ptr() == buf[..., c0:c0 + C].data_ptr(), "concat part is not a slice of the buffer"
            txs.append(a.tx if a.tx is not None else ops.passthrough_tx_const(C, buf.device))
            parts.append((a, c0, c0 + C))
            c0 += C
        assert c0 == buf.shape[3]
        if all(a.tx is None for a in acts):
            return Act(buf, None, parts=parts)
        return Act(buf, torch.cat(txs, 0).contiguous(), parts=parts)

    def output_nchw_plain(self, a: Act):
        assert a.tx is None
        return a.raw.permute(0, 3, 1, 2).contiguous().float()

    def seed_grad_nchw(self, a: Act, g_nchw: torch.Tensor):
        N, C, H, W = g_nchw.shape
        g = g_nchw.permute(0, 2, 3, 1)
        if self.loss_scale != 1.0:
            g = g * self.loss_scale
        a.grad = torch.empty((N, H, W, C), dtype=self.dtype, device=g_nchw.device)
        a.grad.copy_(g)

    _defer_under_sink = False

    def _flush_deferred(self):
        if self._wgrad_deferred:
            ops.wgrad_reduce_flush(self._wgrad_deferred)
        if self._deferred_zero:
            torch._foreach_zero_(self._deferred_zero)
            self._deferred_zero = []
        self._finish_param_grads()
        for dst, src in self._late_adds:
            dst.add_(src)
        self._late_adds, self._pending_fill = [], []
        for p in self._late_ready:
            self.grad_sink.mark_ready(p)
        self._late_ready = []

    def backward(self):
        self._wgrad_deferred = [] if ((self.grad_sink is None or self._defer_under_sink) and _defer_wgrad_reduce()) else None
        for step in reversed(self.steps):
            step()
        self.steps = []
        self._flush_deferred()
        self._wgrad_deferred = None
        if self._deferred_unscale:
            torch._foreach_mul_(self._deferred_unscale, self.inv)
            self._deferred_unscale = []
        if self.grad_sink is not None:
            self.grad_sink.finish()

    def _finish_param_grads(self):
        """Hook: parameter-gradient work batched at the end of the backward pass (TUTape: StdConv2d standardisation)."""

    def input_grad_nchw(self, a: Act):
        if a.grad is None:
            return None
        g = a.grad.permute(0, 3, 1, 2).float()
        if self.loss_scale != 1.0:
            g = g / self.loss_scale
        return g.contiguous()


def _eval_fold():
    import os
    return os.environ.get("UMI_NO_EVAL_FOLD") != "1"


def dropout_seeds(module, device, training):
    if not training or device.type != "cuda":
        return 0, None
    if getattr(module, "_drop_base", None) is None:
        module._drop_base = int(torch.randint(0, 2 ** 31 - 1, (1,)).item())
    ctr = getattr(module, "_drop_step", None)
    if ctr is None or ctr.device != device:
        if torch.cuda.is_current_stream_capturing():
            raise RuntimeError("first training forward inside a HIP-graph capture; run one eager step first")
        ctr = module._drop_step = torch.zeros(1, dtype=torch.int32, device=device)
    ctr.add_(1)
    return module._drop_base, ctr


def pack_cache_of(module):
    import os
    if os.environ.get("UMI_NO_PACK_CACHE") == "1":
        return None
    c = module.__dict__.get("_umi_pack_cache")
    if c is None:
        c = module.__dict__["_umi_pack_cache"] = ops.PackCache()
    c.refresh()
    return c


def _wants_grad(a: Act):
    if a.parts is not None:
        return any(_wants_grad(p) for p, _, _ in a.parts)
    return a.needs_grad


def default_loss_scale(dtype, n_pixels):
    if dtype != torch.float16:
        return 1.0
    import math
    return float(2 ** max(0, int(math.floor(math.log2(max(n_pixels, 1)))) - 3))
```

### unet-torch_amd/umi/ops.py

```python

import numpy as np
import torch

from . import lib as L

NEG_INF = float("-inf")


def _dt(t: torch.Tensor) -> int:
    if t.dtype == torch.float32:
        return L.UMI_F32
    if t.dtype == torch.float16:
        return L.UMI_F16
    raise TypeError(f"libunetmi supports float32/float16 storage, got {t.dtype}")


def torch_dtype(code: int):
    return torch.float32 if code == L.UMI_F32 else torch.float16


def _stream():
    return torch.cuda.current_stream().cuda_stream


# ... 341 lines not shown
        Ho, Wo = H, W
    else:
        Ho, Wo = (H + 2 * pad - R) // stride + 1, (W + 2 * pad - S) // stride + 1
        assert (oH, oW) == (Ho, Wo), f"output view {oH}x{oW} != conv output {Ho}x{Wo}"
    part = None
    layout, rows = conv_plan(x, y, R, S, stride, pad, flags, bias is not None)
    if callable(wp):
        wp = wp(layout)
    elif layout != 0:
        raise ValueError("this conv takes the MFMA path: pass a callable so the weights get the k8 packing")
    if want_stats:
        part = torch.empty(rows * 2 * Co, dtype=torch.float32, device=x.device)
    if tx is not None:
        assert tx.shape == (Ci, 4) and tx.dtype == torch.float32 and tx.is_contiguous()
    L.call("umi_conv_fwd", x.data_ptr(), ldx, _ptr(tx), wp.data_ptr(), _ptr(bias), y.data_ptr(), ldy,
           _ptr(part), N, H, W, Ci, Co, R, S, stride, pad, Ho, Wo,
           up_offset[0], up_offset[1], oH, oW, _dt(x), _dt(y), flags, _stream())
    return part


def conv3x3_fwd_act(x, tx, wp8, out_tx, y):
    N, H, W, Ci, ldx = _nhwc(x)
    _, _, _, Co, ldy = _nhwc(y)
    return L.supported("umi_conv3x3_fwd_act", x.data_ptr(), ldx, _ptr(tx), wp8.data_ptr(), out_tx.data_ptr(), y.data_ptr(), ldy,
                       N, H, W, Ci, Co, _dt(x), _stream())


def bn_finalize(part, C, count, gamma, beta, eps, momentum, running_mean, running_var):
    rows = part.numel() // (2 * C)
    tx = torch.empty(C, 4, dtype=torch.float32, device=part.device)
    rstd = torch.empty(C, dtype=torch.float32, device=part.device)
    L.call("umi_bn_finalize", part.data_ptr(), rows, C, float(count), _ptr(gamma), _ptr(beta), eps, momentum,
           _ptr(running_mean), _ptr(running_var), tx.data_ptr(), rstd.data_ptr(),
           _stream())
    return tx, rstd


def pool2_fwd(x, tx, y):
    N, H, W, C, ldx = _nhwc(x)
    _, Ho, Wo, _, ldy = _nhwc(y)
    assert (Ho, Wo) == (H // 2, W // 2)
    L.call("umi_pool2_fwd", x.data_ptr(), ldx, _ptr(tx), y.data_ptr(), ldy, N, H, W, C, _dt(x), _stream())


def pool2_bwd(dpool, x, tx, da, accumulate):
    N, H, W, C, ldx = _nhwc(x)
    _, _, _, _, lddp = _nhwc(dpool)
    _, _, _, _, ldda = _nhwc(da)
    L.call("umi_pool2_bwd", dpool.data_ptr(), lddp, x.data_ptr(), ldx, _ptr(tx), da.data_ptr(), ldda,
           int(accumulate), N, H, W, C, _dt(x), _stream())


def bn_stats(y):
    N, H, W, C, ldy = _nhwc(y)
    M = N * H * W
    rows = L.fn("umi_bn_stats_rows")(M, C) if y.dtype == torch.float16 else 0
    if rows <= 0:
        return None
    part = torch.empty(rows * 2 * C, dtype=torch.float32, device=y.device)
    if not L.supported("umi_bn_stats", y.data_ptr(), ldy, part.data_ptr(), M, C, _dt(y), _stream()):
        return None
    return part


def pool2_bwd_bnred(dpool, x, tx, rstd, da, accumulate):
    N, H, W, C, ldx = _nhwc(x)
    rows = L.fn("umi_pool2_bwd_bnred_stat_rows")(N, H, W, C)
    if rows <= 0 or x.dtype != torch.float16 or tx is None or rstd is None:
        return None
    part = torch.empty(rows * 2 * C, dtype=torch.float32, device=x.device)
    if not L.supported("umi_pool2_bwd_bnred", dpool.data_ptr(), _nhwc(dpool)[4], x.data_ptr(), ldx, tx.data_ptr(),
                       rstd.data_ptr(), da.data_ptr(), _nhwc(da)[4], int(accumulate), part.data_ptr(), N, H, W, C, _dt(x),
                       _stream()):
        return None
    return part


_ws_cache = {}
_ws_high = {}
_ws_pinned = []


def workspace(nbytes, device):
    key = (device, torch.cuda.current_stream().cuda_stream)
    buf = _ws_cache.get(key)
    need = max(int(nbytes), _ws_high.get(device, 1 << 20))
    _ws_high[device] = need
    if buf is None or buf.numel() < nbytes:
        if buf is not None and torch.cuda.is_current_stream_capturing():
            _ws_pinned.append(buf)
        buf = torch.empty(need, dtype=torch.uint8, device=device)
        _ws_cache[key] = buf
    return buf


def conv_dgrad_bnred(dy, wp8, da, ybn, txbn, rstd):
    N, H, W, Ci, lddy = _nhwc(dy)
    _, _, _, Co, ldda = _nhwc(da)
    ldybn = _nhwc(ybn)[4]
    lay, rows = conv_plan(dy, da, 3, 3, 1, 1)
    if lay != 1:
        return None
    part = torch.empty(rows * 2 * Co, dtype=torch.float32, device=dy.device)
    if not L.supported("umi_conv_dgrad_bnred", dy.data_ptr(), lddy, wp8.data_ptr(), da.data_ptr(), ldda, ybn.data_ptr(), ldybn,
                       txbn.data_ptr(), rstd.data_ptr(), part.data_ptr(), N, H, W, Ci, Co, _dt(dy), _stream()):
        return None
    return part


def conv_gather_bnred(x, wp8, y, ybn, txbn, rstd, R, S, stride, pad, flags=0):
    N, H, W, Ci, ldx = _nhwc(x)
    _, Ho, Wo, Co, ldy = _nhwc(y)
    ldybn = _nhwc(ybn)[4]
    if x.dtype != torch.float16 or y.dtype != torch.float16 or ybn.dtype != torch.float16:
        return None
    if (x.data_ptr() | y.data_ptr() | ybn.data_ptr()) & 15:
        return None
    rows = L.fn("umi_conv_gather_bnred_rows")(N, H, W, Ci, Co, R, S, stride, pad, Ho, Wo, ldx, ldy, _dt(x), flags)
    if rows <= 0:
        return None
    part = torch.empty(rows * 2 * Co, dtype=torch.float32, device=x.device)
    if not L.supported("umi_conv_gather_bnred", x.data_ptr(), ldx, wp8.data_ptr(), y.data_ptr(), ldy, ybn.data_ptr(), ldybn,
                       txbn.data_ptr(), rstd.data_ptr(), part.data_ptr(), N, H, W, Ci, Co, R, S, stride, pad,
                       Ho, Wo, _dt(x), flags, _stream()):
        return None
    return part


def head_dgrad_bnred(dl, wp, da, ybn, txbn, rstd, dW=None, out_scale=1.0):
    N, H, W, Ci, lddl = _nhwc(dl)
    _, _, _, Co, ldda = _nhwc(da)
    ldybn = _nhwc(ybn)[4]
    P = N * H * W
    if dl.dtype != torch.float16 or da.dtype != torch.float16 or ybn.dtype != torch.float16:
        return None
    rows = L.fn("umi_head_dgrad_bnred_rows")(P, Ci, Co, ldda, _dt(dl))
    if rows <= 0:
        return None
    part = torch.empty(rows * 2 * Co, dtype=torch.float32, device=dl.device)
    if dW is not None:
        assert dW.dtype == torch.float32 and dW.is_contiguous() and dW.numel() == Ci * Co
        ws = workspace(L.fn("umi_head_bwd_fused_ws_bytes")(P, Ci, Co), dl.device)
        if not L.supported("umi_head_bwd_fused", dl.data_ptr(), lddl, wp.data_ptr(), da.data_ptr(), ldda, ybn.data_ptr(), ldybn,
                           txbn.data_ptr(), rstd.data_ptr(), part.data_ptr(), dW.data_ptr(), Co, 1, out_scale,
                           ws.data_ptr(), ws.numel(), P, Ci, Co, _dt(dl), _stream()):
            return None
        return part
    if not L.supported("umi_head_dgrad_bnred", dl.data_ptr(), lddl, wp.data_ptr(), da.data_ptr(), ldda, ybn.data_ptr(), ldybn,
                       txbn.data_ptr(), rstd.data_ptr(), part.data_ptr(), P, Ci, Co, _dt(dl), _stream()):
        return None
    return part


def bn_bwd(da, y, tx, rstd, partials=None, apply=True):
    N, H, W, C, ldy = _nhwc(y)
    _, _, _, _, ldda = _nhwc(da)
    M = N * H * W
    nb = L.fn("umi_bn_bwd_ws_bytes")(M, C)
    ws = workspace(nb, y.device)
    sums = torch.empty(2, C, dtype=torch.float32, device=y.device)
    if partials is not None:
        L.call("umi_bn_bwd_from_partials", partials.data_ptr(), partials.numel() // (2 * C), C, sums[0].data_ptr(),
               sums[1].data_ptr(), _stream())
    else:
        L.call("umi_bn_bwd_reduce", da.data_ptr(), ldda, y.data_ptr(), ldy, tx.data_ptr(), rstd.data_ptr(),
               sums[0].data_ptr(), sums[1].data_ptr(), M, C, _dt(y), ws.data_ptr(),
               ws.numel(), _stream())
    if apply:
        bn_bwd_apply(da, y, tx, rstd, sums[0], sums[1])
    return sums[0], sums[1]


def bn_bwd_apply(da, y, tx, rstd, sum_dz, sum_dzx):
    N, H, W, C, ldy = _nhwc(y)
    L.call("umi_bn_bwd_apply", da.data_ptr(), _nhwc(da)[4], y.data_ptr(), ldy, tx.data_ptr(), rstd.data_ptr(),
           sum_dz.data_ptr(), sum_dzx.data_ptr(), N * H * W, C, _dt(y), _stream())


def conv_wgrad_bnapply(x, txa, da, y, tx_bn, rstd, sum_dz, sum_dzx, dz, dW, s_co, s_ci, s_t, out_scale, R, S, stride, pad):
    N, H, W, Ci, ldx = _nhwc(x)
    _, Ho, Wo, Co, ldda = _nhwc(da)
    if (Ho, Wo) != (H, W) or da.dtype != torch.float16:
        return False
    assert dW.dtype == torch.float32 and dW.is_contiguous() and (dz is None or dz.shape == da.shape)
    nb = L.fn("umi_conv_wgrad_ws_bytes")(N, Ho, Wo, Ci, Co, R, S, _dt(x), 0)
    ws = workspace(nb, x.device)
    return L.supported("umi_conv_wgrad_bnapply", x.data_ptr(), ldx, _ptr(txa), da.data_ptr(), ldda, y.data_ptr(), _nhwc(y)[4],
                       tx_bn.data_ptr(), rstd.data_ptr(), sum_dz.data_ptr(), sum_dzx.data_ptr(),
                       _ptr(dz), _nhwc(dz)[4] if dz is not None else 0, dW.data_ptr(), s_co, s_ci, s_t, out_scale,
                       N, H, W, Ci, Co, R, S, stride, pad, _dt(x), 0, ws.data_ptr(), ws.numel(), _stream())


_WgPending = L.STRUCTS["umi_wgrad_pending"]


def conv_wgrad(x, txa, dy, txb, dW, s_co, s_ci, s_t, out_scale, R, S, stride, pad, flags=0, defer=None):
    import ctypes
    N, H, W, Ci, ldx = _nhwc(x)
    _, Ho, Wo, Co, lddy = _nhwc(dy)
    assert dW.dtype == torch.float32 and dW.is_contiguous()
    nb = L.fn("umi_conv_wgrad_ws_bytes")(N, Ho, Wo, Ci, Co, R, S, _dt(x), flags)
    if defer is None:
        ws = workspace(nb, x.device)
        L.call("umi_conv_wgrad", x.data_ptr(), ldx, _ptr(txa), dy.data_ptr(), lddy, _ptr(txb), dW.data_ptr(),
               s_co, s_ci, s_t, out_scale, N, H, W, Ci, Co, R, S, stride, pad, Ho, Wo,
               _dt(x), flags, ws.data_ptr(), ws.numel(), _stream())
        return
    ws = torch.empty(max(nb, 16), dtype=torch.uint8, device=x.device)
    pend = _WgPending()
    L.call("umi_conv_wgrad_deferred", x.data_ptr(), ldx, _ptr(txa), dy.data_ptr(), lddy, _ptr(txb), dW.data_ptr(),
           s_co, s_ci, s_t, out_scale, N, H, W, Ci, Co, R, S, stride, pad, Ho, Wo,
           _dt(x), flags, ws.data_ptr(), ws.numel(), ctypes.addressof(pend), _stream())
    if pend.part:
        defer.append((pend, ws, dW))


def convT_wgrad_bias(g, y, txy, dW, dbias, out_scale, defer=None):
    import ctypes
    N, H, W, Ci, ldx = _nhwc(g)
    _, Ho, Wo, Co, lddy = _nhwc(y)
    if g.dtype != torch.float16 or (H, W) != (2 * Ho, 2 * Wo):
        return False
    assert dW.dtype == torch.float32 and dW.is_contiguous() and dbias.dtype == torch.float32 and dbias.numel() == Ci
    nb = L.fn("umi_conv_wgrad_ws_bytes")(N, Ho, Wo, Ci, Co, 2, 2, _dt(g), 0)
    ws = torch.empty(max(nb, 16), dtype=torch.uint8, device=g.device) if defer is not None else workspace(nb, g.device)
    pend = _WgPending()
    assert dW.numel() == Ci * Co * 4
    if not L.supported("umi_conv_wgrad_bias", g.data_ptr(), ldx, y.data_ptr(), lddy, _ptr(txy), dW.data_ptr(), Ci * 4, 4, 1,
                       dbias.data_ptr(), out_scale, N, H, W, Ci, Co, Ho, Wo, _dt(g), 0, ws.data_ptr(), ws.numel(),
                       ctypes.addressof(pend) if defer is not None else None, _stream()):
        return False
    if defer is not None and pend.part:
        defer.append((pend, ws, dW))
    return True


def wgrad_pending(part, dW, s_co, s_ci, s_t, scale, splits, RS, Ci, Co):
    addr = [p.data_ptr() if torch.is_tensor(p) else p for p in (part, dW)]
    return _WgPending(addr[0], addr[1], s_co, s_ci, s_t, scale, splits, RS, Ci, Co)


def wgrad_reduce_group(pending, check=True):
    import ctypes
    arr = (_WgPending * max(len(pending), 1))(*pending)
    st = L.fn("umi_wgrad_reduce_group")(len(pending), ctypes.addressof(arr), _stream())
    if check:
        L.check(st, "umi_wgrad_reduce_group")
    return st


def wgrad_reduce_flush(defer):
    if defer:
        wgrad_reduce_group([d[0] for d in defer])
        del defer[:]


def conv_wgrad_group(xs, dys, dWs, s_co, s_ci, out_scale):
    import ctypes
    n = len(xs)
    N, H, W, Ci, ldx = _nhwc(xs[0])
    _, _, _, Co, lddy = _nhwc(dys[0])
    for x, dy, dW in zip(xs, dys, dWs):
        assert _nhwc(x) == (N, H, W, Ci, ldx) and _nhwc(dy) == (N, H, W, Co, lddy) and x.dtype == xs[0].dtype
        assert dW.dtype == torch.float32
    arr = ctypes.c_void_p * n
    ptrs = [arr(*[t.data_ptr() for t in ts]) for ts in (xs, dys, dWs)]
    return L.supported("umi_conv_wgrad_group", n, ctypes.cast(ptrs[0], ctypes.c_void_p), ldx,
                       ctypes.cast(ptrs[1], ctypes.c_void_p), lddy, ctypes.cast(ptrs[2], ctypes.c_void_p), s_co, s_ci, out_scale,
                       N * H * W, Ci, Co, _dt(xs[0]), _stream())


def colsum(x, out, out_scale):
    N, H, W, C, ldx = _nhwc(x)
    M = N * H * W
    ws = workspace(L.fn("umi_colsum_ws_bytes")(M, C), x.device)
    L.call("umi_colsum", x.data_ptr(), ldx, out.data_ptr(), out_scale, M, C, _dt(x), ws.data_ptr(),
           ws.numel(), _stream())


def colsum_group(xs, outs, out_scale):
    import ctypes
    n = len(xs)
    N, H, W, C, ldx = _nhwc(xs[0])
    M = N * H * W
    if xs[0].dtype != torch.float16 or C % 8 or ldx % 8:
        return False
    for x, o in zip(xs, outs):
        assert _nhwc(x) == (N, H, W, C, ldx) and o.dtype == torch.float32 and o.numel() == C
    ws = workspace(min(n, 16) * L.fn("umi_colsum_ws_bytes")(M, C), xs[0].device)
    arr = ctypes.c_void_p * n
    px, po = arr(*[t.data_ptr() for t in xs]), arr(*[t.data_ptr() for t in outs])
    return L.supported("umi_colsum_group", n, ctypes.cast(px, ctypes.c_void_p), ldx, ctypes.cast(po, ctypes.c_void_p), out_scale,
                       M, C, _dt(xs[0]), ws.data_ptr(), ws.numel(), _stream())


def add2_relu(a, txa, b, txb, y):
    N, H, W, C, lda = _nhwc(a)
    _, _, _, _, ldb = _nhwc(b)
    _, _, _, _, ldy = _nhwc(y)
    assert a.shape == b.shape == y.shape
    L.call("umi_add2_relu_fwd", a.data_ptr(), lda, _ptr(txa), b.data_ptr(), ldb, _ptr(txb), y.data_ptr(), ldy,
           N * H * W, C, _dt(a), _stream())


def add2_relu_bwd(dy, y, da, db):
    N, H, W, C, lddy = _nhwc(dy)
    L.call("umi_add2_relu_bwd", dy.data_ptr(), lddy, y.data_ptr(), _nhwc(y)[4], da.data_ptr(), _nhwc(da)[4],
           db.data_ptr(), _nhwc(db)[4], N * H * W, C, _dt(dy), _stream())


def gate(x, txx, p, txp, y):
    N, H, W, C, ldx = _nhwc(x)
    assert tuple(p.shape) == (N, H, W, 1) and p.is_contiguous() and y.shape == x.shape
    L.call("umi_gate_fwd", x.data_ptr(), ldx, _ptr(txx), p.data_ptr(), _ptr(txp), y.data_ptr(), _nhwc(y)[4],
           N * H * W, C, _dt(x), _stream())


def gate_bwd(dy, x, txx, p, txp, dx, dp):
    N, H, W, C, ldx = _nhwc(x)
    assert dp.is_contiguous() and tuple(dp.shape) == (N, H, W, 1)
    L.call("umi_gate_bwd", dy.data_ptr(), _nhwc(dy)[4], x.data_ptr(), ldx, _ptr(txx), p.data_ptr(), _ptr(txp),
           dx.data_ptr(), _nhwc(dx)[4], dp.data_ptr(), N * H * W, C, _dt(x), _stream())


def materialize_nchw(x, tx):
    N, H, W, C, ldx = _nhwc(x)
    y = torch.empty(N, C, H, W, dtype=torch.float32, device=x.device)
    L.call("umi_materialize_nchw", x.data_ptr(), ldx, _ptr(tx), y.data_ptr(), N, H, W, C, _dt(x), _stream())
    return y
```

Baseline: 756.9.

## Keep head input gradient low-rank and rebuild it inside fused wgrad BN-apply

The 1x1 head's input gradient (Ci channels) is no longer materialized. It is kept as a low-rank pair: the head output gradient (K<=3 channels) and the packed head weight. BN statistics and the head dW come from a stats-only variant of the head kernel that skips the store. The preceding 3x3 wgrad+BN-apply kernel then rebuilds the dense gradient on the fly from the K-channel gradient and weights, which removes a full-resolution write and read of the widest activation gradient. The cost is extra per-element FMAs and narrow loads in the wgrad kernel, plus a fallback path that densifies when the fused route does not apply.

```diff
diff --git a/include/unetmi.h b/include/unetmi.h
--- a/include/unetmi.h
+++ b/include/unetmi.h
@@ -78,6 +78,9 @@
 int umi_head_bwd_fused(const void* dl, int lddl, const void* wp, void* da, int ldda, const void* ybn, int ldybn,
                        const void* txbn, const float* rstd, float* part, float* dW, long s_co, long s_ci, float out_scale,
                        void* ws, size_t ws_bytes, long P, int Ci, int Co, int dtype, umi_stream_t stream);
+int umi_head_bwd_stats(const void* dl, int lddl, const void* wp, const void* ybn, int ldybn, const void* txbn, const float* rstd,
+                       float* part, float* dW, long s_co, long s_ci, float out_scale, void* ws, size_t ws_bytes, long P, int Ci,
+                       int Co, int dtype, umi_stream_t stream);
 
 int umi_conv3x3_fwd_act(const void* x, int ldx, const void* tx, const void* wp8, const void* out_tx, void* y, int ldy,
                         int N, int H, int W, int Ci, int Co, int dtype, umi_stream_t stream);
@@ -115,6 +118,11 @@
                            int lddz, float* dW, long s_co, long s_ci, long s_t, float out_scale, int N, int H, int W,
                            int Ci, int Co, int R, int S, int stride, int pad, int dtype, int flags, void* ws,
                            size_t ws_bytes, umi_stream_t stream);
+int umi_conv_wgrad_bnapply_lowrank(const void* x, int ldx, const void* txa, const void* dl, int lddl, const void* wl, int K,
+                                   const void* y, int ldy, const void* tx_bn, const float* rstd, const float* sum_dz,
+                                   const float* sum_dzx, void* dz, int lddz, float* dW, long s_co, long s_ci, long s_t,
+                                   float out_scale, int N, int H, int W, int Ci, int Co, int dtype, int flags, void* ws,
+                                   size_t ws_bytes, umi_stream_t stream);
 
 size_t umi_colsum_ws_bytes(long M, int C);
 int umi_colsum(const void* x, int ldx, float* out, float out_scale, long M, int C, int dtype,
diff --git a/unet-torch_amd/csrc/api.hip b/unet-torch_amd/csrc/api.hip
--- a/unet-torch_amd/csrc/api.hip
+++ b/unet-torch_amd/csrc/api.hip
@@ -97,6 +97,14 @@
     if (!dl || !wp || !da || !ybn || !txbn || !rstd || !part || !dW || !ws || P <= 0) return UMI_ERR_BADARG;
     if (!head_dgrad_ok(Ci, Co, ldda, dtype) || Co > 256 || ldybn % 8 || ldybn < Co || lddl < Ci) return UMI_ERR_UNSUPPORTED;
     return umi_smallk_fwd_bnred(dl, lddl, wp, da, ldda, ybn, ldybn, txbn, rstd, part, P, Ci, Co, (hipStream_t)stream, dW, s_co, s_ci,
+                                out_scale, ws, ws_bytes);
+}
+extern "C" int umi_head_bwd_stats(const void* dl, int lddl, const void* wp, const void* ybn, int ldybn, const void* txbn,
+                                  const float* rstd, float* part, float* dW, long s_co, long s_ci, float out_scale, void* ws,
+                                  size_t ws_bytes, long P, int Ci, int Co, int dtype, umi_stream_t stream) {
+    if (!dl || !wp || !ybn || !txbn || !rstd || !part || !dW || !ws || P <= 0) return UMI_ERR_BADARG;
+    if (!head_dgrad_ok(Ci, Co, Co, dtype) || Co > 256 || ldybn % 8 || ldybn < Co || lddl < Ci) return UMI_ERR_UNSUPPORTED;
+    return umi_smallk_fwd_bnred(dl, lddl, wp, nullptr, 0, ybn, ldybn, txbn, rstd, part, P, Ci, Co, (hipStream_t)stream, dW, s_co, s_ci,
                                 out_scale, ws, ws_bytes);
 }
 
@@ -293,3 +301,21 @@
         return UMI_ERR_UNSUPPORTED;
     return umi_wgrad3x3_mfma(p, x, txa, da, o, (hipStream_t)stream, &bna);
 }
+
+extern "C" int umi_conv_wgrad_bnapply_lowrank(const void* x, int ldx, const void* txa, const void* dl, int lddl, const void* wl, int K,
+                                              const void* y, int ldy, const void* tx_bn, const float* rstd, const float* sum_dz,
+                                              const float* sum_dzx, void* dz, int lddz, float* dW, long s_co, long s_ci, long s_t,
+                                              float out_scale, int N, int H, int W, int Ci, int Co, int dtype, int flags, void* ws,
+                                              size_t ws_bytes, umi_stream_t stream) {
+    if (!x || !dl || !wl || !y || !tx_bn || !rstd || !sum_dz || !sum_dzx || !dz || !dW || !ws || N <= 0 || H <= 0 || W <= 0 ||
+        Ci <= 0 || Co <= 0 || K <= 0 || ldx < Ci || ldy < Co || lddz < Co || dz == y || dz == dl)
+        return UMI_ERR_BADARG;
+    const WgradProblem p = wgrad_problem(N, H, W, Ci, Co, 3, 3, 1, 1, H, W, ldx, (Co + 7) / 8 * 8, dtype, flags, txa != nullptr, false);
+    if (umi_conv_wgrad_path(p) != WGRAD_MFMA3X3 || !umi_wgrad3x3_lowrank_ok(p, K, lddl) || ldy % 8 || lddz % 8 ||
+        (long)H * W * (ldy > lddz ? ldy : lddz) * 2 >= 0x7FFFFFF0L)
+        return UMI_ERR_UNSUPPORTED;
+    const WgradOut o{dW, s_co, s_ci, s_t, out_scale, ws, ws_bytes, nullptr, nullptr};
+    const WgradBnApply bna{y, ldy, tx_bn, rstd, sum_dz, sum_dzx, dz, lddz};
+    const WgradLowRank lr{dl, lddl, wl, K};
+    return umi_wgrad3x3_mfma(p, x, txa, nullptr, o, (hipStream_t)stream, &bna, &lr);
+}
diff --git a/unet-torch_amd/csrc/common.h b/unet-torch_amd/csrc/common.h
--- a/unet-torch_amd/csrc/common.h
+++ b/unet-torch_amd/csrc/common.h
@@ -45,6 +45,11 @@
 template <>
 __device__ __forceinline__ float umi_bn_dz<float>(float y, float g, const float4 t, float rstd, float c1, float c2) {
     return t.y * umi_bn_dz_inner(y, g, t, rstd, c1, c2);
+}
+
+__device__ __forceinline__ _Float16 umi_round_f16(float a) {
+    asm volatile("" : "+v"(a));
+    return (_Float16)a;
 }
 
 typedef _Float16 umi_half8 __attribute__((ext_vector_type(8)));
diff --git a/unet-torch_amd/csrc/kernels.h b/unet-torch_amd/csrc/kernels.h
--- a/unet-torch_amd/csrc/kernels.h
+++ b/unet-torch_amd/csrc/kernels.h
@@ -81,10 +81,13 @@
     float* convT_bias;
 };
 struct WgradBnApply { const void* y; int ldy; const void* tx_bn; const float *rstd, *sum_dz, *sum_dzx; void* dz; int lddz; };
+struct WgradLowRank { const void* dl; int lddl; const void* w; int K; };
+constexpr int UMI_WGRAD_LOWRANK_MAXK = 3;
 enum WgradPath { WGRAD_MFMA3X3_F32, WGRAD_MFMA3X3, WGRAD_MFMA1X1, WGRAD_T, WGRAD_GATHER, WGRAD_STEM, WGRAD_HEAD, WGRAD_ROOT, WGRAD_HEAD3, WGRAD_GENERIC };
 
 bool umi_wgrad3x3_f32_mfma_ok(const WgradProblem& p);
 bool umi_wgrad3x3_mfma_ok(const WgradProblem& p);
+bool umi_wgrad3x3_lowrank_ok(const WgradProblem& p, int K, int lddl);
 bool umi_wgrad1x1_mfma_ok(const WgradProblem& p);
 bool umi_wgradT_mfma_ok(const WgradProblem& p);
 bool umi_wgrad_gather_mfma_ok(const WgradProblem& p);
@@ -124,7 +127,7 @@
 
 int umi_wgrad3x3_f32_mfma(const WgradProblem& p, const void* x, const void* txa, const void* dy, const WgradOut& o, hipStream_t s);
 int umi_wgrad3x3_mfma(const WgradProblem& p, const void* x, const void* txa, const void* dy, const WgradOut& o, hipStream_t s,
-                      const WgradBnApply* bna = nullptr);
+                      const WgradBnApply* bna = nullptr, const WgradLowRank* lr = nullptr);
 int umi_wgrad1x1_mfma(const WgradProblem& p, const void* x, const void* txa, const void* dy, const WgradOut& o, hipStream_t s);
 int umi_wgradT_mfma(const WgradProblem& p, const void* x, const void* dy, const void* txb, const WgradOut& o, hipStream_t s);
 int umi_wgrad_gather_mfma(const WgradProblem& p, const void* x, const void* txa, const void* dy, const WgradOut& o, hipStream_t s);
diff --git a/unet-torch_amd/csrc/stem_head.hip b/unet-torch_amd/csrc/stem_head.hip
--- a/unet-torch_amd/csrc/stem_head.hip
+++ b/unet-torch_amd/csrc/stem_head.hip
@@ -302,13 +302,13 @@
             float a = 0.f;
 #pragma unroll
             for (int k = 0; k < NC; ++k) a = fmaf(d[k], w[k][j], a);
-            o[j] = (half_t)a;
+            o[j] = umi_round_f16(a);
         }
         *reinterpret_cast<half8*>(y + p * ldy + cg * 8) = o;
     }
 }
 
-template <int NC>
+template <int NC, bool STORE = true>
 __global__ __launch_bounds__(256) void smallk1x1_bnred_kernel(const half_t* __restrict__ x, int ldx,
                                                               const half_t* __restrict__ wp, half_t* __restrict__ y,
                                                               int ldy, const half_t* __restrict__ ybn, int ldybn,
@@ -343,7 +343,7 @@
             float a = 0.f;
 #pragma unroll
             for (int k = 0; k < NC; ++k) a = fmaf(d[k], w[k][j], a);
-            o[j] = (half_t)a;
+            o[j] = umi_round_f16(a);
             const float yy = (float)yv[j];
             const float dz = umi_tx_pre(yy, t[j]) > t[j].w ? (float)o[j] : 0.f;
             s[j] += dz;
@@ -354,7 +354,7 @@
                 for (int k = 0; k < NC; ++k) wacc[k][j] = fmaf(av, d[k], wacc[k][j]);
             }
         }
-        *reinterpret_cast<half8*>(y + p * ldy + cg * 8) = o;
+        if (STORE) *reinterpret_cast<half8*>(y + p * ldy + cg * 8) = o;
     }
 #pragma unroll
     for (int j = 0; j < 8; ++j) { red[0][threadIdx.x][j] = s[j]; red[1][threadIdx.x][j] = q[j]; }
@@ -551,17 +551,19 @@
 int umi_smallk_fwd_bnred(const void* x, int ldx, const void* wp, void* y, int ldy, const void* ybn, int ldybn, const void* txbn,
                          const float* rstd, float* part, long P, int Ci, int Co, hipStream_t s, float* dW, long s_co, long s_ci,
                          float out_scale, void* ws, size_t ws_bytes) {
-    if (!al16(y) || !al16(ybn)) return UMI_ERR_BADARG;
+    if ((y && !al16(y)) || !al16(ybn)) return UMI_ERR_BADARG;
     int grid = grid_for(P * (Co / 8));
     float* wpart = nullptr;
     if (dW) {
         if (!ws || ws_bytes < (size_t)grid * Co * Ci * sizeof(float)) return UMI_ERR_WORKSPACE;
         wpart = (float*)ws;
     }
-#define GO(NC) hipLaunchKernelGGL(smallk1x1_bnred_kernel<NC>, dim3(grid), dim3(256), 0, s, (const half_t*)x, ldx, (const half_t*)wp, (half_t*)y, ldy, (const half_t*)ybn, ldybn, (const float4*)txbn, rstd, part, P, Co, wpart)
+#define GO_(NC, ST) hipLaunchKernelGGL((smallk1x1_bnred_kernel<NC, ST>), dim3(grid), dim3(256), 0, s, (const half_t*)x, ldx, (const half_t*)wp, (half_t*)y, ldy, (const half_t*)ybn, ldybn, (const float4*)txbn, rstd, part, P, Co, wpart)
+#define GO(NC) do { if (y) GO_(NC, true); else GO_(NC, false); } while (0)
     switch (Ci) { case 1: GO(1); break; case 2: GO(2); break; case 3: GO(3); break; case 4: GO(4); break;
                   case 5: GO(5); break; case 6: GO(6); break; case 7: GO(7); break; default: GO(8); }
 #undef GO
+#undef GO_
     UMI_LAUNCH_CHECK();
     if (dW) {
         hipLaunchKernelGGL(head_wpart_reduce_kernel, dim3(Co * Ci), dim3(256), 0, s, (const float*)wpart, grid, Co, Ci, dW, s_co, s_ci,
diff --git a/unet-torch_amd/csrc/wgrad_mfma.hip b/unet-torch_amd/csrc/wgrad_mfma.hip
--- a/unet-torch_amd/csrc/wgrad_mfma.hip
+++ b/unet-torch_amd/csrc/wgrad_mfma.hip
@@ -238,9 +238,10 @@
 struct BnApply {
     const half_t* y; int ldy; const float4* tx; const float* rstd; const float* sum_dz; const float* sum_dzx; long M;
     half_t* dz; int lddz;
+    const half_t* lrw; int lr_wide;
 };
 
-template <bool HAS_TX, bool BNA>
+template <bool HAS_TX, bool BNA, int LRK = 0>
 __global__ __launch_bounds__(512, 1) void wgrad3x3_ws_kernel(
     const half_t* __restrict__ x, int ldx, const float4* __restrict__ tx, const half_t* __restrict__ dy, int lddy,
     float* __restrict__ part, int N, int H, int W, int Ci, int Co, int tiles_x, int tiles_y, int tiles_total,
@@ -310,6 +311,23 @@
                 c1[j] = in ? ba.sum_dz[c] * invM : 0.f;
                 c2[j] = in ? ba.sum_dzx[c] * invM : 0.f;
             }
+        }
+        static_assert(LRK == 0 || BNA, "the low-rank gradient operand exists only with the BatchNorm apply");
+        constexpr int LRN = LRK > 0 ? LRK : 1;
+        typedef half_t half2v __attribute__((ext_vector_type(2)));
+        constexpr int LRW = (LRN + 1) / 2;
+        typedef unsigned uint4v __attribute__((ext_vector_type(4)));
+        half8 wlr[LRN];
+        unsigned dlr0[KPB][LRW], dlr1[KPB][LRW];
+        const int boffl = bcol * lddy * 2;
+        if (LRK > 0) {
+#pragma unroll
+            for (int kk = 0; kk < LRN; ++kk)
+#pragma unroll
+                for (int j = 0; j < 8; ++j) {
+                    const int c = co0 + sub * 8 + j;
+                    wlr[kk][j] = c < Co ? ba.lrw[kk * Co + c] : (half_t)0.f;
+                }
         }
         half8 yraw0[KPB], yraw1[KPB];
         bool bvalid0[KPB], bvalid1[KPB];
@@ -353,8 +371,18 @@
         }                                                                                                       \
         _Pragma("unroll") for (int k = 0; k < KPB; ++k) {                                                       \
             const bool ok = b_on && (whole_tiles || (nx_y + k < H && nx_x + bcol < W));                         \
-            braw##S[k] = __builtin_bit_cast(half8, __builtin_amdgcn_raw_buffer_load_b128(                       \
-                yrs, UMI_EXP_LOAD_OK(ok) ? (unsigned)boff0 : OOB, bbase + k * W * lddy * 2, 0));                \
+            if (LRK == 0) {                                                                                     \
+                braw##S[k] = __builtin_bit_cast(half8, __builtin_amdgcn_raw_buffer_load_b128(                   \
+                    yrs, UMI_EXP_LOAD_OK(ok) ? (unsigned)boff0 : OOB, bbase + k * W * lddy * 2, 0));            \
+            } else if (LRK == 2 && ba.lr_wide) {                                            \
+                dlr##S[k][0] = __builtin_amdgcn_raw_buffer_load_b32(yrs, ok ? (unsigned)boffl : OOB, bbase + k * W * lddy * 2, 0); \
+            } else {                                                                                            \
+                _Pragma("unroll") for (int kk = 0; kk < LRN; ++kk) {                                            \
+                    const unsigned h_ = (unsigned short)__builtin_amdgcn_raw_buffer_load_b16(                   \
+                        yrs, ok ? (unsigned)(boffl + 2 * kk) : OOB, bbase + k * W * lddy * 2, 0);               \
+                    dlr##S[k][kk >> 1] = (kk & 1) ? (dlr##S[k][kk >> 1] | (h_ << 16)) : h_;                     \
+                }                                                                                               \
+            }                                                                                                   \
             if (BNA) {                                                                                          \
                 const __amdgpu_buffer_rsrc_t ybrs = __builtin_amdgcn_make_buffer_rsrc((void*)(ba.y + nx_n * ybimg), 0, (int)(ybimg * 2), 0x00020000); \
                 bvalid##S[k] = ok;                                                                              \
@@ -384,7 +412,34 @@
         }                                                                                                       \
         _Pragma("unroll") for (int k = 0; k < KPA; ++k)                                                         \
             if ((ptid >> 3) + 32 * k < HPIX) *reinterpret_cast<half8*>(sb + a_lds + k * 32 * PROW) = araw##S[k]; \
-        if (BNA) {                                                                                              \
+        if (LRK > 0) {                                                                                          \
+             \
+            _Pragma("unroll") for (int k = 0; k < KPB; ++k) {                                                   \
+                half8 b_;                                                                                       \
+                 \
+                if (LRK >= 3) {                                                                                 \
+                    _Pragma("unroll") for (int kk = 0; kk < LRN; ++kk) {                                        \
+                        uint4v w_ = __builtin_bit_cast(uint4v, wlr[kk]);                                        \
+                        asm volatile("" : "+v"(w_));                                                            \
+                        wlr[kk] = __builtin_bit_cast(half8, w_);                                                \
+                    }                                                                                           \
+                }                                                                                               \
+                _Pragma("unroll") for (int j = 0; j < 8; ++j) {                                                 \
+                    float a_ = 0.f;                                                                             \
+                    _Pragma("unroll") for (int kk = 0; kk < LRN; ++kk)                                          \
+                        a_ = fmaf((float)__builtin_bit_cast(half2v, dlr##S[k][kk >> 1])[kk & 1],                \
+                                  (float)wlr[kk][j], a_);                                                       \
+                    b_[j] = umi_round_f16(a_);                 \
+                }                                                                                               \
+                const half8 o = umi_bn_dz8(yraw##S[k], b_, tb, rsb, c1, c2);                                    \
+                b_ = bvalid##S[k] ? o : b_;                                                                     \
+                if (dz_writer && bvalid##S[k])                                                                  \
+                    *reinterpret_cast<half8*>(ba.dz + ((long)((long)st_n##S * H + st_y##S + k) * W + st_x##S + bcol) * ba.lddz + \
+                                              co0 + sub * 8) = b_;                                              \
+                *reinterpret_cast<half8*>(sb + b_lds + k * 32 * PROW) = b_;                                     \
+                __builtin_amdgcn_sched_barrier(0);                                                              \
+            }                                                                                                   \
+        } else if (BNA) {                                                                                              \
             _Pragma("unroll") for (int k = 0; k < KPB; ++k) {                                                   \
                 const half8 o = umi_bn_dz8(yraw##S[k], braw##S[k], tb, rsb, c1, c2);    \
                 braw##S[k] = bvalid##S[k] ? o : braw##S[k];              \
@@ -393,7 +448,9 @@
                                               co0 + sub * 8) = braw##S[k];                                      \
             }                                                                                                   \
         }                                                                                                       \
-        _Pragma("unroll") for (int k = 0; k < KPB; ++k) *reinterpret_cast<half8*>(sb + b_lds + k * 32 * PROW) = braw##S[k]; \
+        if (LRK == 0) {                                                                                         \
+            _Pragma("unroll") for (int k = 0; k < KPB; ++k) *reinterpret_cast<half8*>(sb + b_lds + k * 32 * PROW) = braw##S[k]; \
+        }                                                                                                       \
     } while (0)
 #endif
 
@@ -1063,21 +1120,56 @@
     return (size_t)splits * 9 * p.Ci * p.Co * sizeof(float);
 }
 
+bool umi_wgrad3x3_lowrank_ok(const WgradProblem& p, int K, int lddl) {
+    if (!umi_wgrad3x3_mfma_ok(p)) return false;
+    if (K < 1 || K > UMI_WGRAD_LOWRANK_MAXK || lddl < K) return false;
+    return (long)p.H * p.W * lddl * 2 < 0x7FFFFFF0L;
+}
+
 int umi_wgrad3x3_mfma(const WgradProblem& p, const void* x, const void* txa, const void* dy, const WgradOut& o, hipStream_t s,
-                      const WgradBnApply* bna) {
-    const int N = p.N, H = p.H, W = p.W, Ci = p.Ci, Co = p.Co, ldx = p.ldx, lddy = p.lddy;
+                      const WgradBnApply* bna, const WgradLowRank* lr) {
+    const int N = p.N, H = p.H, W = p.W, Ci = p.Ci, Co = p.Co, ldx = p.ldx, lddy = lr ? lr->lddl : p.lddy;
+    if (lr) {
+        if (!bna) return UMI_ERR_BADARG;
+        dy = lr->dl;
+    }
     void* const ws = o.ws;
     int tiles_x, tiles_y, tiles_total, splits, tps;
     plan(N, H, W, Ci, Co, &tiles_x, &tiles_y, &tiles_total, &splits, &tps);
     if (o.ws_bytes < (size_t)splits * 9 * Ci * Co * sizeof(float)) return UMI_ERR_WORKSPACE;
-    if (((uintptr_t)x | (uintptr_t)dy) & 15) return UMI_ERR_BADARG;
+    if (((uintptr_t)x | (lr ? (uintptr_t)0 : (uintptr_t)dy)) & 15) return UMI_ERR_BADARG;
+    if (lr && ((((uintptr_t)lr->dl | (uintptr_t)lr->w) & 1))) return UMI_ERR_BADARG;
     const int n_co_t = (Co + 63) / 64;
     dim3 grid(((Ci + 63) / 64) * n_co_t, splits), block(256);
     static const int force_fast = [] { const char* e = getenv("UMI_WGRAD_FAST_CI"); return e ? atoi(e) : -1; }();
     const int fast_ci = force_fast >= 0 ? force_fast : (Co < 1.59 * Ci ? 1 : 0);
     static const bool classic = [] { const char* e = getenv("UMI_WGRAD_CLASSIC"); return e && e[0] == '1'; }();
     if (bna && classic) return UMI_ERR_UNSUPPORTED;
-    if (!classic) {
+    if (lr) {
+        constexpr int dyn = WS_SMEM + 64 * (int)sizeof(float4);
+        static const int attr_rc_lr = [] {
+            int rc = 0;
+#define UMI_LR_ATTR(K_)                                                                                                                   \
+            if (!rc) rc = (int)hipFuncSetAttribute((const void*)wgrad3x3_ws_kernel<true, true, K_>, hipFuncAttributeMaxDynamicSharedMemorySize, dyn); \
+            if (!rc) rc = (int)hipFuncSetAttribute((const void*)wgrad3x3_ws_kernel<false, true, K_>, hipFuncAttributeMaxDynamicSharedMemorySize, dyn)
+            UMI_LR_ATTR(1); UMI_LR_ATTR(2); UMI_LR_ATTR(3);
+#undef UMI_LR_ATTR
+            return rc;
+        }();
+        if (attr_rc_lr) return attr_rc_lr;
+        const int wide = lr->K == 2 && lddy % 2 == 0 && ((uintptr_t)dy & 3) == 0;
+        const BnApply ba{(const half_t*)bna->y, bna->ldy, (const float4*)bna->tx_bn, bna->rstd, bna->sum_dz, bna->sum_dzx,
+                         (long)N * H * W, (half_t*)bna->dz, bna->lddz, (const half_t*)lr->w, wide};
+#define GO_LR(HT, K_)                                                                                               \
+        hipLaunchKernelGGL((wgrad3x3_ws_kernel<HT, true, K_>), grid, dim3(512), dyn, s, (const half_t*)x, ldx, (const float4*)txa,   \
+                           (const half_t*)dy, lddy, (float*)ws, N, H, W, Ci, Co, tiles_x, tiles_y, tiles_total, tps, n_co_t, fast_ci, ba)
+#define GO_LRK(K_) do { if (txa) GO_LR(true, K_); else GO_LR(false, K_); } while (0)
+        static_assert(UMI_WGRAD_LOWRANK_MAXK == 3, "one instantiation pair per supported K");
+        switch (lr->K) { case 1: GO_LRK(1); break; case 2: GO_LRK(2); break; case 3: GO_LRK(3); break;
+                         default: return UMI_ERR_UNSUPPORTED; }
+#undef GO_LRK
+#undef GO_LR
+    } else if (!classic) {
         constexpr int dyn = WS_SMEM + 64 * (int)sizeof(float4);
         static const int attr_rc = [] {
             int a = (int)hipFuncSetAttribute((const void*)wgrad3x3_ws_kernel<true, false>, hipFuncAttributeMaxDynamicSharedMemorySize, dyn);
@@ -1089,8 +1181,8 @@
         if (attr_rc) return attr_rc;
         dim3 block_ws(512);
         const BnApply ba = bna ? BnApply{(const half_t*)bna->y, bna->ldy, (const float4*)bna->tx_bn, bna->rstd, bna->sum_dz, bna->sum_dzx,
-                                         (long)N * H * W, (half_t*)bna->dz, bna->lddz}
-                               : BnApply{nullptr, 0, nullptr, nullptr, nullptr, nullptr, 1, nullptr, 0};
+                                         (long)N * H * W, (half_t*)bna->dz, bna->lddz, nullptr, 0}
+                               : BnApply{nullptr, 0, nullptr, nullptr, nullptr, nullptr, 1, nullptr, 0, nullptr, 0};
 #define GO_WS(HT, BN_)                                                                                              \
         hipLaunchKernelGGL((wgrad3x3_ws_kernel<HT, BN_>), grid, block_ws, dyn, s, (const half_t*)x, ldx, (const float4*)txa,   \
                            (const half_t*)dy, lddy, (float*)ws, N, H, W, Ci, Co, tiles_x, tiles_y, tiles_total, tps, n_co_t, fast_ci, ba)
diff --git a/unet-torch_amd/umi/graph.py b/unet-torch_amd/umi/graph.py
--- a/unet-torch_amd/umi/graph.py
+++ b/unet-torch_amd/umi/graph.py
@@ -19,13 +19,21 @@
     return mode != "0" and (Ci <= int(os.environ.get("UMI_BNAPPLY_MAXCI", "64")) or mode == "all")
 
 
+class LowRankGrad:
+    __slots__ = ("dl", "wl", "dense")
+
+    def __init__(self, dl, wl, dense):
+        self.dl, self.wl, self.dense = dl, wl, dense
+
+
 class Act:
-    __slots__ = ("raw", "tx", "grad", "parts", "needs_grad", "bn_rstd", "bn_part", "bn_part_at", "gives")
+    __slots__ = ("raw", "tx", "grad", "parts", "needs_grad", "bn_rstd", "bn_part", "bn_part_at", "gives", "lowrank_ok")
 
     def __init__(self, raw, tx=None, parts=None, needs_grad=True):
         self.raw, self.tx, self.grad, self.parts, self.needs_grad = raw, tx, None, parts, needs_grad
         self.bn_rstd = None
         self.bn_part = None
+        self.lowrank_ok = False
         self.gives = 0
         self.bn_part_at = -1
 
@@ -138,10 +146,16 @@
         if act.grad is None:
             act.grad = g
         else:
-            act.grad.add_(g)
+            self._dense_grad(act).add_(g)
+
+    @staticmethod
+    def _dense_grad(act: Act):
+        if isinstance(act.grad, LowRankGrad):
+            act.grad = act.grad.dense()
+        return act.grad
 
     def _accumulate_target(self, act: Act, src, R, S, stride, pad):
-        if (act.parts is not None or not act.needs_grad or act.grad is None or act.grad.dtype != torch.float16
+        if (act.parts is not None or not act.needs_grad or act.grad is None or self._dense_grad(act).dtype != torch.float16
                 or os.environ.get("UMI_NO_DGRAD_ACCUMULATE") == "1"):
             return None
         return act.grad if ops.conv_accumulate_ok(src, act.grad, R, S, stride, pad) else None
@@ -215,6 +229,8 @@
             tx[:, 3] = ops.NEG_INF
         o = Act(out, tx)
         o.bn_rstd = rstd
+        o.lowrank_ok = (self.training and _fuse_bnapply(Ci) and self.dtype == torch.float16 and (R, S, stride, pad) == (3, 3, 1, 1)
+                        and Ci % 8 == 0 and Co % 8 == 0)
         if self.record:
             def bwd():
                 if o.grad is None:
@@ -227,7 +243,12 @@
                         and Ci % 8 == 0 and Co % 8 == 0)
                 stem_fuse = (not fuse and self.dtype == torch.float16 and (R, S, stride, pad) == (3, 3, 1, 1) and Ci <= 4
                              and Co % 8 == 0 and not _wants_grad(a) and os.environ.get("UMI_NO_STEM_BNAPPLY") != "1")
-                dbeta, dgamma = ops.bn_bwd(o.grad, out, tx, rstd, partials=partials, apply=not (fuse or stem_fuse))
+                lr = o.grad if isinstance(o.grad, LowRankGrad) else None
+                if lr is not None and not (fuse and partials is not None):
+                    lr = None
+                    self._dense_grad(o)
+                dbeta, dgamma = ops.bn_bwd(None if lr is not None else o.grad, out, tx, rstd, partials=partials,
+                                           apply=not (fuse or stem_fuse))
                 o.bn_part = None
                 if self.grad_sink is None and inv != 1.0:
                     self._deferred_unscale += [dgamma, dbeta]
@@ -239,8 +260,11 @@
                 gw = self._new_pgrad(weight)
                 if fuse:
                     dz = self.alloc(N, Ho, Wo, Co, device=out.device)
-                    if ops.conv_wgrad_bnapply(a.raw, a.tx, o.grad, out, tx, rstd, dbeta, dgamma, dz, gw, Ci * R * S, R * S, 1,
-                                              inv, R, S, stride, pad):
+                    if lr is not None and ops.conv_wgrad_bnapply_lowrank(a.raw, a.tx, lr.dl, lr.wl, out, tx, rstd, dbeta, dgamma, dz, gw,
+                                                                         Ci * R * S, R * S, 1, inv):
+                        o.grad = dz
+                    elif ops.conv_wgrad_bnapply(a.raw, a.tx, self._dense_grad(o), out, tx, rstd, dbeta, dgamma, dz, gw, Ci * R * S,
+                                                R * S, 1, inv, R, S, stride, pad):
                         o.grad = dz
                     else:
                         fuse = False
@@ -307,11 +331,21 @@
                 if (_wants_grad(a) and (R, S, pad) == (1, 1, 0) and _fuse_bnred() and os.environ.get("UMI_NO_HEAD_BNRED") != "1"
                         and a.grad is None and a.parts is None and a.bn_rstd is not None and a.tx is not None
                         and self.dtype == torch.float16 and g.dtype == torch.float16):
-                    dx = self.alloc(N, H, W, Ci, device=out.device)
                     wf = weight.detach().float()
                     want_w = os.environ.get("UMI_NO_HEAD_WGRAD_FUSION") != "1"
-                    part = ops.head_dgrad_bnred(g, self._pack("conv_dgrad", weight, wf, False), dx, a.raw, a.tx, a.bn_rstd,
-                                                dW=gw if want_w else None, out_scale=inv)
+                    wl = self._pack("conv_dgrad", weight, wf, False)
+                    if (want_w and a.lowrank_ok and Co <= ops.LOWRANK_MAXK and os.environ.get("UMI_NO_HEAD_LOWRANK") != "1"):
+                        part = ops.head_bwd_stats(g, wl, a.raw, a.tx, a.bn_rstd, gw, out_scale=inv)
+                        if part is not None:
+                            def dense():
+                                da = self.alloc(N, H, W, Ci, device=out.device)
+                                ops.conv_fwd(g, None, lambda lay: self._pack("conv_dgrad", weight, wf, bool(lay)), None, da,
+                                             R, S, 1, R - 1 - pad)
+                                return da
+                            dx = LowRankGrad(g, wl, dense)
+                    if part is None:
+                        dx = self.alloc(N, H, W, Ci, device=out.device)
+                        part = ops.head_dgrad_bnred(g, wl, dx, a.raw, a.tx, a.bn_rstd, dW=gw if want_w else None, out_scale=inv)
                     fused_w = part is not None and want_w
                 if not fused_w:
                     ops.conv_wgrad(a.raw, a.tx, g, None, gw, Ci * R * S, R * S, 1, inv, R, S, 1, pad,
@@ -549,7 +583,7 @@
     def input_grad_nchw(self, a: Act):
         if a.grad is None:
             return None
-        g = a.grad.permute(0, 3, 1, 2).float()
+        g = self._dense_grad(a).permute(0, 3, 1, 2).float()
         if self.loss_scale != 1.0:
             g = g / self.loss_scale
         return g.contiguous()
diff --git a/unet-torch_amd/umi/ops.py b/unet-torch_amd/umi/ops.py
--- a/unet-torch_amd/umi/ops.py
+++ b/unet-torch_amd/umi/ops.py
@@ -517,9 +517,27 @@
     return part
 
 
+def head_bwd_stats(dl, wp, ybn, txbn, rstd, dW, out_scale=1.0):
+    N, H, W, Ci, lddl = _nhwc(dl)
+    _, _, _, Co, ldybn = _nhwc(ybn)
+    P = N * H * W
+    if dl.dtype != torch.float16 or ybn.dtype != torch.float16:
+        return None
+    rows = L.fn("umi_head_dgrad_bnred_rows")(P, Ci, Co, Co, _dt(dl))
+    if rows <= 0:
+        return None
+    assert dW.dtype == torch.float32 and dW.is_contiguous() and dW.numel() == Ci * Co
+    part = torch.empty(rows * 2 * Co, dtype=torch.float32, device=dl.device)
+    ws = workspace(L.fn("umi_head_bwd_fused_ws_bytes")(P, Ci, Co), dl.device)
+    if not L.supported("umi_head_bwd_stats", dl.data_ptr(), lddl, wp.data_ptr(), ybn.data_ptr(), ldybn, txbn.data_ptr(),
+                       rstd.data_ptr(), part.data_ptr(), dW.data_ptr(), Co, 1, out_scale, ws.data_ptr(), ws.numel(), P, Ci, Co,
+                       _dt(dl), _stream()):
+        return None
+    return part
+
+
 def bn_bwd(da, y, tx, rstd, partials=None, apply=True):
     N, H, W, C, ldy = _nhwc(y)
-    _, _, _, _, ldda = _nhwc(da)
     M = N * H * W
     nb = L.fn("umi_bn_bwd_ws_bytes")(M, C)
     ws = workspace(nb, y.device)
@@ -528,7 +546,7 @@
         L.call("umi_bn_bwd_from_partials", partials.data_ptr(), partials.numel() // (2 * C), C, sums[0].data_ptr(),
                sums[1].data_ptr(), _stream())
     else:
-        L.call("umi_bn_bwd_reduce", da.data_ptr(), ldda, y.data_ptr(), ldy, tx.data_ptr(), rstd.data_ptr(),
+        L.call("umi_bn_bwd_reduce", da.data_ptr(), _nhwc(da)[4], y.data_ptr(), ldy, tx.data_ptr(), rstd.data_ptr(),
                sums[0].data_ptr(), sums[1].data_ptr(), M, C, _dt(y), ws.data_ptr(),
                ws.numel(), _stream())
     if apply:
@@ -554,6 +572,24 @@
                        tx_bn.data_ptr(), rstd.data_ptr(), sum_dz.data_ptr(), sum_dzx.data_ptr(),
                        _ptr(dz), _nhwc(dz)[4] if dz is not None else 0, dW.data_ptr(), s_co, s_ci, s_t, out_scale,
                        N, H, W, Ci, Co, R, S, stride, pad, _dt(x), 0, ws.data_ptr(), ws.numel(), _stream())
+
+
+LOWRANK_MAXK = 3
+
+
+def conv_wgrad_bnapply_lowrank(x, txa, dl, wl, y, tx_bn, rstd, sum_dz, sum_dzx, dz, dW, s_co, s_ci, s_t, out_scale):
+    N, H, W, Ci, ldx = _nhwc(x)
+    Nl, Hl, Wl, K, lddl = _nhwc(dl)
+    _, _, _, Co, ldy = _nhwc(y)
+    if (Nl, Hl, Wl) != (N, H, W) or tuple(y.shape[:3]) != (N, H, W) or dl.dtype != torch.float16 or y.dtype != torch.float16:
+        return False
+    assert dW.dtype == torch.float32 and dW.is_contiguous() and tuple(dz.shape) == tuple(y.shape) and wl.numel() == K * Co
+    nb = L.fn("umi_conv_wgrad_ws_bytes")(N, H, W, Ci, Co, 3, 3, _dt(x), 0)
+    ws = workspace(nb, x.device)
+    return L.supported("umi_conv_wgrad_bnapply_lowrank", x.data_ptr(), ldx, _ptr(txa), dl.data_ptr(), lddl, wl.data_ptr(), K,
+                       y.data_ptr(), ldy, tx_bn.data_ptr(), rstd.data_ptr(), sum_dz.data_ptr(), sum_dzx.data_ptr(), dz.data_ptr(),
+                       _nhwc(dz)[4], dW.data_ptr(), s_co, s_ci, s_t, out_scale, N, H, W, Ci, Co, _dt(x), 0, ws.data_ptr(),
+                       ws.numel(), _stream())
 
 
 _WgPending = L.STRUCTS["umi_wgrad_pending"]
```

Result: no change. 760.6 (median of 6 runs) (+0.5%).
